# JeongsooP/RGB-no-more

Hardware: AMD Instinct MI355X
Metric: images/sec JPEG-Ti DCT 512x512 train step (higher is better)
Workload: dtype bf16

## Files before the change

### include/rgbnm.h

```cpp
#ifndef RGBNM_H
#define RGBNM_H
#include <stddef.h>
#include <stdint.h>

#ifdef __cplusplus
extern "C" {
#endif

#define RGBNM_ABI_VERSION 3
#define RGBNM_DT_F32 0
#define RGBNM_DT_BF16 1
#define RGBNM_DT_F16 2
#define RGBNM_DT_I16 2

#define RGBNM_EPI_NONE 0
#define RGBNM_EPI_RES 1
#define RGBNM_EPI_GELU 2
#define RGBNM_EPI_POS 3
#define RGBNM_EPI_DGELU 4
#define RGBNM_EPI_TANH 5
#define RGBNM_EPI_DTANH 6
#define RGBNM_EPI_RES_DROP 7
#define RGBNM_EPI_GELU_DROP 8

// ... 61 lines not shown
                        void* workspace, size_t workspace_bytes, void* stream);

int rgbnm_attention_fwd(int dtype, const void* qkv, void* out, float* lse, int B, int N, int heads, float scale,
                        void* stream);
int rgbnm_attention_bwd(int dtype, const void* qkv, const void* out, const void* dout, const float* lse, void* dqkv,
                        int B, int N, int heads, float scale, void* stream);

int rgbnm_subblock_embed(int in_dtype, int out_dtype, const void* y, const void* cbcr, const float* conv16,
                         void* feat, int B, int Hb, int Wb, int transpose_a, void* stream);
int rgbnm_subblock_embed_mix(int in_dtype, int out_dtype, const void* y, const void* cbcr, const float* lam_dev, const float* conv16,
                             void* feat, int B, int Hb, int Wb, int transpose_a, void* stream);

#define RGBNM_OP_IDENTITY 0
#define RGBNM_OP_AUTOCONTRAST 1
#define RGBNM_OP_POSTERIZE 2
#define RGBNM_OP_SOLARIZEADD 3
#define RGBNM_OP_COLOR 4
#define RGBNM_OP_CONTRAST 5
#define RGBNM_OP_BRIGHTNESS 6
#define RGBNM_OP_MIDFREQAUG 7
#define RGBNM_OP_CUTOUT 8
#define RGBNM_OP_TRANSLATEX 9
#define RGBNM_OP_TRANSLATEY 10
#define RGBNM_OP_ROTATE90 11
#define RGBNM_OP_AUTOSATURATION 12
#define RGBNM_OP_GRAYSCALE 13
#define RGBNM_OP_CHROMADROP 14
#define RGBNM_OP_SHARPNESS 15
#define RGBNM_OP_INVERT 16
#define RGBNM_OP_SOLARIZE 17
#define RGBNM_OP_FREQENHANCE 18
#define RGBNM_OP_EQUALIZE 19

typedef struct rgbnm_aug_params {
  int crop_i, crop_j, crop_h, crop_w;
  int flip;
  int op[2];
  float fmag[2];
  int iarg0[2], iarg1[2], iarg2[2];
} rgbnm_aug_params;

size_t rgbnm_dct_augment_workspace(int B);
int rgbnm_dct_augment(const int16_t* Yq, const int16_t* CbCrq, const int16_t* quant, const rgbnm_aug_params* params_dev,
                      const rgbnm_aug_params* params_host, const float* conv16, const float* filters, void* outY,
                      void* outC, int out_dtype, int B, int Hy, int Wy, int Hc, int Wc, int entry_clamp, int nops,
                      void* workspace, size_t workspace_bytes, void* stream);
size_t rgbnm_dct_augment_workspace_ex(int B, int size);
int rgbnm_dct_augment_ex(const int16_t* Yq, const int16_t* CbCrq, const int16_t* quant, const rgbnm_aug_params* params_dev,
                         const rgbnm_aug_params* params_host, const float* conv16, const float* filters, void* outY,
                         void* outC, int out_dtype, int size, int B, int Hy, int Wy, int Hc, int Wc, int entry_clamp,
                         int nops, void* workspace, size_t workspace_bytes, void* stream);

int rgbnm_dct_augment_packed(const int16_t* Ypacked, const int16_t* Cpacked, const long long* y_off, const long long* c_off,
                             const int16_t* quant, const rgbnm_aug_params* params_dev, const rgbnm_aug_params* params_host,
                             const float* conv16, const float* filters, void* outY, void* outC, int out_dtype, int size, int B,
                             int Hy, int Wy, int Hc, int Wc, int entry_clamp, int nops, void* workspace, size_t workspace_bytes,
                             void* stream);

int rgbnm_softxent(int dl_dtype, const float* logits, const float* soft_target, const long long* hard_target,
                   float* loss_rows, float* loss, void* dlogits, int B, int C, float grad_scale, void* stream);
int rgbnm_softxent_loss(const float* logits, const float* soft_target, const long long* hard_target, float* loss_rows,
                        float* row_stats, float* loss, unsigned* ticket, int B, int C, void* stream);
int rgbnm_softxent_grad(int dl_dtype, const float* logits, const float* soft_target, const long long* hard_target,
                        const float* row_stats, const float* gout_dev, void* dlogits, int B, int C, float grad_scale, void* stream);
int rgbnm_softxent_loss_mix(const float* logits, const long long* labels, const float* mix_lam_dev, float* loss_rows,
                            float* row_stats, float* loss, unsigned* ticket, int B, int C, void* stream);
int rgbnm_softxent_grad_mix(int dl_dtype, const float* logits, const long long* labels, const float* mix_lam_dev,
                            const float* row_stats, const float* gout_dev, void* dlogits, int B, int C, float grad_scale,
                            void* stream);
int rgbnm_mixup(int in_dtype, int out_dtype, const void* in, void* out, const float* lam_dev, int B,
                long long per_sample, void* stream);
int rgbnm_mixup_target(const long long* labels, float* target, const float* lam_dev, int B, int C, void* stream);
size_t rgbnm_clip_adamw_wd_workspace(void);
int rgbnm_clip_adamw_wd_step(float* p, const float* g, float* m, float* v, const unsigned char* wd_flag_per_256,
                             long long n, float lr, float beta1, float beta2, float eps, int step, float wd_factor,
                             float max_norm, float* norm_out, void* workspace, size_t workspace_bytes, void* stream);

typedef struct rgbnm_vit_cfg {
  int dtype, B, N, E, heads;
  float ln_eps, attn_scale;
} rgbnm_vit_cfg;

typedef struct rgbnm_block_params {
  const float *ln1_g, *ln1_b, *ln2_g, *ln2_b;
  const float *bqkv_perm, *bproj, *b1, *b2;
  const void *wqkv, *wqkv_t, *wproj, *wproj_t, *w1, *w1_t, *w2, *w2_t;
} rgbnm_block_params;

typedef struct rgbnm_block_acts {
  void* x_in;
  void* xn1;
  float *mean1, *rstd1;
  void* qkv;
  float* lse;
  void* attn;
  void* x_mid;
  void* xn2;
  float *mean2, *rstd2;
  void* u;
  void* gl;
  void* x_out;
} rgbnm_block_acts;

typedef struct rgbnm_block_grads {
  float *dln1_g, *dln1_b, *dln2_g, *dln2_b;
  float *dwqkv, *dbqkv, *dwproj, *dbproj, *dw1, *db1, *dw2, *db2;
} rgbnm_block_grads;

typedef struct rgbnm_block_scratch {
  void* du;
  void* dxn;
  void* dx_mid;
  void* dattn;
  void* dqkv;
  void* ws;
  size_t ws_bytes;
} rgbnm_block_scratch;

size_t rgbnm_vit_workspace(const rgbnm_vit_cfg* cfg);
size_t rgbnm_vit_workspace_ex(const rgbnm_vit_cfg* cfg, int n_classes);
int rgbnm_vit_block_fwd(const rgbnm_vit_cfg* cfg, const rgbnm_block_params* p, const rgbnm_block_acts* a,
                        void* stream);
int rgbnm_vit_ln_chain(const rgbnm_vit_cfg* cfg);
int rgbnm_vit_block_fwd_chain(const rgbnm_vit_cfg* cfg, const rgbnm_block_params* p, const rgbnm_block_acts* a,
                              int flags, const rgbnm_block_params* next_p, const rgbnm_block_acts* next_a,
                              void* stream);
int rgbnm_vit_block_bwd(const rgbnm_vit_cfg* cfg, const rgbnm_block_params* p, const rgbnm_block_acts* a,
                        const rgbnm_block_grads* g, const rgbnm_block_scratch* s, const void* dy, void* dx,
                        void* stream);

typedef struct rgbnm_dropout {
  const void* seed;
  float p;
  int block;
  void *dy_m, *dxmid_m;
} rgbnm_dropout;
int rgbnm_vit_block_fwd_drop(const rgbnm_vit_cfg* cfg, const rgbnm_block_params* p, const rgbnm_block_acts* a,
                             const rgbnm_dropout* d, void* stream);
int rgbnm_vit_block_bwd_drop(const rgbnm_vit_cfg* cfg, const rgbnm_block_params* p, const rgbnm_block_acts* a,
                             const rgbnm_block_grads* g, const rgbnm_block_scratch* s, const rgbnm_dropout* d, const void* dy,
                             void* dx, void* stream);

typedef struct rgbnm_chain_block {
  const void* wimg;
  const float *ln1_g, *ln1_b, *ln2_g, *ln2_b, *bqkv_perm, *bproj, *b1, *b2;
  void* xn1; float *mean1, *rstd1;
  void* qkv; float* lse; void* attn; void* x_mid; void* xn2; float *mean2, *rstd2;
  void* u; void* gl; void* x_out;
} rgbnm_chain_block;
size_t rgbnm_chain_block_bytes(void);
long long rgbnm_chain_image_elems(void);
int rgbnm_chain_gather(const void* src, const int* idx, void* dst, long long n, void* stream);
int rgbnm_vit_chain_fwd(const rgbnm_vit_cfg* cfg, const rgbnm_chain_block* blocks, int depth, const void* x0, void* stream);

typedef struct rgbnm_chain_bwd_block {
  const void* wimg;
  const float *ln1_g, *ln2_g;
  const void* x_in; const float *mean1, *rstd1;
  const void* qkv; const float* lse; const void* attn; const void* x_mid; const float *mean2, *rstd2; const void* u;
  const void* dy;
  void* du; void* dx_mid; void* dqkv; void* dx;
  float *part2, *part1;
} rgbnm_chain_bwd_block;
size_t rgbnm_chain_bwd_block_bytes(void);
int rgbnm_vit_chain_bwd(const rgbnm_vit_cfg* cfg, const rgbnm_chain_bwd_block* blocks, int depth, void* dattn, void* stream);
int rgbnm_vit_block_bwd_dw(const rgbnm_vit_cfg* cfg, const rgbnm_block_acts* a, const rgbnm_block_grads* g,
                           const rgbnm_block_scratch* s, const void* dy, const float* part2, const float* part1, void* stream);
int rgbnm_vit_blocks_bwd_dw(const rgbnm_vit_cfg* cfg, int n, const rgbnm_block_acts* const* a, const rgbnm_block_grads* const* g,
                            const rgbnm_block_scratch* const* s, const void* const* dy, const float* const* part2,
                            const float* const* part1, void* stream);
int rgbnm_vit_blocks_bwd_dw_pe(const rgbnm_vit_cfg* cfg, int n, const rgbnm_block_acts* const* a, const rgbnm_block_grads* const* g,
                               const rgbnm_block_scratch* const* s, const void* const* dy, const float* const* part2,
                               const float* const* part1, const void* pe_dx0, const void* pe_feat, float* pe_dw, float* pe_db,
                               void* pe_ws, size_t pe_ws_bytes, void* stream);

int rgbnm_gelu_table_init(void* stream);
int rgbnm_gelu_table_info(int* win16, unsigned* full65536);

int rgbnm_reduce_hold_begin(void);
int rgbnm_reduce_hold_end(void* table, void* table_host, size_t table_bytes, void* stream);
void rgbnm_reduce_hold_cancel(void);
size_t rgbnm_reduce_hold_table_bytes(void);

int rgbnm_patch_embed_fwd(const rgbnm_vit_cfg* cfg, int in_dtype, const void* y, const void* cbcr,
                          const float* conv16, const void* wpe, const float* bpe, const float* pos, void* feat,
                          void* x0, int Hb, int Wb, void* stream);
int rgbnm_patch_embed_fwd_mix(const rgbnm_vit_cfg* cfg, int in_dtype, const void* y, const void* cbcr, const float* lam_dev,
                              const float* conv16, const void* wpe, const float* bpe, const float* pos, void* feat, void* x0,
                              int Hb, int Wb, void* stream);
int rgbnm_patch_embed_bwd(const rgbnm_vit_cfg* cfg, const void* dx0, const void* feat, float* dwpe, float* dbpe,
                          void* ws, size_t ws_bytes, void* stream);

typedef struct rgbnm_head_params {
  const float *ln_g, *ln_b, *b1, *b2;
  const void *w1, *w1_t, *w2, *w2_t;
  int n_classes;
  int _pad;
} rgbnm_head_params;
typedef struct rgbnm_head_acts {
  void* x;
  float *mean, *rstd;
  void* pooled;
  void* h1;
  float* logits;
} rgbnm_head_acts;
typedef struct rgbnm_head_grads {
  float *dln_g, *dln_b, *dw1, *db1, *dw2, *db2;
} rgbnm_head_grads;
int rgbnm_head_fwd(const rgbnm_vit_cfg* cfg, const rgbnm_head_params* p, const rgbnm_head_acts* a, void* stream);
size_t rgbnm_head_bwd_workspace(const rgbnm_vit_cfg* cfg, int n_classes);
int rgbnm_head_bwd(const rgbnm_vit_cfg* cfg, const rgbnm_head_params* p, const rgbnm_head_acts* a,
                   const rgbnm_head_grads* g, const void* dlogits, void* da, void* dpooled, void* dx, void* ws,
                   size_t ws_bytes, void* stream);

int rgbnm_swin_embed(int in_dtype, int out_dtype, const void* y, const void* cbcr, const float* convY, const float* convC,
                     void* feat, int B, int Hb, int Wb, void* stream);
int rgbnm_ln_generic_fwd(int dtype, const void* x, const float* gamma, const float* beta, const void* res,
                         const float* sample_scale, int rows_per_sample, void* y, float* mean, float* rstd, int M, int E,
                         float eps, void* stream);
size_t rgbnm_ln_generic_bwd_workspace(int M, int E);
int rgbnm_ln_generic_bwd(int dtype, const void* dy, const void* x, const float* gamma, const float* mean,
                         const float* rstd, const float* sample_scale, int rows_per_sample, void* dx, float* dgamma,
                         float* dbeta, int M, int E, int accumulate, void* workspace, size_t workspace_bytes,
                         void* stream);
int rgbnm_window_attention_fwd(int dtype, const void* qkv, const float* bias, const float* scale, void* out, float* lse,
                               int B, int res, int C, int heads, int shift, void* stream);
size_t rgbnm_window_attention_bwd_workspace(int B, int res, int heads);
int rgbnm_window_attention_bwd(int dtype, const void* qkv, const void* out, const void* dout, const float* bias,
                               float* dscale , const float* scale, const float* lse, void* dqkv,
                               float* dbias, float* dscale_part, int B, int res, int C, int heads, int shift, void* workspace,
                               size_t workspace_bytes, void* stream);
typedef struct rgbnm_cpb_block {
  const float *w1, *b1, *w2, *ls;
  float *bias, *scale;
  const float *dbias, *dscale;
  float *dw1, *db1, *dw2, *dls;
  int heads, _pad;
} rgbnm_cpb_block;
size_t rgbnm_swin_cpb_table_elems(int nblocks);
int rgbnm_swin_cpb_fwd(const rgbnm_cpb_block* blocks, int nblocks, const float* coords, const int* index, float* table, void* stream);
int rgbnm_swin_cpb_bwd(const rgbnm_cpb_block* blocks, int nblocks, const float* coords, const int* inv_index, const float* table,
                       float* dtable, void* stream);
int rgbnm_merge_gather(int dtype, const void* in, void* out, int B, int res, int C, int inverse, void* stream);
int rgbnm_token_mean(int dtype, const void* in, void* out, int B, int N, int C, int backward, void* stream);


int rgbnm_calib_mfma_bf16(int workgroups, int iters, float* sink, void* stream);
int rgbnm_calib_stream(const void* src, void* dst, size_t bytes, int mode, int workgroups, void* sink, void* stream);
int rgbnm_calib_vmem_issue(int mode, int workgroups, int waves, void* buf, size_t wave_bytes, int ld,
                           unsigned long long* out, void* stream);
int rgbnm_calib_l2(const void* buf, size_t slice_bytes, int iters, int mode, int workgroups, int waves, void* sink,
                   void* stream);
int rgbnm_calib_pipes(const int* role_dev, int waves, int iters, int workgroups, unsigned long long* out, float* sink,
                      void* stream);

int rgbnm_calib_occupy(const void* buf, size_t slice_bytes, int workgroups, int lds_bytes, long long ticks, int mode,
                       const int* stop, void* sink, void* stream);
int rgbnm_calib_occupy_log(const void* buf, size_t slice_bytes, int workgroups, int lds_bytes, long long ticks, int mode,
                           const int* stop, void* sink, unsigned long long* log, void* stream);

#ifdef __cplusplus
}
#endif
#endif
```

### rgb-no-more_amd/csrc/vit.hip

```cpp
#include "common.h"
#include "../../include/rgbnm.h"

#define TRY(x)                 \
  do {                         \
    int rc__ = (x);            \
    if (rc__ != 0) return rc__; \
  } while (0)

static inline size_t max_sz(size_t a, size_t b) { return a > b ? a : b; }

#include <string.h>
#include <atomic>
#include <mutex>
#include <vector>
#include "internal.h"
namespace {
std::mutex g_trace_mu;
struct TraceRec { hipEvent_t a, b; int tag; double flops, bytes; };
std::vector<TraceRec> g_recs;
std::vector<hipEvent_t> g_event_pool;
hipEvent_t take_event() {
  if (!g_event_pool.empty()) { hipEvent_t e = g_event_pool.back(); g_event_pool.pop_back(); return e; }
  hipEvent_t e = nullptr;
  if (hipEventCreate(&e) != hipSuccess) return nullptr;
  return e;
}
struct Opt { const char* name; std::atomic<int> value; };
Opt g_opts[] = {{"nt_staged", 1}, {"tn_tr", 1}, {"tn_pipe", 1}, {"attn_v2", 1}, {"nt_wres", 1}, {"nt_kpipe", 1}, {"attn_persist", 1}, {"ln_fuse", 1}, {"tn_group", 2}, {"trace", 0}, {"tn_wgs", 512}, {"mlp_fuse", 1}, {"nt_cold", 0}, {"mlp_bwd", 1}, {"nt_small", 1}, {"mlp_dmast", 1}, {"gelu_table", 1}, {"ln_rows", 1}, {"kp8", 1}, {"win_xcd", 1}, {"kp_persist", 1}, {"fwd_chain", 1}, {"bwd_chain", 1}, {"tn_direct", 1}, {"tn_pack", 1}, {"tn_wide", 1}};
}

int rgbnm_trace_begin(int tag, double flops, double bytes, hipStream_t st) {
  int mask = 0;
  for (auto& o : g_opts) if (!strcmp(o.name, "trace")) mask = o.value.load(std::memory_order_relaxed);
  if (!((mask >> tag) & 1)) return -1;
  std::lock_guard<std::mutex> lk(g_trace_mu);
  TraceRec r;
  r.a = take_event();
  r.b = take_event();
  if (!r.a || !r.b) return -1;
  r.tag = tag; r.flops = flops; r.bytes = bytes;
  (void)hipEventRecord(r.a, st);
  g_recs.push_back(r);
  return (int)g_recs.size() - 1;
}
void rgbnm_trace_end(int slot, hipStream_t st) {
  if (slot < 0) return;
  std::lock_guard<std::mutex> lk(g_trace_mu);
  if (slot >= 0 && slot < (int)g_recs.size()) (void)hipEventRecord(g_recs[slot].b, st);
}

extern "C" {

int rgbnm_abi_version(void) { return RGBNM_ABI_VERSION; }

int rgbnm_set_option(const char* name, int value) {
  for (auto& o : g_opts)
    if (name && !strcmp(o.name, name)) { o.value.store(value, std::memory_order_relaxed); return RGBNM_OK; }
  return RGBNM_EINVAL;
}
int rgbnm_get_option(const char* name) {
  for (auto& o : g_opts)
    if (name && !strcmp(o.name, name)) return o.value.load(std::memory_order_relaxed);
  return -1;
}

int rgbnm_trace_reserve(int n_events) {
  if (n_events < 0 || n_events > (1 << 16)) return RGBNM_EINVAL;
  std::lock_guard<std::mutex> lk(g_trace_mu);
  while ((int)g_event_pool.size() < n_events) {
    hipEvent_t e = nullptr;
    if (hipEventCreate(&e) != hipSuccess) return RGBNM_ELAUNCH;
    g_event_pool.push_back(e);
  }
  return RGBNM_OK;
}

int rgbnm_trace_collect(int tag, double* ms_total, double* flops_total, double* bytes_total, int* count) {
  double ms = 0, fl = 0, by = 0;
  int n = 0;
  std::lock_guard<std::mutex> lk(g_trace_mu);
  std::vector<TraceRec> keep;
  for (auto& r : g_recs) {
    if (r.tag != tag) { keep.push_back(r); continue; }
    if (hipEventSynchronize(r.b) != hipSuccess) return RGBNM_ELAUNCH;
    float t = 0.f;
    if (hipEventElapsedTime(&t, r.a, r.b) != hipSuccess) return RGBNM_ELAUNCH;
    ms += t; fl += r.flops; by += r.bytes; ++n;
    g_event_pool.push_back(r.a);
    g_event_pool.push_back(r.b);
  }
  g_recs.swap(keep);
  if (ms_total) *ms_total = ms;
  if (flops_total) *flops_total = fl;
  if (bytes_total) *bytes_total = by;
  if (count) *count = n;
  return RGBNM_OK;
}

const char* rgbnm_strerror(int code) {
  switch (code) {
    case 0: return "ok";
    case RGBNM_EINVAL: return "invalid argument (null pointer, bad shape, alignment or dtype)";
    case RGBNM_ELAUNCH: return "HIP kernel launch failed";
    case RGBNM_EWORKSPACE: return "workspace too small";
    default: return "unknown rgbnm error";
  }
}

static bool fused_dx_lnbwd(int dt, const void* A, int lda, const void* Wt, int ldw, const void* x, const float* gamma,
                           const float* mean, const float* rstd, const void* dres, void* dx, float* dgamma,
                           float* dbeta, int M, int E, int K, void* ws, size_t ws_bytes, hipStream_t st) {
  if (dt != RGBNM_DT_BF16 || E != 192 || !rgbnm_get_option("ln_fuse") || !rgbnm_get_option("nt_kpipe")) return false;
  if (ws_bytes < (size_t)cdiv(M, cdiv(M, 512)) * 2 * E * sizeof(float)) return false;
  int npanels = 0;
  const int rc = rgbnm_launch_nt_kpipe_lnbwd(A, lda, Wt, ldw, x, E, gamma, mean, rstd, dres, E, dx, E, (float*)ws,
                                             &npanels, M, E, K, st);
  if (rc != RGBNM_OK) return false;
  RgbnmReduceJob j;
  j.part = (const float*)ws; j.stride = 2LL * E; j.out = dgamma; j.n = E; j.S = npanels; j.cols = 1; j.perm_heads = 0;
  j.accumulate = 0; j.epw = 8;
  if (rgbnm_reduce_submit(j, st) != RGBNM_OK) return false;
  j.part = (const float*)ws + E; j.out = dbeta;
  return rgbnm_reduce_submit(j, st) == RGBNM_OK;
}

static bool fused_mlp_bwd(int dt, const void* dy, const void* w2t, const void* w1t, const void* gp, void* du, const void* x,
                          const float* gamma, const float* mean, const float* rstd, void* dx, float* dgamma, float* dbeta,
                          int M, int E, void* ws, size_t ws_bytes, hipStream_t st) {
  if (dt != RGBNM_DT_BF16 || E != 192 || !rgbnm_get_option("mlp_bwd") || !rgbnm_get_option("ln_fuse")) return false;
  if (ws_bytes < (size_t)cdiv(M, cdiv(M, 256)) * 2 * E * sizeof(float)) return false;
  int npanels = 0;
  const int rc = rgbnm_launch_mlp_bwd(dy, E, w2t, w1t, gp, 4 * E, du, 4 * E, x, E, gamma, mean, rstd, dx, E, (float*)ws,
                                      &npanels, M, E, 4 * E, st);
  if (rc != RGBNM_OK) return false;
  RgbnmReduceJob j;
  j.part = (const float*)ws; j.stride = 2LL * E; j.out = dgamma; j.n = E; j.S = npanels; j.cols = 1; j.perm_heads = 0;
  j.accumulate = 0; j.epw = 8;
  if (rgbnm_reduce_submit(j, st) != RGBNM_OK) return false;
  j.part = (const float*)ws + E; j.out = dbeta;
  return rgbnm_reduce_submit(j, st) == RGBNM_OK;
}

static size_t block_ws_offsets(int M, int E, int I, size_t (&off)[7]) {
  const size_t sz[6] = {rgbnm_gemm_tn_workspace(M, E, 4 * E), rgbnm_gemm_tn_workspace(M, 4 * E, E),
                        rgbnm_gemm_tn_workspace(M, E, I),     rgbnm_gemm_tn_workspace(M, 3 * I, E),
                        rgbnm_layernorm_bwd_workspace(M, E),  rgbnm_layernorm_bwd_workspace(M, E)};
  off[0] = 0;
  for (int i = 0; i < 6; ++i) off[i + 1] = off[i] + ((sz[i] + 255) & ~(size_t)255);
  return off[6];
}

size_t rgbnm_vit_workspace(const rgbnm_vit_cfg* c) { return rgbnm_vit_workspace_ex(c, 1024); }

size_t rgbnm_vit_workspace_ex(const rgbnm_vit_cfg* c, int n_classes) {
  if (!c) return 0;
  if (n_classes < 1024) n_classes = 1024;
  const int M = c->B * c->N, E = c->E, I = c->heads * 64;
  size_t off[7];
  size_t w = block_ws_offsets(M, E, I, off);
  w = max_sz(w, rgbnm_gemm_tn_workspace(M, E, 384));
  w = max_sz(w, rgbnm_gemm_tn_workspace(c->B, n_classes, E));
  w = max_sz(w, rgbnm_layernorm_bwd_workspace(M, E));
  w = max_sz(w, (size_t)c->B * 2 * E * sizeof(float));
  return w;
}

int rgbnm_vit_ln_chain(const rgbnm_vit_cfg* c) {
  if (!c) return 0;
  return c->dtype == RGBNM_DT_BF16 && c->E == 192 && c->B * c->N >= 8192 && rgbnm_get_option("ln_fuse") &&
         rgbnm_get_option("nt_kpipe");
}

int rgbnm_vit_block_fwd_chain(const rgbnm_vit_cfg* c, const rgbnm_block_params* p, const rgbnm_block_acts* a, int flags,
                              const rgbnm_block_params* next_p, const rgbnm_block_acts* next_a, void* st) {
  if (!c || !p || !a) return RGBNM_EINVAL;
  const int dt = c->dtype, M = c->B * c->N, E = c->E, I = c->heads * 64;
  const bool chain = rgbnm_vit_ln_chain(c) != 0;
  if ((flags & 1) && !chain) return RGBNM_EINVAL;
  if (!(flags & 1))
    TRY(rgbnm_layernorm_fwd(dt, a->x_in, p->ln1_g, p->ln1_b, a->xn1, a->mean1, a->rstd1, M, E, c->ln_eps, st));
  TRY(rgbnm_gemm_nt(dt, RGBNM_EPI_NONE, a->xn1, E, p->wqkv, E, a->qkv, 3 * I, p->bqkv_perm, 0, 0, 0, 0, 0, 0, M,
// ... 61 lines not shown
  char* wsb = (char*)s->ws;
#define WS(i) (wsb + off[i]), (off[(i) + 1] - off[i])
  rgbnm_reduce_defer_begin();
  bool tn_open = false;
  const int rc = [&]() -> int {
  int group = rgbnm_get_option("tn_group");
  const bool wide4 = rgbnm_get_option("tn_wide") && E % 384 == 0 && I % 384 == 0 && M % 64 == 0;
  if (group == 2 && E > 192 && !wide4) group = 1;
  if (group) { rgbnm_tn_defer_begin(); tn_open = true; }
  const void* dyg = dy;
  if (d) {
    TRY(rgbnm_dropout_apply(dt, d->seed, d->p, 2, d->block, dy, E, d->dy_m, E, M, E, st));
    dyg = d->dy_m;
  }
  TRY(rgbnm_gemm_tn(dt, dyg, E, a->gl, 4 * E, g->dw2, g->db2, M, E, 4 * E, 0, 0, WS(0), st));
  const bool mlp_bwd_fused = !d && fused_mlp_bwd(dt, dy, p->w2_t, p->w1_t, a->u, s->du, a->x_mid, p->ln2_g, a->mean2, a->rstd2,
                                                 s->dx_mid, g->dln2_g, g->dln2_b, M, E, WS(4), (hipStream_t)st);
  if (!mlp_bwd_fused)
    TRY(rgbnm_gemm_nt(dt, RGBNM_EPI_DGELU, dyg, E, p->w2_t, E, s->du, 4 * E, 0, a->u, 4 * E, 0, 0, 0, 0, M, 4 * E, E, 0,
                      st));
  TRY(rgbnm_gemm_tn(dt, s->du, 4 * E, a->xn2, E, g->dw1, g->db1, M, 4 * E, E, 0, 0, WS(1), st));
  if (group == 1) { tn_open = false; TRY(rgbnm_tn_defer_flush((hipStream_t)st)); }
  if (mlp_bwd_fused) {
  } else if (!fused_dx_lnbwd(dt, s->du, 4 * E, p->w1_t, 4 * E, a->x_mid, p->ln2_g, a->mean2, a->rstd2, dy, s->dx_mid,
                      g->dln2_g, g->dln2_b, M, E, 4 * E, WS(4), (hipStream_t)st)) {
    TRY(rgbnm_gemm_nt(dt, RGBNM_EPI_NONE, s->du, 4 * E, p->w1_t, 4 * E, s->dxn, E, 0, 0, 0, 0, 0, 0, 0, M, E, 4 * E,
                      0, st));
    TRY(rgbnm_layernorm_bwd(dt, s->dxn, a->x_mid, p->ln2_g, a->mean2, a->rstd2, dy, s->dx_mid, g->dln2_g, g->dln2_b,
                            M, E, 0, WS(4), st));
  }
  const void* dxmg = s->dx_mid;
  if (d) {
    TRY(rgbnm_dropout_apply(dt, d->seed, d->p, 0, d->block, s->dx_mid, E, d->dxmid_m, E, M, E, st));
    dxmg = d->dxmid_m;
  }
  if (group == 1) { rgbnm_tn_defer_begin(); tn_open = true; }
  TRY(rgbnm_gemm_tn(dt, dxmg, E, a->attn, I, g->dwproj, g->dbproj, M, E, I, 0, 0, WS(2), st));
  TRY(rgbnm_gemm_nt(dt, RGBNM_EPI_NONE, dxmg, E, p->wproj_t, E, s->dattn, I, 0, 0, 0, 0, 0, 0, 0, M, I, E, 0, st));
  TRY(rgbnm_attention_bwd(dt, a->qkv, a->attn, s->dattn, a->lse, s->dqkv, c->B, c->N, c->heads, c->attn_scale, st));
  TRY(rgbnm_gemm_tn(dt, s->dqkv, 3 * I, a->xn1, E, g->dwqkv, g->dbqkv, M, 3 * I, E, c->heads, 0, WS(3), st));
  if (group) { tn_open = false; TRY(rgbnm_tn_defer_flush((hipStream_t)st)); }
  if (!fused_dx_lnbwd(dt, s->dqkv, 3 * I, p->wqkv_t, 3 * I, a->x_in, p->ln1_g, a->mean1, a->rstd1, s->dx_mid, dx,
                      g->dln1_g, g->dln1_b, M, E, 3 * I, WS(5), (hipStream_t)st)) {
    TRY(rgbnm_gemm_nt(dt, RGBNM_EPI_NONE, s->dqkv, 3 * I, p->wqkv_t, 3 * I, s->dxn, E, 0, 0, 0, 0, 0, 0, 0, M, E,
                      3 * I, 0, st));
    TRY(rgbnm_layernorm_bwd(dt, s->dxn, a->x_in, p->ln1_g, a->mean1, a->rstd1, s->dx_mid, dx, g->dln1_g, g->dln1_b, M,
                            E, 0, WS(5), st));
  }
  return RGBNM_OK;
  }();
#undef WS
  const int rt = tn_open ? rgbnm_tn_defer_flush((hipStream_t)st) : RGBNM_OK;
  const int rf = rgbnm_reduce_defer_flush((hipStream_t)st);
  return rc != RGBNM_OK ? rc : (rt != RGBNM_OK ? rt : rf);
}

int rgbnm_vit_block_bwd(const rgbnm_vit_cfg* c, const rgbnm_block_params* p, const rgbnm_block_acts* a,
                        const rgbnm_block_grads* g, const rgbnm_block_scratch* s, const void* dy, void* dx, void* st) {
  return block_bwd(c, p, a, g, s, nullptr, dy, dx, st);
}

int rgbnm_vit_block_bwd_drop(const rgbnm_vit_cfg* c, const rgbnm_block_params* p, const rgbnm_block_acts* a,
                             const rgbnm_block_grads* g, const rgbnm_block_scratch* s, const rgbnm_dropout* d, const void* dy,
                             void* dx, void* st) {
  if (!d) return RGBNM_EINVAL;
  return block_bwd(c, p, a, g, s, d, dy, dx, st);
}

int rgbnm_vit_blocks_bwd_dw(const rgbnm_vit_cfg* c, int n, const rgbnm_block_acts* const* a, const rgbnm_block_grads* const* g,
                            const rgbnm_block_scratch* const* s, const void* const* dy, const float* const* part2,
                            const float* const* part1, void* st) {
  return rgbnm_vit_blocks_bwd_dw_pe(c, n, a, g, s, dy, part2, part1, nullptr, nullptr, nullptr, nullptr, nullptr, 0, st);
}

int rgbnm_vit_blocks_bwd_dw_pe(const rgbnm_vit_cfg* c, int n, const rgbnm_block_acts* const* a, const rgbnm_block_grads* const* g,
                               const rgbnm_block_scratch* const* s, const void* const* dy, const float* const* part2,
                               const float* const* part1, const void* pe_dx0, const void* pe_feat, float* pe_dw, float* pe_db,
                               void* pe_ws, size_t pe_ws_bytes, void* st) {
  if (!c || n < 1 || n > 12 || !a || !g || !s || !dy || !part2 || !part1) return RGBNM_EINVAL;
  if (pe_dx0 && (!pe_feat || !pe_dw || !pe_ws)) return RGBNM_EINVAL;
  const int dt = c->dtype, M = c->B * c->N, E = c->E, I = c->heads * 64;
  size_t off[7];
  const size_t need = block_ws_offsets(M, E, I, off);
  for (int i = 0; i < n; ++i) {
    if (!a[i] || !g[i] || !s[i] || !dy[i] || !part2[i] || !part1[i]) return RGBNM_EINVAL;
    if (s[i]->ws_bytes < need) return RGBNM_EWORKSPACE;
    for (int k = 0; k < i; ++k)
      if (s[k]->ws == s[i]->ws) return RGBNM_EINVAL;
  }
  rgbnm_reduce_defer_begin();
  bool tn_open = false;
  const int rc = [&]() -> int {
    const int group = rgbnm_get_option("tn_group");
    if (group) { rgbnm_tn_defer_begin_n(group == 1 ? 2 : 4 * n + (pe_dx0 ? 1 : 0)); tn_open = true; }
    for (int i = 0; i < n; ++i) {
      char* wsb = (char*)s[i]->ws;
#define WS(k) (wsb + off[k]), (off[(k) + 1] - off[k])
      TRY(rgbnm_gemm_tn(dt, dy[i], E, a[i]->gl, 4 * E, g[i]->dw2, g[i]->db2, M, E, 4 * E, 0, 0, WS(0), st));
      TRY(rgbnm_gemm_tn(dt, s[i]->du, 4 * E, a[i]->xn2, E, g[i]->dw1, g[i]->db1, M, 4 * E, E, 0, 0, WS(1), st));
      TRY(rgbnm_gemm_tn(dt, s[i]->dx_mid, E, a[i]->attn, I, g[i]->dwproj, g[i]->dbproj, M, E, I, 0, 0, WS(2), st));
      TRY(rgbnm_gemm_tn(dt, s[i]->dqkv, 3 * I, a[i]->xn1, E, g[i]->dwqkv, g[i]->dbqkv, M, 3 * I, E, c->heads, 0, WS(3), st));
#undef WS
    }
    if (pe_dx0) TRY(rgbnm_gemm_tn(dt, pe_dx0, E, pe_feat, 384, pe_dw, pe_db, M, E, 384, 0, 0, pe_ws, pe_ws_bytes, st));
    if (group) { tn_open = false; TRY(rgbnm_tn_defer_flush((hipStream_t)st)); }
    for (int i = 0; i < n; ++i) {
      RgbnmReduceJob j;
      j.stride = 2LL * E; j.n = E; j.S = c->B; j.cols = 1; j.perm_heads = 0; j.accumulate = 0; j.epw = 8;
      j.part = part2[i]; j.out = g[i]->dln2_g;
      TRY(rgbnm_reduce_submit(j, (hipStream_t)st));
      j.part = part2[i] + E; j.out = g[i]->dln2_b;
      TRY(rgbnm_reduce_submit(j, (hipStream_t)st));
      j.part = part1[i]; j.out = g[i]->dln1_g;
      TRY(rgbnm_reduce_submit(j, (hipStream_t)st));
      j.part = part1[i] + E; j.out = g[i]->dln1_b;
      TRY(rgbnm_reduce_submit(j, (hipStream_t)st));
    }
    return RGBNM_OK;
  }();
  const int rt = tn_open ? rgbnm_tn_defer_flush((hipStream_t)st) : RGBNM_OK;
  const int rf = rgbnm_reduce_defer_flush((hipStream_t)st);
  return rc != RGBNM_OK ? rc : (rt != RGBNM_OK ? rt : rf);
}

int rgbnm_vit_block_bwd_dw(const rgbnm_vit_cfg* c, const rgbnm_block_acts* a, const rgbnm_block_grads* g,
                           const rgbnm_block_scratch* s, const void* dy, const float* part2, const float* part1, void* st) {
  return rgbnm_vit_blocks_bwd_dw(c, 1, &a, &g, &s, &dy, &part2, &part1, st);
}

int rgbnm_patch_embed_fwd_mix(const rgbnm_vit_cfg* c, int in_dtype, const void* y, const void* cbcr, const float* lam_dev,
                              const float* conv16, const void* wpe, const float* bpe, const float* pos, void* feat, void* x0, int Hb,
                              int Wb, void* st) {
  if (!c) return RGBNM_EINVAL;
  const int M = c->B * c->N;
  if ((Hb / 2) * (Wb / 2) != c->N) return RGBNM_EINVAL;
  TRY(rgbnm_subblock_embed_mix(in_dtype, c->dtype, y, cbcr, lam_dev, conv16, feat, c->B, Hb, Wb, 0, st));
  TRY(rgbnm_gemm_nt(c->dtype, RGBNM_EPI_POS, feat, 384, wpe, 384, x0, c->E, bpe, 0, 0, 0, 0, pos, c->N, M, c->E, 384,
                    0, st));
  return RGBNM_OK;
}

int rgbnm_patch_embed_fwd(const rgbnm_vit_cfg* c, int in_dtype, const void* y, const void* cbcr, const float* conv16,
                          const void* wpe, const float* bpe, const float* pos, void* feat, void* x0, int Hb, int Wb,
                          void* st) {
  return rgbnm_patch_embed_fwd_mix(c, in_dtype, y, cbcr, nullptr, conv16, wpe, bpe, pos, feat, x0, Hb, Wb, st);
}

int rgbnm_patch_embed_bwd(const rgbnm_vit_cfg* c, const void* dx0, const void* feat, float* dwpe, float* dbpe,
                          void* ws, size_t ws_bytes, void* st) {
  if (!c) return RGBNM_EINVAL;
  return rgbnm_gemm_tn(c->dtype, dx0, c->E, feat, 384, dwpe, dbpe, c->B * c->N, c->E, 384, 0, 0, ws, ws_bytes, st);
}

int rgbnm_head_fwd(const rgbnm_vit_cfg* c, const rgbnm_head_params* p, const rgbnm_head_acts* a, void* st) {
  if (!c || !p || !a) return RGBNM_EINVAL;
  const int dt = c->dtype, E = c->E, C = p->n_classes;
  TRY(rgbnm_head_pool_fwd(dt, a->x, p->ln_g, p->ln_b, a->pooled, a->mean, a->rstd, c->B, c->N, E, c->ln_eps, st));
  TRY(rgbnm_gemm_nt(dt, RGBNM_EPI_TANH, a->pooled, E, p->w1, E, a->h1, E, p->b1, 0, 0, 0, 0, 0, 0, c->B, E, E, 0, st));
  TRY(rgbnm_gemm_nt(dt, RGBNM_EPI_NONE, a->h1, E, p->w2, E, a->logits, C, p->b2, 0, 0, 0, 0, 0, 0, c->B, C, E, 1, st));
  return RGBNM_OK;
}

size_t rgbnm_head_bwd_workspace(const rgbnm_vit_cfg* c, int n_classes) {
  if (!c) return 0;
  return ((rgbnm_gemm_tn_workspace(c->B, n_classes, c->E) + 255) & ~(size_t)255) + ((rgbnm_gemm_tn_workspace(c->B, c->E, c->E) + 255) & ~(size_t)255) +
         (size_t)c->B * 2 * c->E * sizeof(float);
}

int rgbnm_head_bwd(const rgbnm_vit_cfg* c, const rgbnm_head_params* p, const rgbnm_head_acts* a,
                   const rgbnm_head_grads* g, const void* dlogits, void* da, void* dpooled, void* dx, void* ws,
                   size_t ws_bytes, void* st) {
  if (!c || !p || !a || !g || !dlogits || !da || !dpooled || !dx) return RGBNM_EINVAL;
  const int dt = c->dtype, E = c->E, C = p->n_classes, B = c->B;
  const size_t s1 = (rgbnm_gemm_tn_workspace(B, C, E) + 255) & ~(size_t)255, s2 = (rgbnm_gemm_tn_workspace(B, E, E) + 255) & ~(size_t)255;
  const size_t s3 = (size_t)B * 2 * E * sizeof(float);
  const bool apart = ws_bytes >= s1 + s2 + s3;
  char* w1 = (char*)ws;
  char* w2 = apart ? w1 + s1 : w1;
  char* w3 = apart ? w2 + s2 : w1;
  const size_t b1 = apart ? s1 : ws_bytes, b2 = apart ? s2 : ws_bytes, b3 = apart ? ws_bytes - s1 - s2 : ws_bytes;
  const bool grouped = apart && rgbnm_get_option("tn_group") != 0;
  if (grouped) rgbnm_tn_defer_begin();
  const int rc = [&]() -> int {
    TRY(rgbnm_gemm_tn(dt, dlogits, C, a->h1, E, g->dw2, g->db2, B, C, E, 0, 0, w1, b1, st));
    TRY(rgbnm_gemm_nt(dt, RGBNM_EPI_DTANH, dlogits, C, p->w2_t, C, da, E, 0, a->h1, E, 0, 0, 0, 0, B, E, C, 0, st));
    TRY(rgbnm_gemm_tn(dt, da, E, a->pooled, E, g->dw1, g->db1, B, E, E, 0, 0, w2, b2, st));
    return RGBNM_OK;
  }();
  const int rt = grouped ? rgbnm_tn_defer_flush((hipStream_t)st) : RGBNM_OK;
  if (rc != RGBNM_OK) return rc;
  if (rt != RGBNM_OK) return rt;
  TRY(rgbnm_gemm_nt(dt, RGBNM_EPI_NONE, da, E, p->w1_t, E, dpooled, E, 0, 0, 0, 0, 0, 0, 0, B, E, E, 0, st));
  TRY(rgbnm_head_pool_bwd(dt, dpooled, a->x, p->ln_g, a->mean, a->rstd, dx, g->dln_g, g->dln_b, B, c->N, E, 0, w3, b3, st));
  return RGBNM_OK;
}

}
```

### rgb-no-more_amd/csrc/vit_chain.hip

```cpp
#include "common.h"
#include <string.h>
#include <type_traits>
#include "internal.h"
#include "tile128.h"
#include "../../include/rgbnm.h"

namespace {

constexpr int E = 192, HID = 768, HD = 64, HEADS = 3, NTOK = 196, NTILE = 7, NPAD = 224, INNER = HEADS * HD;
constexpr int NCW = 7, NTHREADS = 64 * (NCW + 1);
constexpr int SLOT = 24576;
constexpr int A_SLOT0 = 0;
constexpr int K_OFF = 3 * SLOT;
constexpr int ARR = NPAD * ROWB;
constexpr int V_OFF = K_OFF + ARR;
constexpr int STGA_OFF = V_OFF + ARR;
constexpr int STG_TILE = 32 * ROWB;
constexpr int MISC_OFF = STGA_OFF + 6 * STG_TILE + 4 * ROWB;
constexpr int BPROJ_OFF = MISC_OFF + 2 * E * 4, BQKV_OFF = BPROJ_OFF + E * 4;
constexpr int LN1P_OFF = K_OFF + NTOK * ROWB;
constexpr int TAB_LIMIT = 13328;
constexpr int ST1_OFF = 13440;
constexpr int STAGE = 2 * SLOT;
constexpr int TA_OFF = ST1_OFF + STAGE;
constexpr int B1R_OFF = TA_OFF + 2 * STG_TILE + 2 * 4 * ROWB;
constexpr int B2_OFF = B1R_OFF + 512;
constexpr int FLAG_OFF = B2_OFF + E * 4;
constexpr int ST0_OFF = K_OFF;
constexpr int TB_OFF = ST0_OFF + STAGE;
constexpr int SMEM = 163840;
#ifndef PIPE_QKV
#define PIPE_QKV 6
#endif
#ifndef PIPE_P
#define PIPE_P 6
#endif
#ifndef PIPE_M1
#define PIPE_M1 5
#endif
#ifndef PIPE_M2
#define PIPE_M2 6
#endif
static_assert(BQKV_OFF + 3 * INNER * 4 <= SMEM, "LDS");
static_assert(TB_OFF + 10 * STG_TILE <= SMEM, "LDS");
static_assert(FLAG_OFF + 16 <= ST0_OFF, "LDS");
static_assert(LN1P_OFF + 2 * E * 4 <= V_OFF, "LDS");
static_assert(TAB_LIMIT <= ST1_OFF && ST1_OFF % 128 == 0 && TA_OFF % 128 == 0, "LDS");

struct ChainBlk {
  const bf16* wimg;
  const float *ln1_g, *ln1_b, *ln2_g, *ln2_b, *bqkv, *bproj, *b1, *b2;
  bf16* xn1; float *mean1, *rstd1;
  bf16* qkv; float* lse; bf16* attn; bf16* x_mid; bf16* xn2; float *mean2, *rstd2;
  bf16* gp; bf16* gl; bf16* x_out;
};
static_assert(sizeof(ChainBlk) == sizeof(rgbnm_chain_block), "rgbnm_chain_block layout");
constexpr int MAX_DEPTH = 12;
struct ChainArgs {
  ChainBlk blk[MAX_DEPTH]; const bf16* x0;
  int depth, nimg;
  float eps, scale;
  const unsigned* tab_img; int tab_pieces;
  unsigned kneg, kpos, klo, koff, ksgn;
};

#ifndef X_STORE
#define X_STORE 1
#endif
template <typename V, typename P>
__device__ __forceinline__ void gstore(P* ptr, const V& v) {
#if X_STORE == 1
  __builtin_nontemporal_store(v, reinterpret_cast<V*>(ptr));
#elif X_STORE == 2
  asm volatile("global_store_dwordx4 %0, %1, off sc1\n\ts_nop 2" ::"v"(reinterpret_cast<V*>(ptr)), "v"(v) : "memory");
#elif X_STORE == 3
  asm volatile("global_store_dwordx4 %0, %1, off sc0 sc1\n\ts_nop 2" ::"v"(reinterpret_cast<V*>(ptr)), "v"(v) : "memory");
#else
  *reinterpret_cast<V*>(ptr) = v;
#endif
}

__device__ __forceinline__ void dma_f32x192(const float* src, unsigned char* dst, int lane) {
#pragma unroll
  for (int i = 0; i < 3; ++i)
    __builtin_amdgcn_global_load_lds((glb_ptr)(src + 64 * i + lane), (lds_ptr)(dst + 256 * i), 4, 0, 0);
}

struct Rows { u32x4 v[12]; };
__device__ __forceinline__ float bf_lo(unsigned u) { return __builtin_bit_cast(float, u << 16); }
__device__ __forceinline__ float bf_hi(unsigned u) { return __builtin_bit_cast(float, u & 0xffff0000u); }

__device__ __forceinline__ void ln_stats(const Rows& x, float& mu, float& rs, float eps) {
  float s0 = 0.f, s1 = 0.f;
#pragma unroll
  for (int c = 0; c < 12; ++c)
#pragma unroll
    for (int d = 0; d < 4; ++d) {
      const unsigned u = opaque(x.v[c][d]);
      s0 += bf_lo(u);
      s1 += bf_hi(u);
    }
  float s = s0 + s1;
  s += __shfl_xor(s, 32, 64);
  mu = s * (1.f / E);
  float q0 = 0.f, q1 = 0.f;
#pragma unroll
  for (int c = 0; c < 12; ++c)
#pragma unroll
    for (int d = 0; d < 4; ++d) {
      const unsigned u = opaque(x.v[c][d]);
      const float d0 = bf_lo(u) - mu, d1 = bf_hi(u) - mu;
      q0 = __builtin_fmaf(d0, d0, q0);
      q1 = __builtin_fmaf(d1, d1, q1);
    }
  float q = q0 + q1;
  q += __shfl_xor(q, 32, 64);
  rs = rsqrtf(__builtin_fmaf(q, 1.f / E, eps));
}
__device__ __forceinline__ void ln_apply(const Rows& x, float mu, float rs, const float* gb, int g, Rows& y) {
#ifdef X_NOLN
#pragma unroll
  for (int c = 0; c < 12; ++c) y.v[c] = x.v[c];
  return;
#endif
#pragma unroll
  for (int c = 0; c < 12; ++c) {
    const float* gp = gb + 16 * c + 8 * g;
    const f32x4 g0 = *reinterpret_cast<const f32x4*>(gp), g1 = *reinterpret_cast<const f32x4*>(gp + 4);
    const f32x4 b0 = *reinterpret_cast<const f32x4*>(gp + E), b1 = *reinterpret_cast<const f32x4*>(gp + E + 4);
#pragma unroll
    for (int d = 0; d < 4; ++d) {
      const float gm0 = d < 2 ? g0[2 * d] : g1[2 * d - 4], gm1 = d < 2 ? g0[2 * d + 1] : g1[2 * d - 3];
      const float bt0 = d < 2 ? b0[2 * d] : b1[2 * d - 4], bt1 = d < 2 ? b0[2 * d + 1] : b1[2 * d - 3];
      const unsigned u = opaque(x.v[c][d]);
      y.v[c][d] = pack2(__builtin_fmaf((bf_lo(u) - mu) * rs, gm0, bt0), __builtin_fmaf((bf_hi(u) - mu) * rs, gm1, bt1));
    }
    if (c & 1) __builtin_amdgcn_sched_barrier(0);
  }
}

__device__ __forceinline__ void tile_out(unsigned char* smem, unsigned stg, const u32x4& p0, const u32x4& p1, const u32x4& p2,
                                         const u32x4& p3, bf16* dst, int ld, int live) {
  const int ln = lane_id_here();
  const unsigned wo = stg + (unsigned)((ln & 31) * ROWB + (((ln >> 5) ^ (ln & 7)) << 4));
  if ((ln & 31) < live) {
    *reinterpret_cast<u32x4*>(smem + wo) = p0;
    *reinterpret_cast<u32x4*>(smem + (wo ^ 32u)) = p1;
    *reinterpret_cast<u32x4*>(smem + (wo ^ 64u)) = p2;
    *reinterpret_cast<u32x4*>(smem + (wo ^ 96u)) = p3;
  }
  own_tile_fence();
  const int rl = ln >> 3, seg = ln & 7;
  const unsigned ro = stg + (unsigned)(rl * ROWB + ((seg ^ rl) << 4));
  bf16* gp = dst + (size_t)rl * ld + seg * 8;
  u32x4 v[4];
#pragma unroll
  for (int i = 0; i < 4; ++i) v[i] = *reinterpret_cast<const u32x4*>(smem + ro + i * 8 * ROWB);
#ifndef X_NOSAVE
  if (live == 32) {
#pragma unroll
    for (int i = 0; i < 4; ++i) gstore(gp + (size_t)i * 8 * ld, v[i]);
  } else {
#pragma unroll
    for (int i = 0; i < 4; ++i)
      if (i * 8 + rl < live) gstore(gp + (size_t)i * 8 * ld, v[i]);
  }
#endif
  own_tile_fence();
}
__device__ __forceinline__ void rows_out(unsigned char* smem, unsigned stg, const Rows& x, bf16* dst, int live) {
#pragma unroll
  for (int t = 0; t < 3; ++t) {
    tile_out(smem, stg, x.v[4 * t], x.v[4 * t + 1], x.v[4 * t + 2], x.v[4 * t + 3], dst + 64 * t, E, live);
    __builtin_amdgcn_sched_barrier(0);
  }
}

__device__ __forceinline__ void gemm_k192(f32x16& acc, const unsigned char* sW, int ht, const Rows& x, const Geo& L) {
  int wbase = L.l31 * (E * 2) + ((L.g ^ L.fl) << 4) + ht * 32 * (E * 2);
  asm volatile("" : "+v"(wbase));
  Frag<bf16> fb;
#pragma unroll
  for (int c = 0; c < 12; ++c) {
    Frag<bf16> fx;
#ifdef X_HALFW
    if ((c & 1) == 0)
#endif
    fb.v = *reinterpret_cast<const bf16x8*>(sW + ((wbase ^ ((c % 4) << 5)) + 128 * (c / 4)));
    fx.v = as_bf16x8(x.v[c]);
    mma(acc, fb, fx);
  }
}

template <int DEPTH>
__device__ __forceinline__ void gemm_k192x2(f32x16& a0, f32x16& a1, const unsigned char* sW, const Rows& x, const Geo& L) {
  int wb0 = L.l31 * (E * 2) + ((L.g ^ L.fl) << 4);
  asm volatile("" : "+v"(wb0));
  const int wb1 = wb0 + 32 * (E * 2);
  Frag<bf16> fb[24];
#pragma unroll
  for (int i = 0; i < 24; ++i) {
    const int c = i >> 1;
    fb[i].v = *reinterpret_cast<const bf16x8*>(sW + ((((i & 1) ? wb1 : wb0) ^ ((c % 4) << 5)) + 128 * (c / 4)));
  }
#pragma unroll
  for (int i = 0; i < 24; ++i) {
    Frag<bf16> fx;
    fx.v = as_bf16x8(x.v[i >> 1]);
    mma((i & 1) ? a1 : a0, fb[i], fx);
  }
  __builtin_amdgcn_sched_group_barrier(0x100, DEPTH, 0);
#pragma unroll
  for (int i = 0; i < 24 - DEPTH; ++i) {
    __builtin_amdgcn_sched_group_barrier(0x008, 1, 0);
    __builtin_amdgcn_sched_group_barrier(0x100, 1, 0);
  }
#pragma unroll
  for (int i = 0; i < DEPTH; ++i) __builtin_amdgcn_sched_group_barrier(0x008, 1, 0);
}

#ifdef CHAIN_PROF
#ifndef CHAIN_PROF_BLK
#define CHAIN_PROF_BLK 1
#endif
__device__ unsigned long long g_chain_prof[8 * 8 * 128];
#define CP(i)                                                                                          \
  do {                                                                                                 \
    if (ib == CHAIN_PROF_BLK && blockIdx.x < 8) {                                                      \
      const unsigned long long t_ = __builtin_amdgcn_s_memtime();                                      \
      if ((threadIdx.x & 63) == 0) g_chain_prof[(blockIdx.x * 8 + (threadIdx.x >> 6)) * 128 + (i)] = t_; \
    }                                                                                                  \
  } while (0)
#define CP_RT(i)                                                                                       \
  do {                                                                                                 \
    if (blockIdx.x < 8 && (threadIdx.x & 63) == 0)                                                     \
      g_chain_prof[(blockIdx.x * 8 + (threadIdx.x >> 6)) * 128 + (i)] = __builtin_amdgcn_s_memrealtime(); \
  } while (0)
#else
#define CP(i) do {} while (0)
#define CP_RT(i) do {} while (0)
#endif
#define BAR(s) do { CP(2 * (s)); wg_barrier(); CP(2 * (s) + 1); } while (0)

__global__ __launch_bounds__(NTHREADS) void vit_chain_fwd_kernel(ChainArgs p) {
  extern __shared__ __attribute__((aligned(16))) unsigned char smem[];
  const int img = blockIdx.x;
  if (img >= p.nimg) return;
  const Geo L = make_geo();
  const int w = __builtin_amdgcn_readfirstlane(threadIdx.x >> 6);
  const int depth = p.depth;
  CP_RT(126);

  if (w == NCW) {
#ifdef X_DMAPRIO
    __builtin_amdgcn_s_setprio(X_DMAPRIO);
#endif
    const int lane = L.lane;
    auto chunkA = [&](const ChainBlk& b, int idx, int slot) {
      dma_linear<24>(reinterpret_cast<const unsigned char*>(b.wimg) + (size_t)idx * SLOT, smem + A_SLOT0 + slot * SLOT, lane);
    };
    auto chunkM = [&](const ChainBlk& b, int c) {
      unsigned char* st = smem + ((c & 1) ? ST1_OFF : ST0_OFF);
      dma_linear<48>(reinterpret_cast<const unsigned char*>(b.wimg) + (size_t)12 * SLOT + (size_t)c * STAGE, st, lane);
    };
    auto bias1 = [&](const ChainBlk& b, int c) {
      __builtin_amdgcn_global_load_lds((glb_ptr)(b.b1 + c * 64 + lane), (lds_ptr)(smem + B1R_OFF + (c & 1) * 256), 4, 0, 0);
    };
    auto ln1p = [&](const ChainBlk& b) {
      dma_f32x192(b.ln1_g, smem + LN1P_OFF, lane);
      dma_f32x192(b.ln1_b, smem + LN1P_OFF + E * 4, lane);
    };
    auto misc = [&](const ChainBlk& b) {
      dma_f32x192(b.ln2_g, smem + MISC_OFF, lane);
      dma_f32x192(b.ln2_b, smem + MISC_OFF + E * 4, lane);
      dma_f32x192(b.bproj, smem + BPROJ_OFF, lane);
#pragma unroll
      for (int i = 0; i < 3; ++i) dma_f32x192(b.bqkv + i * INNER, smem + BQKV_OFF + i * INNER * 4, lane);
    };
    {
      const ChainBlk& b0 = p.blk[0];
      ln1p(b0);
      misc(b0);
      chunkA(b0, 0, 0);
      chunkA(b0, 1, 1);
      wait_vm<24>();
      wg_barrier();
    }
    for (int ib = 0; ib < depth; ++ib) {
      const ChainBlk& b = p.blk[ib];
      wait_vm<24>(); BAR(0);
      chunkA(b, 2, 2); wait_vm<24>(); BAR(1);
      chunkA(b, 3, 0); wait_vm<24>(); BAR(2);
      chunkA(b, 4, 1); BAR(3);
      chunkA(b, 5, 2); wait_vm<48>(); BAR(4);
      wait_vm<24>(); BAR(5);
      chunkA(b, 6, 0); wait_vm<24>(); BAR(6);
      chunkA(b, 7, 1); BAR(7);
      chunkA(b, 8, 2); wait_vm<48>(); BAR(8);
      wait_vm<24>(); BAR(9);
      chunkA(b, 9, 0); wait_vm<24>(); BAR(10);
      chunkA(b, 10, 1); BAR(11);
      chunkA(b, 11, 2); wait_vm<48>(); BAR(12);
      chunkM(b, 0); wait_vm<63>(); BAR(13);
      {
        for (int i = 0; i * 64 < p.tab_pieces; ++i)
          if (i * 64 + lane < p.tab_pieces)
            __builtin_amdgcn_global_load_lds((glb_ptr)(p.tab_img + (i * 64 + lane) * 4), (lds_ptr)(smem + i * 1024), 16, 0, 0);
      }
      wait_vm<48>(); BAR(14);
      BAR(15);
      bias1(b, 0);
      dma_f32x192(b.b2, smem + B2_OFF, lane);
      volatile int* flag = reinterpret_cast<volatile int*>(smem + FLAG_OFF);
      if (lane == 0) *flag = 0;
      u32x4 tv[3][2][4];
      const int trow = lane >> 3, tvec = lane & 7;
      auto take_tiles = [&]() {
#pragma unroll
        for (int q = 0; q < 3; ++q) {
          const unsigned tb = (unsigned)(q == 0 ? TB_OFF + 8 * STG_TILE : (q == 1 ? TA_OFF : TA_OFF + 2 * STG_TILE));
          const int lr = q == 2 ? NTOK - 6 * 32 : 32;
#pragma unroll
          for (int t = 0; t < 2; ++t)
#pragma unroll
            for (int i = 0; i < 4; ++i) {
              const int row = trow + 8 * i;
              if (row < lr) tv[q][t][i] = *reinterpret_cast<const u32x4*>(smem + tb + t * lr * ROWB + row * ROWB + ((tvec ^ (row & 7)) << 4));
            }
        }
        wait_lds();
      };
      auto store_tiles = [&](int chunk) {
#pragma unroll
        for (int q = 0; q < 3; ++q) {
          const int lr = q == 2 ? NTOK - 6 * 32 : 32;
#pragma unroll
          for (int i = 0; i < 4; ++i) {
            const int row = trow + 8 * i;
            if (row < lr) {
              const size_t go = ((size_t)img * NTOK + 32 * (4 + q) + row) * HID + chunk * 64 + tvec * 8;
#ifndef X_NOSAVE
              gstore(b.gl + go, tv[q][0][i]);
              gstore(b.gp + go, tv[q][1][i]);
#endif
            }
          }
        }
      };
      wait_vm<0>(); BAR(16);
      for (int c = 0; c < 11; ++c) {
        if (c >= 1) {
          take_tiles();
          if (lane == 0) *flag = c;
          store_tiles(c - 1);
        }
        chunkM(b, c + 1);
        bias1(b, c + 1);
        wait_vm<0>(); BAR(17 + c);
      }
      take_tiles();
      if (lane == 0) *flag = 11;
      store_tiles(10);
      if (ib + 1 < depth) ln1p(p.blk[ib + 1]);
      wait_vm<0>(); BAR(28);
      take_tiles();
      if (lane == 0) *flag = 12;
      store_tiles(11);
      if (ib + 1 < depth) {
        const ChainBlk& nb = p.blk[ib + 1];
        misc(nb);
        chunkA(nb, 0, 0);
        chunkA(nb, 1, 1);
      }
    }
    return;
  }

#if defined(X_PRIO) && X_PRIO == 1
  if (w >= 4) __builtin_amdgcn_s_setprio(1);
#elif defined(X_PRIO) && X_PRIO == 2
  if (w < 4) __builtin_amdgcn_s_setprio(1);
#endif
  const int row0 = 32 * w;
  const int live = NTOK - row0 < 32 ? NTOK - row0 : 32;
  const int tok = row0 + L.l31 < NTOK ? row0 + L.l31 : NTOK - 1;
  const size_t grow0 = (size_t)img * NTOK + row0;
  const unsigned stg = (unsigned)(STGA_OFF + w * STG_TILE);
  const float c2 = p.scale * 1.4426950408889634f;
  const float* ln1p = reinterpret_cast<const float*>(smem + LN1P_OFF);
  const float* ln2p = reinterpret_cast<const float*>(smem + MISC_OFF);
  const float* bprj = reinterpret_cast<const float*>(smem + BPROJ_OFF);

  Rows xr;
  {
    const bf16* xrow = p.x0 + ((size_t)img * NTOK + tok) * E + 8 * L.g;
#pragma unroll
    for (int c = 0; c < 12; ++c) xr.v[c] = *reinterpret_cast<const u32x4*>(xrow + 16 * c);
  }
  float mu1, rs1;
  ln_stats(xr, mu1, rs1, p.eps);
  asm volatile("s_waitcnt vmcnt(0)" ::: "memory");
  wg_barrier();
  {
    const ChainBlk& b0 = p.blk[0];
    Rows xn;
    ln_apply(xr, mu1, rs1, ln1p, L.g, xn);
    rows_out(smem, stg, xn, b0.xn1 + grow0 * E, live);
    if (L.g == 0 && L.l31 < live) {
      b0.mean1[grow0 + L.l31] = mu1;
      b0.rstd1[grow0 + L.l31] = rs1;
    }
  }

  for (int ib = 0; ib < depth; ++ib) {
    const ChainBlk& b = p.blk[ib];
    Frag<bf16> of[HEADS][4];
#pragma unroll
    for (int h = 0; h < HEADS; ++h) {
      const Geo L = fresh_geo();
      Rows xn;
      __builtin_amdgcn_sched_barrier(0);
      ln_apply(xr, mu1, rs1, ln1p, L.g, xn);
      __builtin_amdgcn_sched_barrier(0);
      Frag<bf16> qf[4];
#pragma unroll
      for (int m = 0; m < 3; ++m) {
        const float* bias = reinterpret_cast<const float*>(smem + BQKV_OFF) + m * INNER + h * HD + 8 * L.g;
        BAR(4 * h + m);
        const unsigned char* sW = smem + A_SLOT0 + m * SLOT;
        f32x16 acc[2];
#pragma unroll
        for (int ht = 0; ht < 2; ++ht)
#pragma unroll
          for (int r = 0; r < 16; ++r) acc[ht][r] = 0.f;
#ifdef X_NOPIPE
        gemm_k192(acc[0], sW, 0, xn, L);
        gemm_k192(acc[1], sW, 1, xn, L);
#else
        gemm_k192x2<PIPE_QKV>(acc[0], acc[1], sW, xn, L);
#endif
        u32x4 pc[4];
#pragma unroll
        for (int ht = 0; ht < 2; ++ht)
#pragma unroll
          for (int hs = 0; hs < 2; ++hs) {
            const f32x4 b0 = *reinterpret_cast<const f32x4*>(bias + 32 * ht + 16 * hs);
            const f32x4 b1 = *reinterpret_cast<const f32x4*>(bias + 32 * ht + 16 * hs + 4);
#pragma unroll
            for (int d = 0; d < 4; ++d)
              pc[2 * ht + hs][d] = pack2(acc[ht][8 * hs + 2 * d] + (d < 2 ? b0[2 * d] : b1[2 * d - 4]),
                                         acc[ht][8 * hs + 2 * d + 1] + (d < 2 ? b0[2 * d + 1] : b1[2 * d - 3]));
          }
        if (m == 0) {
#pragma unroll
          for (int c = 0; c < 4; ++c) qf[c].v = as_bf16x8(pc[c]);
        } else {
          const unsigned ao = opaque((unsigned)((m == 1 ? K_OFF : V_OFF) + (row0 + L.l31) * ROWB + ((L.g ^ L.fl) << 4)));
          if (m == 2 || L.l31 < live) {
#pragma unroll
            for (int c = 0; c < 4; ++c) *reinterpret_cast<u32x4*>(smem + (ao ^ (unsigned)(c << 5))) = pc[c];
          }
        }
        tile_out(smem, stg, pc[0], pc[1], pc[2], pc[3], b.qkv + grow0 * (3 * INNER) + m * INNER + h * HD, 3 * INNER, live);
      }
      BAR(4 * h + 3);
      {
        const Geo L = fresh_geo();
        const unsigned char* Ks = smem + K_OFF;
        unsigned rb = (unsigned)(L.l31 * ROWB + ((L.g ^ L.fl) << 4)), tr = L.tr0;
        asm volatile("" : "+v"(rb), "+v"(tr));
        float mx = -INFINITY;
#if defined(X_NOPIPE) || defined(X_NOATTN)
#ifdef X_NOATTN
        TileLoop<0>::run([&](auto tc) {
#else
        TileLoop<NTILE>::run([&](auto tc) {
#endif
          constexpr int t = decltype(tc)::value;
          f32x16 acc;
#pragma unroll
          for (int r = 0; r < 16; ++r) acc[r] = 0.f;
#pragma unroll
          for (int c = 0; c < 4; ++c) {
            Frag<bf16> kf;
            kf.v = *reinterpret_cast<const bf16x8*>(Ks + (rb ^ (unsigned)(c << 5)) + t * 32 * ROWB);
            mma(acc, kf, qf[c]);
          }
#pragma unroll
          for (int r = 0; r < 16; ++r) {
            float v = acc[r];
            if (t * 32 + 32 > NTOK && t * 32 + acc_row(r, L.lane) >= NTOK) v = -INFINITY;
            mx = fmaxf(mx, v);
          }
        });
#else
        {
          Frag<bf16> kc[4], kn[4];
          f32x16 prev;
#pragma unroll
          for (int c = 0; c < 4; ++c) kc[c].v = *reinterpret_cast<const bf16x8*>(Ks + (rb ^ (unsigned)(c << 5)));
          TileLoop<NTILE + 1>::run([&](auto tc) {
            constexpr int t = decltype(tc)::value;
            f32x16 acc;
            if (t + 1 < NTILE) {
#pragma unroll
              for (int c = 0; c < 4; ++c)
                kn[c].v = *reinterpret_cast<const bf16x8*>(Ks + (rb ^ (unsigned)(c << 5)) + (t + 1) * 32 * ROWB);
            }
            if (t < NTILE) {
#pragma unroll
              for (int r = 0; r < 16; ++r) acc[r] = 0.f;
#pragma unroll
              for (int c = 0; c < 4; ++c) mma(acc, kc[c], qf[c]);
            }
            if (t >= 1) {
#pragma unroll
              for (int r = 0; r < 16; ++r) {
                float v = prev[r];
                if (t * 32 > NTOK && (t - 1) * 32 + acc_row(r, L.lane) >= NTOK) v = -INFINITY;
                mx = fmaxf(mx, v);
              }
            }
            __builtin_amdgcn_sched_barrier(0);
            prev = acc;
#pragma unroll
            for (int c = 0; c < 4; ++c) kc[c] = kn[c];
          });
// ... 297 lines not shown
            agv[jj] = alo[jj] = ahi[jj] = 0;
            continue;
#endif
            unsigned p1, p2, ak, i4, sg;
            asm("v_pk_min_u16 %0, %1, %2" : "=v"(p1) : "v"(pb[jj]), "s"(kneg));
            asm("v_pk_min_i16 %0, %1, %2" : "=v"(p2) : "v"(p1), "s"(kpos));
            p1 &= 0x7FFF7FFFu;
            p2 &= 0x7FFF7FFFu;
            asm("v_pk_max_u16 %0, %1, %2" : "=v"(agv[jj]) : "v"(p1), "s"(0x00800080u));
            asm("v_pk_max_u16 %0, %1, %2" : "=v"(ak) : "v"(p2), "s"(klo));
            asm("v_pk_mad_u16 %0, %1, %2, %3" : "=v"(i4) : "v"(ak), "v"(k4v), "s"(koff));
            asm("v_pk_lshrrev_b16 %0, %1, %2" : "=v"(sg) : "s"(0x000F000Fu), "v"(pb[jj]));
            asm("v_pk_mad_u16 %0, %1, %2, %3" : "=v"(i4) : "v"(sg), "s"(ksgn), "v"(i4));
            alo[jj] = i4 & 0xffffu;
            ahi[jj] = i4 >> 16;
          }
#ifndef X_NOGELU
          asm volatile(
              "ds_read_b32 %0, %8\n\tds_read_b32 %1, %9\n\tds_read_b32 %2, %10\n\tds_read_b32 %3, %11\n\t"
              "ds_read_b32 %4, %12\n\tds_read_b32 %5, %13\n\tds_read_b32 %6, %14\n\tds_read_b32 %7, %15\n\t"
              "s_waitcnt lgkmcnt(0)"
              : "=&v"(e0[0]), "=&v"(e1[0]), "=&v"(e0[1]), "=&v"(e1[1]), "=&v"(e0[2]), "=&v"(e1[2]), "=&v"(e0[3]), "=&v"(e1[3])
              : "v"(alo[0]), "v"(ahi[0]), "v"(alo[1]), "v"(ahi[1]), "v"(alo[2]), "v"(ahi[2]), "v"(alo[3]), "v"(ahi[3])
              : "memory");
#endif
          u32x4 gq, dq;
#pragma unroll
          for (int jj = 0; jj < 4; ++jj) {
#ifdef X_NOGELU
            gq[jj] = dq[jj] = pb[jj];
#else
            const unsigned dpair = __builtin_amdgcn_perm(e1[jj], e0[jj], 0x05040100u);
            unsigned gm;
            asm("v_pk_sub_u16 %0, %1, %2" : "=v"(gm) : "v"(agv[jj]), "v"(dpair));
            gq[jj] = (pb[jj] & 0x80008000u) | gm;
            dq[jj] = __builtin_amdgcn_perm(e1[jj], e0[jj], 0x07060302u);
#endif
          }
          gv = __builtin_bit_cast(bf16x8, gq);
          dv = __builtin_bit_cast(bf16x8, dq);
          pg[hs].v = gv;
          if (lane_live) {
            const unsigned to = two ^ (unsigned)((2 * ht + hs) << 5);
            *reinterpret_cast<bf16x8*>(smem + to) = gv;
            *reinterpret_cast<bf16x8*>(smem + to + tpoff) = dv;
          }
        }
#ifdef X_NOPIPE
#pragma unroll
        for (int hs = 0; hs < 2; ++hs) {
          const int s = 2 * ht + hs;
          Frag<bf16> fw[6];
#pragma unroll
          for (int bt = 0; bt < 6; ++bt)
#ifdef X_HALFW
            if (bt & 1) fw[bt].v = fw[bt - 1].v; else
#endif
            fw[bt].v = *reinterpret_cast<const bf16x8*>(smem + (w2o ^ (unsigned)(s << 5)) + bt * 32 * ROWB);
#pragma unroll
          for (int bt = 0; bt < 6; ++bt) mma(acc2[bt], fw[bt], pg[hs]);
        }
#else
        __builtin_amdgcn_sched_barrier(0);
#pragma unroll
        for (int bt = 0; bt < 6; ++bt)
          fw2[6 + bt].v = *reinterpret_cast<const bf16x8*>(smem + (w2o ^ (unsigned)((2 * ht + 1) << 5)) + bt * 32 * ROWB);
#pragma unroll
        for (int bt = 0; bt < 6; ++bt) mma(acc2[bt], fw2[bt], pg[0]);
#pragma unroll
        for (int bt = 0; bt < 6; ++bt) mma(acc2[bt], fw2[6 + bt], pg[1]);
#pragma unroll
        for (int i = 0; i < 6; ++i) {
          __builtin_amdgcn_sched_group_barrier(0x008, 1, 0);
          __builtin_amdgcn_sched_group_barrier(0x100, 1, 0);
        }
        __builtin_amdgcn_sched_group_barrier(0x008, 6, 0);
        __builtin_amdgcn_sched_barrier(0);
#endif
      }
      if (handed) wait_lds();
      else own_tile_fence();
      if (!handed) {
        const int ln = lane_id_here();
        if (live == 32) {
          bf16x8 v0[4], v1[4];
#pragma unroll
          for (int i = 0; i < 4; ++i) {
            const int idx = ln + 64 * i, row = idx >> 3, vec = idx & 7;
            const unsigned so = tg + (unsigned)(row * ROWB + ((vec ^ (row & 7)) << 4));
            v0[i] = *reinterpret_cast<const bf16x8*>(smem + so);
            v1[i] = *reinterpret_cast<const bf16x8*>(smem + so + tpoff);
          }
#ifndef X_NOSAVE
#pragma unroll
          for (int i = 0; i < 4; ++i) {
            const int idx = ln + 64 * i, row = idx >> 3, vec = idx & 7;
            const size_t go = (grow0 + row) * HID + chunk * 64 + vec * 8;
            gstore(b.gl + go, v0[i]);
            gstore(b.gp + go, v1[i]);
          }
#endif
        } else {
#pragma unroll
          for (int i = 0; i < 4; ++i) {
            const int idx = ln + 64 * i, row = idx >> 3, vec = idx & 7;
            if (row < live) {
              const unsigned so = tg + (unsigned)(row * ROWB + ((vec ^ (row & 7)) << 4));
              const bf16x8 v0 = *reinterpret_cast<const bf16x8*>(smem + so);
              const bf16x8 v1 = *reinterpret_cast<const bf16x8*>(smem + so + tpoff);
              const size_t go = (grow0 + row) * HID + chunk * 64 + vec * 8;
#ifndef X_NOSAVE
              gstore(b.gl + go, v0);
              gstore(b.gp + go, v1);
#endif
            }
          }
        }
        own_tile_fence();
      }
    }
    BAR(28);
    while (__builtin_amdgcn_readfirstlane(*flag) < HID / 64) __builtin_amdgcn_s_sleep(1);
    {
      const float* b2p = reinterpret_cast<const float*>(smem + B2_OFF) + 8 * L.g;
#pragma unroll
      for (int c = 0; c < 12; ++c) {
        const f32x4 b0 = *reinterpret_cast<const f32x4*>(b2p + 16 * c), b1 = *reinterpret_cast<const f32x4*>(b2p + 16 * c + 4);
#pragma unroll
        for (int d = 0; d < 4; ++d)
          xr.v[c][d] = pack2(acc2[c >> 1][8 * (c & 1) + 2 * d] + (d < 2 ? b0[2 * d] : b1[2 * d - 4]),
                             acc2[c >> 1][8 * (c & 1) + 2 * d + 1] + (d < 2 ? b0[2 * d + 1] : b1[2 * d - 3]));
        if (c & 1) __builtin_amdgcn_sched_barrier(0);
      }
      __builtin_amdgcn_sched_barrier(0);
      rows_out(smem, stg, xr, b.x_out + grow0 * E, live);
      __builtin_amdgcn_sched_barrier(0);
      if (ib + 1 < depth) {
        const ChainBlk& nb = p.blk[ib + 1];
        ln_stats(xr, mu1, rs1, p.eps);
        __builtin_amdgcn_sched_barrier(0);
        Rows xn;
        ln_apply(xr, mu1, rs1, ln1p, L.g, xn);
        __builtin_amdgcn_sched_barrier(0);
        rows_out(smem, stg, xn, nb.xn1 + grow0 * E, live);
        __builtin_amdgcn_sched_barrier(0);
        if (L.g == 0 && L.l31 < live) {
          nb.mean1[grow0 + L.l31] = mu1;
          nb.rstd1[grow0 + L.l31] = rs1;
        }
      }
    }
    CP(58);
  }
  CP_RT(127);
}

__global__ __launch_bounds__(256) void chain_gather_kernel(const bf16* __restrict__ src, const int* __restrict__ idx,
                                                           bf16* __restrict__ dst, long long n8) {
  for (long long i = blockIdx.x * 256ll + threadIdx.x; i < n8; i += (long long)gridDim.x * 256) {
    const int4 a = *reinterpret_cast<const int4*>(idx + 8 * i), c = *reinterpret_cast<const int4*>(idx + 8 * i + 4);
    bf16x8 v;
    v[0] = src[a.x]; v[1] = src[a.y]; v[2] = src[a.z]; v[3] = src[a.w];
    v[4] = src[c.x]; v[5] = src[c.y]; v[6] = src[c.z]; v[7] = src[c.w];
    *reinterpret_cast<bf16x8*>(dst + 8 * i) = v;
  }
}

}

int rgbnm_gelu_table_query(const unsigned** img, int* A0, int* P1, int* N1, int* ndw);

#ifdef CHAIN_PROF
extern "C" int rgbnm_chain_prof_read(unsigned long long* host_out) {
  return hipMemcpyFromSymbol(host_out, HIP_SYMBOL(g_chain_prof), sizeof(unsigned long long) * 8 * 8 * 128) == hipSuccess ? 0 : -1;
}
#endif

extern "C" {

size_t rgbnm_chain_block_bytes(void) { return sizeof(ChainBlk); }
long long rgbnm_chain_image_elems(void) { return 12ll * (SLOT / 2) + 12ll * (STAGE / 2); }

int rgbnm_chain_gather(const void* src, const int* idx, void* dst, long long n, void* stream) {
  if (!src || !idx || !dst || n <= 0 || n % 8) return RGBNM_EINVAL;
  const long long n8 = n / 8;
  int grid = (int)((n8 + 255) / 256);
  if (grid > 2048) grid = 2048;
  hipLaunchKernelGGL(chain_gather_kernel, dim3(grid), dim3(256), 0, (hipStream_t)stream, (const bf16*)src, idx, (bf16*)dst, n8);
  LAUNCH_CHECK();
  return RGBNM_OK;
}

int rgbnm_vit_chain_fwd(const rgbnm_vit_cfg* c, const rgbnm_chain_block* blocks, int depth, const void* x0, void* stream) {
  if (!c || !blocks || !x0 || depth <= 0) return RGBNM_EINVAL;
  if (c->dtype != RGBNM_DT_BF16 || c->E != E || c->heads != HEADS || c->N != NTOK || c->B < 1 || depth > MAX_DEPTH) return 1;
  const unsigned* img = nullptr;
  int A0 = 0, P1 = 0, N1 = 0, ndw = 0;
  if (rgbnm_gelu_table_query(&img, &A0, &P1, &N1, &ndw) != 1 || ndw * 4 > TAB_LIMIT) return 1;
  ChainArgs p;
  memcpy(p.blk, blocks, sizeof(ChainBlk) * depth);
  p.x0 = (const bf16*)x0; p.depth = depth; p.nimg = c->B;
  p.eps = c->ln_eps; p.scale = c->attn_scale;
  p.tab_img = img; p.tab_pieces = (ndw * 4 + 15) / 16;
  p.kneg = 0x00010001u * (unsigned)(0x8000 | N1);
  p.kpos = 0x00010001u * (unsigned)P1;
  p.klo = 0x00010001u * (unsigned)(A0 - 1);
  p.koff = 0x00010001u * (unsigned)((0x10000 - 4 * (A0 - 1)) & 0xffff);
  p.ksgn = 0x00010001u * (unsigned)(4 * (P1 - A0 + 2));
  static DevOnce attr;
  if (attr.need()) {
    if (hipFuncSetAttribute((const void*)vit_chain_fwd_kernel, hipFuncAttributeMaxDynamicSharedMemorySize, SMEM) != hipSuccess)
      return RGBNM_ELAUNCH;
    attr.done();
  }
  const double tok = (double)c->B * NTOK;
  const double flops = depth * tok * 2.0 * (E * 3.0 * INNER + 2.0 * NTOK * INNER + INNER * E + 2.0 * E * HID);
  const double bytes = depth * (tok * ((5.0 * E + 3.0 * INNER + 2.0 * HID) * 2.0 + 4 * 4 + HEADS * 4) + 12.0 * SLOT + 12.0 * STAGE) + tok * E * 2.0;
  const int slot = rgbnm_trace_begin(TR_CHAIN_FWD, flops, bytes, (hipStream_t)stream);
  hipLaunchKernelGGL(vit_chain_fwd_kernel, dim3(c->B), dim3(NTHREADS), SMEM, (hipStream_t)stream, p);
  rgbnm_trace_end(slot, (hipStream_t)stream);
  LAUNCH_CHECK();
  return RGBNM_OK;
}

}
```

### rgb-no-more_amd/csrc/vit_chain_bwd.hip

```cpp
#include "common.h"
#include <string.h>
#include <type_traits>
#include "internal.h"
#include "ln_bwd_rows.h"
#include "tile128.h"
#include "../../include/rgbnm.h"

namespace {

constexpr int E = 192, HID = 768, HD = 64, HEADS = 3, NTOK = 196, NTILE = 7, NPAD = 224, INNER = HEADS * HD, LDQ = 3 * INNER;
constexpr int NCW = 7, NTHREADS = 64 * (NCW + 1), CTHREADS = 64 * NCW, BM = 32 * NCW;
constexpr int ARR = NPAD * ROWB, SLOT = 24576, STAGE = 2 * SLOT, CH = 64, NCHUNK = HID / CH;
constexpr int CP = E + 4;
constexpr int SMEM = 163840;
#ifndef PIPE_P
#define PIPE_P 6
#endif
#ifndef PIPE_M1
#define PIPE_M1 5
#endif
#ifndef PIPE_X
#define PIPE_X 7
#endif
constexpr int M_STG = 2 * STAGE;
constexpr int TILE = 32 * ROWB;
typedef rgbnm::LnBwdRows<CTHREADS, BM> LnBwd;
constexpr int RED_OFF = (BM * CP * 2 + 1023) / 1024 * 1024;
static_assert(RED_OFF + LnBwd::RED_BYTES <= 132096, "LDS");
constexpr int P_SLOT0 = 132096, P_SLOT1 = 0, P_TILES = 98304;
static_assert(P_SLOT0 + SLOT <= SMEM && P_TILES + NCW * TILE <= P_SLOT0, "LDS");
constexpr int A_Q = 0, A_K = ARR, A_V = 2 * ARR, A_G = 3 * ARR, A_L2 = 4 * ARR, A_D = A_L2 + NPAD * 4, A_STG = A_D + NPAD * 4;
constexpr int A_SIDE = A_STG + NCW * STG_WAVE;
static_assert(A_SIDE + NCW * 1024 <= SMEM, "LDS");
constexpr int X_SLOT0 = A_K, X_SLOT1 = A_K + SLOT, X_SLOT2 = 0, X_TILES = A_K + 2 * SLOT, X_TSET = NCW * TILE;
static_assert(X_SLOT1 + SLOT <= X_TILES && X_TILES + 3 * X_TSET <= SMEM && SLOT <= A_K, "LDS");

struct BwdBlk {
  const bf16* wimg;
  const float *ln1_g, *ln2_g;
  const bf16* x_in; const float *mean1, *rstd1;
  const bf16* qkv; const float* lse; const bf16* attn; const bf16* x_mid; const float *mean2, *rstd2; const bf16* gp;
  const bf16* dy;
  bf16* du; bf16* dx_mid; bf16* dqkv; bf16* dx;
  float *part2, *part1;
};
static_assert(sizeof(BwdBlk) == sizeof(rgbnm_chain_bwd_block), "rgbnm_chain_bwd_block layout");
constexpr int MAX_DEPTH = 12;
struct BwdArgs {
  BwdBlk blk[MAX_DEPTH]; bf16* dattn;
  int depth, nimg;
  float scale;
};

#ifndef XB_ROWPIPE
#define XB_ROWPIPE 1
#endif
#ifndef XB_NT
#define XB_NT 1
#endif
#ifndef XB_NTLD
#define XB_NTLD 0
#endif
constexpr int A_AUX = (XB_NTLD & 2) ? 2 : 0;
template <bool NT, typename V, typename P>
__device__ __forceinline__ void gstore(P* ptr, const V& v) {
#ifdef XB_NOSTORE
  if ((XB_NOSTORE & 1) && NT) return;
  if ((XB_NOSTORE & 2) && !NT) return;
#endif
  if constexpr (NT) __builtin_nontemporal_store(v, reinterpret_cast<V*>(ptr));
  else *reinterpret_cast<V*>(ptr) = v;
}

struct Rows { u32x4 v[12]; };

__device__ __forceinline__ void dma_row_tiles(const bf16* __restrict__ src, int ld, unsigned char* dst, int lane) {
#pragma unroll 4
  for (int i = 0; i < 28; ++i) {
    const int row = 8 * i + (lane >> 3), pc = lane & 7;
    const int lc = pc ^ (row & 7);
    const int srow = row < NTOK ? row : NTOK - 1;
    __builtin_amdgcn_global_load_lds((glb_ptr)(src + (size_t)srow * ld + lc * 8), (lds_ptr)(dst + i * 1024), 16, 0, 0);
  }
}

__device__ __forceinline__ void tile_out(unsigned char* smem, unsigned stg, const u32x4& p0, const u32x4& p1, const u32x4& p2,
                                         const u32x4& p3, bf16* dst, int ld, int live) {
  const int ln = lane_id_here();
  const unsigned wo = stg + (unsigned)((ln & 31) * ROWB + (((ln >> 5) ^ (ln & 7)) << 4));
  *reinterpret_cast<u32x4*>(smem + wo) = p0;
  *reinterpret_cast<u32x4*>(smem + (wo ^ 32u)) = p1;
  *reinterpret_cast<u32x4*>(smem + (wo ^ 64u)) = p2;
  *reinterpret_cast<u32x4*>(smem + (wo ^ 96u)) = p3;
  own_tile_fence();
  const int rl = ln >> 3, seg = ln & 7;
  const unsigned ro = stg + (unsigned)(rl * ROWB + ((seg ^ rl) << 4));
  bf16* gp = dst + (size_t)rl * ld + seg * 8;
  u32x4 v[4];
#pragma unroll
  for (int i = 0; i < 4; ++i) v[i] = *reinterpret_cast<const u32x4*>(smem + ro + i * 8 * ROWB);
  if (live == 32) {
#pragma unroll
    for (int i = 0; i < 4; ++i) gstore<(XB_NT & 4) != 0>(gp + (size_t)i * 8 * ld, v[i]);
  } else {
#pragma unroll
    for (int i = 0; i < 4; ++i)
      if (i * 8 + rl < live) gstore<(XB_NT & 4) != 0>(gp + (size_t)i * 8 * ld, v[i]);
  }
  own_tile_fence();
}

__device__ __forceinline__ void gemm_k192(f32x16& acc, const unsigned char* sW, int ht, const Rows& x, const Geo& L) {
  int wbase = L.l31 * (E * 2) + ((L.g ^ L.fl) << 4) + ht * 32 * (E * 2);
  asm volatile("" : "+v"(wbase));
#pragma unroll
  for (int c = 0; c < 12; ++c) {
    Frag<bf16> fb, fx;
    fb.v = *reinterpret_cast<const bf16x8*>(sW + ((wbase ^ ((c % 4) << 5)) + 128 * (c / 4)));
    fx.v = as_bf16x8(x.v[c]);
    mma(acc, fb, fx);
  }
}

template <int DEPTH>
__device__ __forceinline__ void gemm_k192x2(f32x16& a0, f32x16& a1, const unsigned char* sW, const Rows& x, const Geo& L) {
  int wb0 = L.l31 * (E * 2) + ((L.g ^ L.fl) << 4);
  asm volatile("" : "+v"(wb0));
  const int wb1 = wb0 + 32 * (E * 2);
  Frag<bf16> fb[24];
#pragma unroll
  for (int i = 0; i < 24; ++i) {
    const int c = i >> 1;
    fb[i].v = *reinterpret_cast<const bf16x8*>(sW + ((((i & 1) ? wb1 : wb0) ^ ((c % 4) << 5)) + 128 * (c / 4)));
  }
#pragma unroll
  for (int i = 0; i < 24; ++i) {
    Frag<bf16> fx;
    fx.v = as_bf16x8(x.v[i >> 1]);
    mma((i & 1) ? a1 : a0, fb[i], fx);
  }
  __builtin_amdgcn_sched_group_barrier(0x100, DEPTH, 0);
#pragma unroll
  for (int i = 0; i < 24 - DEPTH; ++i) {
    __builtin_amdgcn_sched_group_barrier(0x008, 1, 0);
    __builtin_amdgcn_sched_group_barrier(0x100, 1, 0);
  }
#pragma unroll
  for (int i = 0; i < DEPTH; ++i) __builtin_amdgcn_sched_group_barrier(0x008, 1, 0);
  __builtin_amdgcn_sched_barrier(0);
}
__device__ __forceinline__ void tiles_write(const u32x4 (&v)[NTILE][4], bf16* __restrict__ g0, size_t ld, int lane) {
  const int rl = lane >> 3, seg = lane & 7;
#pragma unroll
  for (int wv = 0; wv < NTILE; ++wv)
#pragma unroll
    for (int i = 0; i < 4; ++i) {
      const int row = wv * 32 + i * 8 + rl;
      if (row < NTOK) gstore<(XB_NT & 2) != 0>(g0 + (size_t)row * ld + seg * 8, v[wv][i]);
    }
}

#ifdef CHAINB_PROF
__device__ unsigned long long g_chainb_prof[8 * 8 * 128];
#define CP_(i)                                                                                          \
  do {                                                                                                  \
    if (ib == CHAINB_PROF_BLK && blockIdx.x < 8) {                                                      \
      const unsigned long long t_ = __builtin_amdgcn_s_memtime();                                       \
      if ((threadIdx.x & 63) == 0) g_chainb_prof[(blockIdx.x * 8 + (threadIdx.x >> 6)) * 128 + (i)] = t_; \
    }                                                                                                   \
  } while (0)
#ifndef CHAINB_PROF_BLK
#define CHAINB_PROF_BLK 6
#endif
#else
#define CP_(i) do {} while (0)
#endif
#define BAR(s) do { CP_(2 * (s)); wg_barrier(); CP_(2 * (s) + 1); } while (0)
constexpr int B_M0 = 0;
constexpr int B_E2 = 12;
constexpr int B_P = 19;
constexpr int B_A = 24;
constexpr int B_X = 37;
constexpr int B_E1 = 46;
constexpr int B_END = 53;

__device__ __forceinline__ void ln_bwd_request(LnBwd& lnb, const bf16* X, const float* mean, const float* rstd, const bf16* R, int img,
                                               int w) {
  const int tid = w * 64 + lane_id_here();
  lnb.request_x(X, E, mean, rstd, img * NTOK, NTOK, tid);
  lnb.request_res(R, E, img * NTOK, NTOK, tid);
}
template <int B0>
__device__ __forceinline__ void ln_bwd_epilogue(unsigned char* smem, const f32x16 (&acc)[6], const bf16* X, const float* mean,
                                                const float* rstd, const bf16* R, const float* gamma, bf16* DX,
                                                float* part, int img, int w, int ib) {
  const int lane_ = lane_id_here();
  const int tid = w * 64 + lane_, rloc = w * 32 + (lane_ & 31), g = lane_ >> 5;
  LnBwd lnb;
  lnb.request_x(X, E, mean, rstd, img * NTOK, NTOK, tid);
  lnb.request_res(R, E, img * NTOK, NTOK, tid);
  wait_lds();
  BAR(B0);
  bf16* Cs = reinterpret_cast<bf16*>(smem);
#pragma unroll
  for (int b = 0; b < 6; ++b)
#pragma unroll
    for (int q = 0; q < 4; ++q) {
      const int nl = 32 * b + 8 * q + 4 * g;
      const f32x4 v = {acc[b][4 * q + 0], acc[b][4 * q + 1], acc[b][4 * q + 2], acc[b][4 * q + 3]};
      store4<bf16>(Cs + rloc * CP + nl, v);
    }
  wait_lds();
  BAR(B0 + 1);
  lnb.run<true>(Cs, CP, DX, E, gamma, true, part, img, reinterpret_cast<float*>(smem + RED_OFF), img * NTOK, NTOK, tid, Cs,
          [&](int k) { if (k == 0) BAR(B0 + 2); else if (k == 1) BAR(B0 + 3); else if (k == 2) BAR(B0 + 4); else BAR(B0 + 5); });
  wait_lds();
  BAR(B0 + 6);
}
__device__ __forceinline__ void read_own_rows(const unsigned char* smem, int w, Rows& x) {
  const int lane_ = lane_id_here();
  const unsigned char* rp = smem + (w * 32 + (lane_ & 31)) * (CP * 2) + 16 * (lane_ >> 5);
#pragma unroll
  for (int c = 0; c < 12; ++c) {
    const u32x2 lo = *reinterpret_cast<const u32x2*>(rp + 32 * c), hi = *reinterpret_cast<const u32x2*>(rp + 32 * c + 8);
    x.v[c] = u32x4{lo[0], lo[1], hi[0], hi[1]};
  }
}

__global__ __launch_bounds__(NTHREADS) void vit_chain_bwd_kernel(BwdArgs p) {
  extern __shared__ __attribute__((aligned(16))) unsigned char smem[];
  const int img = blockIdx.x;
  if (img >= p.nimg) return;
  const int w = __builtin_amdgcn_readfirstlane(threadIdx.x >> 6);
  const int depth = p.depth;

  if (w == NCW) {
#ifdef X_DMAPRIO
    __builtin_amdgcn_s_setprio(X_DMAPRIO);
#endif
    const int lane = threadIdx.x & 63;
    for (int ib = depth - 1; ib >= 0; --ib) {
      const BwdBlk& b = p.blk[ib];
      const unsigned char* wimg = reinterpret_cast<const unsigned char*>(b.wimg);
      dma_linear<48>(wimg, smem, lane);
      for (int c = 0; c < NCHUNK; ++c) {
        wait_vm<0>();
        BAR(B_M0 + c);
        if (c + 1 < NCHUNK) dma_linear<48>(wimg + (size_t)(c + 1) * STAGE, smem + ((c + 1) & 1) * STAGE, lane);
      }
      BAR(B_E2);
      dma_linear<24>(wimg + (size_t)NCHUNK * STAGE, smem + P_SLOT0, lane);
#pragma unroll
      for (int k = 1; k < 7; ++k) BAR(B_E2 + k);
      const bf16* qkv0 = b.qkv + (size_t)img * NTOK * LDQ;
      const bf16* do0 = p.dattn + (size_t)img * NTOK * INNER;
      bf16* dq0 = b.dqkv + (size_t)img * NTOK * LDQ;
      const unsigned char* stg0 = smem + A_STG;
      auto issue_kv = [&](int h) {
        dma_matrix_all<A_AUX>(qkv0 + INNER + h * HD, LDQ, NTOK, smem + A_K, lane);
        dma_matrix_all<A_AUX>(qkv0 + 2 * INNER + h * HD, LDQ, NTOK, smem + A_V, lane);
      };
      auto issue_q = [&](int h) { dma_matrix_all<A_AUX>(qkv0 + h * HD, LDQ, NTOK, smem + A_Q, lane); };
      auto issue_g = [&](int h) { dma_matrix_all<A_AUX>(do0 + h * HD, INNER, NTOK, smem + A_G, lane); };
      const unsigned char* xw = wimg + (size_t)NCHUNK * STAGE + 3 * SLOT;
      auto issue_xt = [&](int j) { dma_row_tiles(dq0 + j * 64, LDQ, smem + X_TILES + (j % 3) * X_TSET, lane); };
      wait_vm<0>();
      BAR(B_P);
      BAR(B_P + 1);
      dma_linear<24>(wimg + (size_t)NCHUNK * STAGE + SLOT, smem + P_SLOT1, lane);
      issue_kv(0);
      wait_vm<56>(); BAR(B_P + 2);
      dma_linear<24>(wimg + (size_t)NCHUNK * STAGE + 2 * SLOT, smem + P_SLOT0, lane);
      wait_vm<0>(); BAR(B_P + 3);
      issue_q(0);
      BAR(B_P + 4);
      {
        issue_g(0);
        wait_vm<0>();
        BAR(B_A);
        for (int h = 0; h < HEADS; ++h) {
          bf16* g0 = dq0 + h * HD;
          wait_vm<0>();
          BAR(B_A + 1 + 4 * h);
          u32x4 tq[NTILE][4];
          tiles_read<true>(stg0, NTOK, lane, tq);
          wait_lds();
          BAR(B_A + 2 + 4 * h);
          tiles_write(tq, g0, LDQ, lane);
          if (h + 1 < HEADS) issue_kv(h + 1);
          else {
            dma_linear<24>(xw, smem + X_SLOT0, lane);
            dma_linear<24>(xw + SLOT, smem + X_SLOT1, lane);
          }
          wait_vm<0>();
          BAR(B_A + 3 + 4 * h);
          tiles_read<true>(stg0, NTOK, lane, tq);
          wait_lds();
          BAR(B_A + 4 + 4 * h);
          tiles_write(tq, g0 + INNER, LDQ, lane);
          tiles_read<false>(smem + A_G, NTOK, lane, tq);
          wait_lds();
          if (h + 1 < HEADS) {
            issue_q(h + 1);
            issue_g(h + 1);
          } else {
            issue_xt(0);
          }
          tiles_write(tq, g0 + 2 * INNER, LDQ, lane);
        }
      }
      for (int j = 0; j < 9; ++j) {
        if (j == 0) wait_vm<28>();
        else if (j + 1 < 9) wait_vm<52>();
        else wait_vm<0>();
        BAR(B_X + j);
        if (j == 0) {
          issue_xt(1);
          dma_linear<24>(xw + 2 * SLOT, smem + X_SLOT2, lane);
          issue_xt(2);
        }
        if (j + 2 < 9 && j >= 1) {
          dma_linear<24>(xw + (size_t)(j + 2) * SLOT, smem + ((j + 2) % 3 == 0 ? X_SLOT0 : ((j + 2) % 3 == 1 ? X_SLOT1 : X_SLOT2)), lane);
          issue_xt(j + 2);
        }
      }
#pragma unroll
      for (int k = 0; k < 7; ++k) BAR(B_E1 + k);
      BAR(B_END);
    }
    return;
  }

#if defined(X_PRIO) && X_PRIO == 1
  if (w >= 4) __builtin_amdgcn_s_setprio(1);
#elif defined(X_PRIO) && X_PRIO == 2
  if (w < 4) __builtin_amdgcn_s_setprio(1);
#endif
  const int row0 = 32 * w;
  const int live = NTOK - row0 < 32 ? NTOK - row0 : 32;
  const size_t grow0 = (size_t)img * NTOK + row0;
  const float LOG2E = 1.4426950408889634f;
  const float c2 = p.scale * LOG2E;

  Rows dyf;
  {
    const int lane_ = lane_id_here();
    const int rloc = row0 + (lane_ & 31), tok = rloc < NTOK ? rloc : NTOK - 1;
    const bf16* yrow = p.blk[depth - 1].dy + ((size_t)img * NTOK + tok) * E + 8 * (lane_ >> 5);
#pragma unroll
    for (int c = 0; c < 12; ++c) dyf.v[c] = *reinterpret_cast<const u32x4*>(yrow + 16 * c);
  }

  for (int ib = depth - 1; ib >= 0; --ib) {
    const BwdBlk& b = p.blk[ib];
    f32x16 acc2[6];
#pragma unroll
    for (int bt = 0; bt < 6; ++bt)
#pragma unroll
      for (int r = 0; r < 16; ++r) acc2[bt][r] = 0.f;
    {
      const Geo L = fresh_geo();
      const int fl = L.fl;
      const int woff0 = L.l31 * (E * 2) + ((L.g ^ fl) << 4);
      const unsigned stg = (unsigned)(M_STG + w * 2 * TILE);
      bf16x8 gpraw[4];
      auto load_gp = [&](int chunk) {
        const int ln = lane_id_here();
#pragma unroll
        for (int i = 0; i < 4; ++i) {
          const int idx = ln + 64 * i, row = idx >> 3, vec = idx & 7;
          int rr = row0 + row;
          rr = rr < NTOK ? rr : NTOK - 1;
          const bf16x8* gsrc = reinterpret_cast<const bf16x8*>(b.gp + ((size_t)img * NTOK + rr) * HID + chunk * CH + vec * 8);
          gpraw[i] = (XB_NTLD & 1) ? __builtin_nontemporal_load(gsrc) : *gsrc;
        }
      };
      load_gp(0);
      for (int chunk = 0; chunk < NCHUNK; ++chunk) {
        {
          const int ln = lane_id_here();
#pragma unroll
          for (int i = 0; i < 4; ++i) {
            const int idx = ln + 64 * i, row = idx >> 3, vec = idx & 7;
            *reinterpret_cast<bf16x8*>(smem + stg + row * ROWB + ((vec ^ (row & 7)) << 4)) = gpraw[i];
          }
        }
        if (chunk + 1 < NCHUNK) load_gp(chunk + 1);
        wait_lds();
        BAR(B_M0 + chunk);
        const unsigned st_off = (unsigned)((chunk & 1) * STAGE);
        const unsigned char* sW1 = smem + st_off;
        const unsigned w2o = opaque(st_off + (unsigned)(SLOT + L.l31 * ROWB + ((L.g ^ fl) << 4)));
        const unsigned two = opaque(stg + (unsigned)(L.l31 * ROWB + ((L.g ^ (L.l31 & 7)) << 4)));
#pragma unroll
        for (int ht = 0; ht < 2; ++ht) {
          f32x16 a1;
#pragma unroll
          for (int r = 0; r < 16; ++r) a1[r] = 0.f;
          int wbase = woff0 + ht * 32 * (E * 2);
          asm volatile("" : "+v"(wbase));
#ifdef X_NOPIPE
#pragma unroll
          for (int c = 0; c < 12; ++c) {
            Frag<bf16> fb, fx;
            fb.v = *reinterpret_cast<const bf16x8*>(sW1 + ((wbase ^ ((c % 4) << 5)) + 128 * (c / 4)));
            fx.v = as_bf16x8(dyf.v[c]);
            mma(a1, fb, fx);
          }
#else
          {
            Frag<bf16> fb[12];
#pragma unroll
            for (int c = 0; c < 12; ++c)
              fb[c].v = *reinterpret_cast<const bf16x8*>(sW1 + ((wbase ^ ((c % 4) << 5)) + 128 * (c / 4)));
#pragma unroll
            for (int c = 0; c < 12; ++c) {
              Frag<bf16> fx;
              fx.v = as_bf16x8(dyf.v[c]);
              mma(a1, fb[c], fx);
            }
            __builtin_amdgcn_sched_group_barrier(0x100, PIPE_M1, 0);
#pragma unroll
            for (int i = 0; i < 12 - PIPE_M1; ++i) {
              __builtin_amdgcn_sched_group_barrier(0x008, 1, 0);
              __builtin_amdgcn_sched_group_barrier(0x100, 1, 0);
            }
#pragma unroll
            for (int i = 0; i < PIPE_M1; ++i) __builtin_amdgcn_sched_group_barrier(0x008, 1, 0);
            __builtin_amdgcn_sched_barrier(0);
          }
          Frag<bf16> fw2[12];
#pragma unroll
          for (int bt = 0; bt < 6; ++bt)
            fw2[bt].v = *reinterpret_cast<const bf16x8*>(smem + (w2o ^ (unsigned)((2 * ht) << 5)) + bt * 32 * ROWB);
          __builtin_amdgcn_sched_barrier(0);
#endif
          Frag<bf16> pg[2];
#pragma unroll
          for (int hs = 0; hs < 2; ++hs) {
            const unsigned to = two ^ (unsigned)((2 * ht + hs) << 5);
            const bf16x8 gpv = *reinterpret_cast<const bf16x8*>(smem + to);
            bf16x8 dv;
#pragma unroll
            for (int j = 0; j < 8; ++j) dv[j] = (bf16)((float)(bf16)a1[8 * hs + j] * (float)gpv[j]);
            pg[hs].v = dv;
            *reinterpret_cast<bf16x8*>(smem + to + TILE) = dv;
          }
#ifdef X_NOPIPE
#pragma unroll
          for (int hs = 0; hs < 2; ++hs) {
            const int s = 2 * ht + hs;
            Frag<bf16> fw[6];
#pragma unroll
            for (int bt = 0; bt < 6; ++bt)
              fw[bt].v = *reinterpret_cast<const bf16x8*>(smem + (w2o ^ (unsigned)(s << 5)) + bt * 32 * ROWB);
#pragma unroll
            for (int bt = 0; bt < 6; ++bt) mma(acc2[bt], fw[bt], pg[hs]);
          }
#else
          __builtin_amdgcn_sched_barrier(0);
#pragma unroll
          for (int bt = 0; bt < 6; ++bt)
            fw2[6 + bt].v = *reinterpret_cast<const bf16x8*>(smem + (w2o ^ (unsigned)((2 * ht + 1) << 5)) + bt * 32 * ROWB);
#pragma unroll
          for (int bt = 0; bt < 6; ++bt) mma(acc2[bt], fw2[bt], pg[0]);
#pragma unroll
          for (int bt = 0; bt < 6; ++bt) mma(acc2[bt], fw2[6 + bt], pg[1]);
#pragma unroll
          for (int i = 0; i < 6; ++i) {
            __builtin_amdgcn_sched_group_barrier(0x008, 1, 0);
            __builtin_amdgcn_sched_group_barrier(0x100, 1, 0);
          }
          __builtin_amdgcn_sched_group_barrier(0x008, 6, 0);
          __builtin_amdgcn_sched_barrier(0);
#endif
        }
        own_tile_fence();
        const int ln = lane_id_here();
        bf16x8 dv0[4];
#pragma unroll
        for (int i = 0; i < 4; ++i) {
          const int idx = ln + 64 * i, row = idx >> 3, vec = idx & 7;
          dv0[i] = *reinterpret_cast<const bf16x8*>(smem + stg + TILE + row * ROWB + ((vec ^ (row & 7)) << 4));
        }
        if (live == 32) {
#pragma unroll
          for (int i = 0; i < 4; ++i) {
            const int idx = ln + 64 * i, row = idx >> 3, vec = idx & 7;
            gstore<(XB_NT & 1) != 0>(b.du + (grow0 + row) * HID + chunk * CH + vec * 8, dv0[i]);
          }
        } else {
#pragma unroll
          for (int i = 0; i < 4; ++i) {
            const int idx = ln + 64 * i, row = idx >> 3, vec = idx & 7;
            if (row < live) gstore<(XB_NT & 1) != 0>(b.du + (grow0 + row) * HID + chunk * CH + vec * 8, dv0[i]);
          }
        }
      }
// ... 130 lines not shown
#pragma unroll
            for (int r = 0; r < 16; ++r) dq[dt][r] = 0.f;
          unsigned rb = rb0, tr = L.tr0;
          asm volatile("" : "+v"(rb), "+v"(tr));
          const unsigned kt = (unsigned)A_K + tr;
          TileLoop<NTILE>::run([&](auto tc) {
            constexpr int t = decltype(tc)::value;
            f32x16 sa, da;
#pragma unroll
            for (int r = 0; r < 16; ++r) { sa[r] = 0.f; da[r] = 0.f; }
            row_pair_mma<XB_ROWPIPE != 0>(sa, da, Ks, Vs, rb, t, qf, gf);
            float ds[16];
#pragma unroll
            for (int r = 0; r < 16; ++r) {
              const float pr = __builtin_amdgcn_exp2f(fmaf(sa[r], c2, -lq2));
              ds[r] = pr * (da[r] - Dq);
            }
            if (t * 32 + 32 > NTOK) {
#pragma unroll
              for (int r = 0; r < 16; ++r)
                if (t * 32 + acc_row(r, L.lane) >= NTOK) ds[r] = 0.f;
            }
            Frag<bf16> kk[4];
            tfrag4<t>(kt, kk);
            Frag<bf16> sf = pfrag<bf16>(ds, 0);
            mma(dq[0], kk[0], sf);
            mma(dq[1], kk[1], sf);
            sf = pfrag<bf16>(ds, 1);
            mma(dq[0], kk[2], sf);
            mma(dq[1], kk[3], sf);
          });
          tile_park_private(stg, dq, p.scale, L);
#pragma unroll
          for (int c = 0; c < 4; ++c) {
            kf[c] = rowfrag_x(Ks, rb, w, c);
            vf[c] = rowfrag_x(Vs, rb, w, c);
          }
        }
        wait_lds();
        BAR(B_A + 1 + 4 * h);
        BAR(B_A + 2 + 4 * h);
        {
          f32x16 dk[2], dv[2];
#pragma unroll
          for (int dt = 0; dt < 2; ++dt)
#pragma unroll
            for (int r = 0; r < 16; ++r) { dk[dt][r] = 0.f; dv[dt][r] = 0.f; }
          unsigned rb = rb0, tr = L.tr0;
          asm volatile("" : "+v"(rb), "+v"(tr));
          const unsigned qt_ = (unsigned)A_Q + tr, gt_ = (unsigned)A_G + tr;
          TileLoop<NTILE>::run([&](auto tc) {
            constexpr int t = decltype(tc)::value;
            f32x16 sa, da;
#pragma unroll
            for (int r = 0; r < 16; ++r) { sa[r] = 0.f; da[r] = 0.f; }
            row_pair_mma<XB_ROWPIPE != 0>(sa, da, Qs, Gs, rb, t, kf, vf);
            float pp[16], ds[16];
#pragma unroll
            for (int q4 = 0; q4 < 4; ++q4) {
              const f32x4 l4 = *reinterpret_cast<const f32x4*>(L2_s + t * 32 + 8 * q4 + 4 * L.g);
              const f32x4 d4 = *reinterpret_cast<const f32x4*>(D_s + t * 32 + 8 * q4 + 4 * L.g);
#pragma unroll
              for (int e = 0; e < 4; ++e) {
                const int r = 4 * q4 + e;
                const float pr = __builtin_amdgcn_exp2f(fmaf(sa[r], c2, -l4[e]));
                pp[r] = pr;
                ds[r] = pr * (da[r] - d4[e]);
              }
            }
            if (t * 32 + 32 > NTOK) {
#pragma unroll
              for (int r = 0; r < 16; ++r)
                if (t * 32 + acc_row(r, L.lane) >= NTOK) { pp[r] = 0.f; ds[r] = 0.f; }
            }
            Frag<bf16> gg[4];
            tfrag4<t>(gt_, gg);
            Frag<bf16> f = pfrag<bf16>(pp, 0);
            mma(dv[0], gg[0], f);
            mma(dv[1], gg[1], f);
            f = pfrag<bf16>(pp, 1);
            mma(dv[0], gg[2], f);
            mma(dv[1], gg[3], f);
            tfrag4<t>(qt_, gg);
            f = pfrag<bf16>(ds, 0);
            mma(dk[0], gg[0], f);
            mma(dk[1], gg[1], f);
            f = pfrag<bf16>(ds, 1);
            mma(dk[0], gg[2], f);
            mma(dk[1], gg[3], f);
          });
          if (more) load_own_g(h + 1);
          tile_park_private(stg, dk, p.scale, L);
          if (more) load_own_q(h + 1);
          wait_lds();
          BAR(B_A + 3 + 4 * h);
          tile_park_rows(Gs, w, dv, 1.0f);
        }
        if (more) load_own_o(h + 1);
        wait_lds();
        BAR(B_A + 4 + 4 * h);
      }
    }
    f32x16 accx[6];
#pragma unroll
    for (int bt = 0; bt < 6; ++bt)
#pragma unroll
      for (int r = 0; r < 16; ++r) accx[bt][r] = 0.f;
    for (int j = 0; j < 9; ++j) {
      BAR(B_X + j);
      const Geo L = fresh_geo();
      const int fl = L.fl;
      const int set = j % 3;
      const unsigned wo = opaque((unsigned)((set == 0 ? X_SLOT0 : (set == 1 ? X_SLOT1 : X_SLOT2)) + L.l31 * ROWB + ((L.g ^ fl) << 4)));
      const unsigned to = opaque((unsigned)(X_TILES + set * X_TSET + w * TILE + L.l31 * ROWB + ((L.g ^ (L.l31 & 7)) << 4)));
#pragma unroll
      for (int s = 0; s < 4; ++s) {
        Frag<bf16> fx, fw[6];
        fx.v = *reinterpret_cast<const bf16x8*>(smem + (to ^ (unsigned)(s << 5)));
#pragma unroll
        for (int bt = 0; bt < 6; ++bt)
          fw[bt].v = *reinterpret_cast<const bf16x8*>(smem + (wo ^ (unsigned)(s << 5)) + bt * 32 * ROWB);
#pragma unroll
        for (int bt = 0; bt < 6; ++bt) mma(accx[bt], fw[bt], fx);
      }
#ifndef X_NOPIPE
      __builtin_amdgcn_sched_group_barrier(0x100, PIPE_X, 0);
#pragma unroll
      for (int i = 0; i < 24; ++i) {
        __builtin_amdgcn_sched_group_barrier(0x008, 1, 0);
        if (i < 28 - PIPE_X) __builtin_amdgcn_sched_group_barrier(0x100, 1, 0);
      }
      __builtin_amdgcn_sched_barrier(0);
#endif
    }
    ln_bwd_epilogue<B_E1>(smem, accx, b.x_in, b.mean1, b.rstd1, b.dx_mid, b.ln1_g, b.dx, b.part1, img, w, ib);
    read_own_rows(smem, w, dyf);
    wait_lds();
    BAR(B_END);
  }
}

}

#ifdef CHAINB_PROF
extern "C" int rgbnm_chainb_prof_read(unsigned long long* host_out) {
  return hipMemcpyFromSymbol(host_out, HIP_SYMBOL(g_chainb_prof), sizeof(unsigned long long) * 8 * 8 * 128) == hipSuccess ? 0 : -1;
}
#endif

extern "C" {

size_t rgbnm_chain_bwd_block_bytes(void) { return sizeof(BwdBlk); }

int rgbnm_vit_chain_bwd(const rgbnm_vit_cfg* c, const rgbnm_chain_bwd_block* blocks, int depth, void* dattn, void* stream) {
  if (!c || !blocks || !dattn || depth <= 0) return RGBNM_EINVAL;
  if (c->dtype != RGBNM_DT_BF16 || c->E != E || c->heads != HEADS || c->N != NTOK || c->B < 1 || depth > MAX_DEPTH) return 1;
  BwdArgs p;
  memcpy(p.blk, blocks, sizeof(BwdBlk) * depth);
  p.dattn = (bf16*)dattn; p.depth = depth; p.nimg = c->B; p.scale = c->attn_scale;
  static DevOnce attr;
  if (attr.need()) {
    if (hipFuncSetAttribute((const void*)vit_chain_bwd_kernel, hipFuncAttributeMaxDynamicSharedMemorySize, SMEM) != hipSuccess)
      return RGBNM_ELAUNCH;
    attr.done();
  }
  const double tok = (double)c->B * NTOK;
  const double flops = depth * tok * 2.0 * (2.0 * E * HID + INNER * E + 3.0 * INNER * E + 4.0 * NTOK * INNER);
  const double bytes = depth * (tok * ((2.0 * HID + 5.0 * E + 2.0 * 3.0 * INNER) * 2.0 + 4 * 4 + HEADS * 4) + 36.0 * SLOT) + tok * E * 2.0;
  const int slot = rgbnm_trace_begin(TR_CHAIN_BWD, flops, bytes, (hipStream_t)stream);
  hipLaunchKernelGGL(vit_chain_bwd_kernel, dim3(c->B), dim3(NTHREADS), SMEM, (hipStream_t)stream, p);
  rgbnm_trace_end(slot, (hipStream_t)stream);
  LAUNCH_CHECK();
  return RGBNM_OK;
}

}
```

### rgb-no-more_amd/lib.py

```python
import ctypes as C
import os

import torch

HERE = os.path.dirname(os.path.abspath(__file__))
LIB_PATH = os.path.join(HERE, "librgbnm.so")

DT_F32, DT_BF16, DT_F16 = 0, 1, 2
EPI_NONE, EPI_RES, EPI_GELU, EPI_POS, EPI_DGELU, EPI_TANH, EPI_DTANH = range(7)
EPI_RES_DROP, EPI_GELU_DROP = 7, 8

_vp, _i, _f, _sz, _ll = C.c_void_p, C.c_int, C.c_float, C.c_size_t, C.c_longlong
HOST_WAIT = {"sec": 0.0}


class LinearDesc(C.Structure):
    _fields_ = [("w_off", _ll), ("b_off", _ll), ("ws_off", _ll), ("wst_off", _ll), ("bperm_off", _ll),
                ("N", _i), ("K", _i), ("perm_heads", _i), ("add_identity", _i), ("ldn", _i), ("pair", _i),
                ("chain_kind", _i), ("chain_off", _ll), ("bias_mode", _i), ("_pad2", _i), ("b2_off", _ll)]


class VitCfg(C.Structure):
    _fields_ = [("dtype", _i), ("B", _i), ("N", _i), ("E", _i), ("heads", _i), ("ln_eps", _f), ("attn_scale", _f)]


class BlockParams(C.Structure):
    _fields_ = [(n, _vp) for n in ("ln1_g", "ln1_b", "ln2_g", "ln2_b", "bqkv_perm", "bproj", "b1", "b2",
                                   "wqkv", "wqkv_t", "wproj", "wproj_t", "w1", "w1_t", "w2", "w2_t")]


class BlockActs(C.Structure):
    _fields_ = [(n, _vp) for n in ("x_in", "xn1", "mean1", "rstd1", "qkv", "lse", "attn", "x_mid", "xn2", "mean2",
                                   "rstd2", "u", "gl", "x_out")]


class BlockGrads(C.Structure):
    _fields_ = [(n, _vp) for n in ("dln1_g", "dln1_b", "dln2_g", "dln2_b", "dwqkv", "dbqkv", "dwproj", "dbproj",
                                   "dw1", "db1", "dw2", "db2")]


class BlockScratch(C.Structure):
    _fields_ = [("du", _vp), ("dxn", _vp), ("dx_mid", _vp), ("dattn", _vp), ("dqkv", _vp), ("ws", _vp),
                ("ws_bytes", _sz)]


class Dropout(C.Structure):
    _fields_ = [("seed", _vp), ("p", _f), ("block", _i), ("dy_m", _vp), ("dxmid_m", _vp)]


class HeadParams(C.Structure):
    _fields_ = [(n, _vp) for n in ("ln_g", "ln_b", "b1", "b2", "w1", "w1_t", "w2", "w2_t")] + \
               [("n_classes", _i), ("_pad", _i)]


class HeadActs(C.Structure):
    _fields_ = [(n, _vp) for n in ("x", "mean", "rstd", "pooled", "h1", "logits")]


class HeadGrads(C.Structure):
    _fields_ = [(n, _vp) for n in ("dln_g", "dln_b", "dw1", "db1", "dw2", "db2")]


class CpbBlock(C.Structure):
    _fields_ = [(n, _vp) for n in ("w1", "b1", "w2", "ls", "bias", "scale", "dbias", "dscale", "dw1", "db1", "dw2", "dls")] + \
               [("heads", _i), ("_pad", _i)]


class ChainBlock(C.Structure):
    _fields_ = [(n, _vp) for n in ("wimg", "ln1_g", "ln1_b", "ln2_g", "ln2_b", "bqkv_perm", "bproj", "b1", "b2", "xn1", "mean1",
                                   "rstd1", "qkv", "lse", "attn", "x_mid", "xn2", "mean2", "rstd2", "u", "gl", "x_out")]


class ChainBwdBlock(C.Structure):
    _fields_ = [(n, _vp) for n in ("wimg", "ln1_g", "ln2_g", "x_in", "mean1", "rstd1", "qkv", "lse", "attn", "x_mid", "mean2",
                                   "rstd2", "u", "dy", "du", "dx_mid", "dqkv", "dx", "part2", "part1")]


ABI_VERSION = 3

_P = C.POINTER
PROTOTYPES = {
    "rgbnm_abi_version": (_i, []),
    "rgbnm_strerror": (C.c_char_p, [_i]),
    "rgbnm_set_option": (_i, [C.c_char_p, _i]),
    "rgbnm_gemm_tn_group_begin": (None, []),
    "rgbnm_gemm_tn_group_begin_n": (None, [_i]),
    "rgbnm_gemm_tn_group_begin_id": (None, [_i, C.c_ulonglong]),
    "rgbnm_gemm_tn_group_abort": (None, [C.c_ulonglong]),
    "rgbnm_gemm_tn_group_end": (_i, [_vp]),
    "rgbnm_get_option": (_i, [C.c_char_p]),
    "rgbnm_trace_collect": (_i, [_i, _vp, _vp, _vp, _vp]),
    "rgbnm_trace_reserve": (_i, [_i]),
    "rgbnm_gemm_nt": (_i, [_i, _i, _vp, _i, _vp, _i, _vp, _i, _vp, _vp, _i, _vp, _i, _vp, _i, _i, _i, _i, _i, _vp]),
    "rgbnm_gemm_nt_drop": (_i, [_i, _i, _vp, _i, _vp, _i, _vp, _i, _vp, _vp, _i, _vp, _i, _vp, _i, _i, _i, _i, _i, _vp, _f, _i,
                                _i, _vp]),
    "rgbnm_dropout_apply": (_i, [_i, _vp, _f, _i, _i, _vp, _i, _vp, _i, _i, _i, _vp]),
    "rgbnm_gemm_tn_workspace": (_sz, [_i, _i, _i]),
    "rgbnm_gemm_tn_workspace_splits": (_sz, [_i, _i, _i]),
    "rgbnm_gemm_tn": (_i, [_i, _vp, _i, _vp, _i, _vp, _vp, _i, _i, _i, _i, _i, _vp, _sz, _vp]),
    "rgbnm_prep_weights": (_i, [_i, _vp, _i, _vp, _vp, _vp, _vp]),
    "rgbnm_prep_weights_chain": (_i, [_i, _vp, _i, _vp, _vp, _vp, _vp, _vp, _i, _vp]),
    "rgbnm_layernorm_fwd": (_i, [_i, _vp, _vp, _vp, _vp, _vp, _vp, _i, _i, _f, _vp]),
    "rgbnm_layernorm_bwd_workspace": (_sz, [_i, _i]),
    "rgbnm_layernorm_bwd": (_i, [_i, _vp, _vp, _vp, _vp, _vp, _vp, _vp, _vp, _vp, _i, _i, _i, _vp, _sz, _vp]),
    "rgbnm_head_pool_fwd": (_i, [_i, _vp, _vp, _vp, _vp, _vp, _vp, _i, _i, _i, _f, _vp]),
    "rgbnm_head_pool_bwd": (_i, [_i, _vp, _vp, _vp, _vp, _vp, _vp, _vp, _vp, _i, _i, _i, _i, _vp, _sz, _vp]),
    "rgbnm_attention_fwd": (_i, [_i, _vp, _vp, _vp, _i, _i, _i, _f, _vp]),
    "rgbnm_attention_bwd": (_i, [_i, _vp, _vp, _vp, _vp, _vp, _i, _i, _i, _f, _vp]),
    "rgbnm_subblock_embed": (_i, [_i, _i, _vp, _vp, _vp, _vp, _i, _i, _i, _i, _vp]),
    "rgbnm_subblock_embed_mix": (_i, [_i, _i, _vp, _vp, _vp, _vp, _vp, _i, _i, _i, _i, _vp]),
    "rgbnm_dct_augment_workspace": (_sz, [_i]),
    "rgbnm_dct_augment": (_i, [_vp, _vp, _vp, _vp, _vp, _vp, _vp, _vp, _vp, _i, _i, _i, _i, _i, _i, _i, _i, _vp, _sz,
                               _vp]),
    "rgbnm_dct_augment_workspace_ex": (_sz, [_i, _i]),
    "rgbnm_dct_augment_ex": (_i, [_vp, _vp, _vp, _vp, _vp, _vp, _vp, _vp, _vp, _i, _i, _i, _i, _i, _i, _i, _i, _i, _vp,
                                  _sz, _vp]),
    "rgbnm_dct_augment_packed": (_i, [_vp, _vp, _vp, _vp, _vp, _vp, _vp, _vp, _vp, _vp, _vp, _i, _i, _i, _i, _i, _i, _i, _i,
                                      _i, _vp, _sz, _vp]),
    "rgbnm_softxent": (_i, [_i, _vp, _vp, _vp, _vp, _vp, _vp, _i, _i, _f, _vp]),
    "rgbnm_softxent_loss": (_i, [_vp, _vp, _vp, _vp, _vp, _vp, _vp, _i, _i, _vp]),
    "rgbnm_softxent_grad": (_i, [_i, _vp, _vp, _vp, _vp, _vp, _vp, _i, _i, _f, _vp]),
    "rgbnm_softxent_loss_mix": (_i, [_vp, _vp, _vp, _vp, _vp, _vp, _vp, _i, _i, _vp]),
    "rgbnm_softxent_grad_mix": (_i, [_i, _vp, _vp, _vp, _vp, _vp, _vp, _i, _i, _f, _vp]),
    "rgbnm_mixup": (_i, [_i, _i, _vp, _vp, _vp, _i, _ll, _vp]),
    "rgbnm_mixup_target": (_i, [_vp, _vp, _vp, _i, _i, _vp]),
    "rgbnm_clip_adamw_wd_workspace": (_sz, []),
    "rgbnm_clip_adamw_wd_step": (_i, [_vp, _vp, _vp, _vp, _vp, _ll, _f, _f, _f, _f, _i, _f, _f, _vp, _vp, _sz, _vp]),
    "rgbnm_vit_workspace": (_sz, [_P(VitCfg)]),
    "rgbnm_vit_workspace_ex": (_sz, [_P(VitCfg), _i]),
    "rgbnm_head_bwd_workspace": (_sz, [_vp, _i]),
    "rgbnm_gelu_table_init": (_i, [_vp]),
    "rgbnm_gelu_table_info": (_i, [_vp, _vp]),
    "rgbnm_reduce_hold_begin": (_i, []),
    "rgbnm_reduce_hold_end": (_i, [_vp, _vp, _sz, _vp]),
    "rgbnm_reduce_hold_cancel": (None, []),
    "rgbnm_reduce_hold_table_bytes": (_sz, []),
    "rgbnm_vit_block_fwd": (_i, [_P(VitCfg), _P(BlockParams), _P(BlockActs), _vp]),
    "rgbnm_vit_ln_chain": (_i, [_P(VitCfg)]),
    "rgbnm_swin_embed": (_i, [_i, _i, _vp, _vp, _vp, _vp, _vp, _i, _i, _i, _vp]),
    "rgbnm_ln_generic_fwd": (_i, [_i, _vp, _vp, _vp, _vp, _vp, _i, _vp, _vp, _vp, _i, _i, _f, _vp]),
    "rgbnm_ln_generic_bwd_workspace": (_sz, [_i, _i]),
    "rgbnm_ln_generic_bwd": (_i, [_i, _vp, _vp, _vp, _vp, _vp, _vp, _i, _vp, _vp, _vp, _i, _i, _i, _vp, _sz, _vp]),
    "rgbnm_window_attention_fwd": (_i, [_i, _vp, _vp, _vp, _vp, _vp, _i, _i, _i, _i, _i, _vp]),
    "rgbnm_window_attention_bwd_workspace": (_sz, [_i, _i, _i]),
    "rgbnm_window_attention_bwd": (_i, [_i, _vp, _vp, _vp, _vp, _vp, _vp, _vp, _vp, _vp, _vp, _i, _i, _i, _i, _i, _vp, _sz, _vp]),
    "rgbnm_swin_cpb_table_elems": (_sz, [_i]),
    "rgbnm_swin_cpb_fwd": (_i, [_vp, _i, _vp, _vp, _vp, _vp]),
    "rgbnm_swin_cpb_bwd": (_i, [_vp, _i, _vp, _vp, _vp, _vp, _vp]),
    "rgbnm_merge_gather": (_i, [_i, _vp, _vp, _i, _i, _i, _i, _vp]),
    "rgbnm_token_mean": (_i, [_i, _vp, _vp, _i, _i, _i, _i, _vp]),
    "rgbnm_calib_mfma_bf16": (_i, [_i, _i, _vp, _vp]),
    "rgbnm_calib_stream": (_i, [_vp, _vp, _sz, _i, _i, _vp, _vp]),
    "rgbnm_calib_vmem_issue": (_i, [_i, _i, _i, _vp, _sz, _i, _vp, _vp]),
    "rgbnm_calib_l2": (_i, [_vp, _sz, _i, _i, _i, _i, _vp, _vp]),
    "rgbnm_calib_pipes": (_i, [_vp, _i, _i, _i, _vp, _vp, _vp]),
    "rgbnm_calib_occupy": (_i, [_vp, _sz, _i, _i, C.c_longlong, _i, _vp, _vp, _vp]),
    "rgbnm_calib_occupy_log": (_i, [_vp, _sz, _i, _i, C.c_longlong, _i, _vp, _vp, _vp, _vp]),
    "rgbnm_chain_block_bytes": (_sz, []),
    "rgbnm_chain_image_elems": (_ll, []),
    "rgbnm_chain_gather": (_i, [_vp, _vp, _vp, _ll, _vp]),
    "rgbnm_vit_chain_fwd": (_i, [_P(VitCfg), _P(ChainBlock), _i, _vp, _vp]),
    "rgbnm_chain_bwd_block_bytes": (_sz, []),
    "rgbnm_vit_chain_bwd": (_i, [_P(VitCfg), _P(ChainBwdBlock), _i, _vp, _vp]),
    "rgbnm_vit_block_bwd_dw": (_i, [_P(VitCfg), _P(BlockActs), _P(BlockGrads), _P(BlockScratch), _vp, _vp, _vp, _vp]),
    "rgbnm_vit_blocks_bwd_dw": (_i, [_P(VitCfg), _i, _vp, _vp, _vp, _vp, _vp, _vp, _vp]),
    "rgbnm_vit_blocks_bwd_dw_pe": (_i, [_P(VitCfg), _i, _vp, _vp, _vp, _vp, _vp, _vp, _vp, _vp, _vp, _vp, _vp, _sz, _vp]),
    "rgbnm_vit_block_fwd_chain": (_i, [_P(VitCfg), _P(BlockParams), _P(BlockActs), _i, _P(BlockParams), _P(BlockActs), _vp]),
    "rgbnm_vit_block_bwd": (_i, [_P(VitCfg), _P(BlockParams), _P(BlockActs), _P(BlockGrads), _P(BlockScratch), _vp,
                                 _vp, _vp]),
    "rgbnm_vit_block_fwd_drop": (_i, [_P(VitCfg), _P(BlockParams), _P(BlockActs), _P(Dropout), _vp]),
    "rgbnm_vit_block_bwd_drop": (_i, [_P(VitCfg), _P(BlockParams), _P(BlockActs), _P(BlockGrads), _P(BlockScratch), _P(Dropout),
                                      _vp, _vp, _vp]),
    "rgbnm_patch_embed_fwd": (_i, [_P(VitCfg), _i, _vp, _vp, _vp, _vp, _vp, _vp, _vp, _vp, _i, _i, _vp]),
    "rgbnm_patch_embed_fwd_mix": (_i, [_P(VitCfg), _i, _vp, _vp, _vp, _vp, _vp, _vp, _vp, _vp, _vp, _i, _i, _vp]),
    "rgbnm_patch_embed_bwd": (_i, [_P(VitCfg), _vp, _vp, _vp, _vp, _vp, _sz, _vp]),
    "rgbnm_head_fwd": (_i, [_P(VitCfg), _P(HeadParams), _P(HeadActs), _vp]),
    "rgbnm_head_bwd": (_i, [_P(VitCfg), _P(HeadParams), _P(HeadActs), _P(HeadGrads), _vp, _vp, _vp, _vp, _vp, _sz,
                            _vp]),
}

_lib = None


class RgbnmError(RuntimeError):
    pass


def lib():
    global _lib
    if _lib is None:
        if not os.path.exists(LIB_PATH):
            raise RgbnmError(f"HIP extension missing: {LIB_PATH} (run `python -c 'import __graft_entry__ as g; g.build()'`). "
                             "There is no CPU fallback.")
        L = C.CDLL(LIB_PATH)
        for name, (res, args) in PROTOTYPES.items():
            fn = getattr(L, name)
            fn.restype = res
            fn.argtypes = args
        if L.rgbnm_abi_version() != ABI_VERSION:
            raise RgbnmError(f"{LIB_PATH} has ABI version {L.rgbnm_abi_version()}, this binding expects {ABI_VERSION}: rebuild "
                             "(python rgb-no-more_amd/build.py)")
        if L.rgbnm_chain_block_bytes() != C.sizeof(ChainBlock) or L.rgbnm_chain_bwd_block_bytes() != C.sizeof(ChainBwdBlock):
            raise RgbnmError("rgbnm_chain_block layout mismatch between librgbnm.so and lib.py")
        _lib = L
    return _lib


def source_hash():
    import hashlib
    h = hashlib.sha256()
    csrc = os.path.join(HERE, "csrc")
    files = sorted(os.path.join(csrc, f) for f in os.listdir(csrc) if f.endswith((".hip", ".inc", ".h", ".c")))
    files.append(os.path.join(os.path.dirname(HERE), "include", "rgbnm.h"))
    for f in files:
        h.update(os.path.basename(f).encode())
        with open(f, "rb") as fh:
            h.update(fh.read())
    return h.hexdigest()[:16]


def check(rc, what=""):
    if rc != 0:
        msg = lib().rgbnm_strerror(rc).decode()
        raise RgbnmError(f"{what}: rgbnm error {rc}: {msg}")


def dt_of(t):
    if t == torch.float32:
        return DT_F32
    if t == torch.bfloat16:
        return DT_BF16
    if t == torch.float16:
        return DT_F16
    raise TypeError(f"unsupported dtype {t} (float32, bfloat16 or float16)")


def ptr(t):
    return None if t is None else t.data_ptr()


_raw_stream = getattr(torch._C, "_cuda_getCurrentRawStream", None)


def stream():
    if _raw_stream is not None:
        return _raw_stream(torch.cuda.current_device())
    return torch.cuda.current_stream().cuda_stream


def require_cuda(*tensors):
    for t in tensors:
        if t is not None and not t.is_cuda:
            raise RgbnmError("rgb-no-more_amd kernels need device (HIP) tensors; there is no CPU fallback")
        if t is not None and not t.is_contiguous():
            raise RgbnmError("tensor must be contiguous")
```

### rgb-no-more_amd/plainvit.py

```python
import ctypes as C
import numpy as np
import math
import threading
import warnings
from collections import OrderedDict

import torch
from torch import nn

from . import dct_ops as dops
from . import lib as L
from .cls_transforms import LazyMixed
from .flatparams import FlatParamModule, align as _align


class ResidualAdd(nn.Module):
    def __init__(self, fn):
        super().__init__()
        self.fn = fn


class MultiHeadAttention(nn.Module):
    def __init__(self, emb_size, num_heads, head_size, input_embed=-1, device="cpu", dtype=torch.float32):
        super().__init__()
# ... 247 lines not shown
                                         a.feat.data_ptr(), a.cfg.B, Hb, Wb, 0, L.stream()), "subblock_embed")
        g, gp = a.pe_g, a.pe_gp
        L.check(lib.rgbnm_gemm_nt(dt, L.EPI_GELU, a.feat.data_ptr(), 384, m._sh_ptr("peY", "ws"), 256, g.data_ptr(), E,
                                  by.data_ptr(), None, 0, gp.data_ptr(), E, None, 0, M, Ey, 256, 0, L.stream()), "pe2 Y")
        L.check(lib.rgbnm_gemm_nt(dt, L.EPI_GELU, a.feat.data_ptr() + 256 * es, 384, m._sh_ptr("peC", "ws"), 128,
                                  g.data_ptr() + Ey * es, E, bc.data_ptr(), None, 0, gp.data_ptr() + Ey * es, E, None,
                                  0, M, E - Ey, 128, 0, L.stream()), "pe2 C")
        L.check(lib.rgbnm_gemm_nt(dt, L.EPI_POS, g.data_ptr(), E, m._sh_ptr("peM", "ws"), E, a.xbuf(0).data_ptr(), E,
                                  bm.data_ptr(), None, 0, None, 0, m._pos.data_ptr(), a.cfg.N, M, E, E, 0, L.stream()),
                "pe2 mix")
        ctx.st = st
        return a.xbuf(0).detach()

    @staticmethod
    def backward(ctx, dx0):
        st = ctx.st
        st.end_hold()
        m, a = st.model, st.arena
        lib, dt, M, E = L.lib(), a.cfg.dtype, a.cfg.B * a.cfg.N, a.cfg.E
        Ey = E // 6 * 4
        dx0 = dx0.contiguous()
        es = a.feat.element_size()
        gr = [m._gview(st.gbuf, n) for n in _PE2_NAMES]
        ws, wsb = a.ws.data_ptr(), a.ws_bytes
        L.check(lib.rgbnm_gemm_tn(dt, dx0.data_ptr(), E, a.pe_g.data_ptr(), E, gr[4].data_ptr(), gr[5].data_ptr(), M, E,
                                  E, 0, 0, ws, wsb, L.stream()), "pe2 dWm")
        dh = a.pe_dh
        L.check(lib.rgbnm_gemm_nt(dt, L.EPI_DGELU, dx0.data_ptr(), E, m._sh_ptr("peM", "wst"), E, dh.data_ptr(), E,
                                  None, a.pe_gp.data_ptr(), E, None, 0, None, 0, M, E, E, 0, L.stream()), "pe2 dh")
        L.check(lib.rgbnm_gemm_tn(dt, dh.data_ptr(), E, a.feat.data_ptr(), 384, gr[0].data_ptr(), gr[1].data_ptr(), M, Ey,
                                  256, 0, 0, ws, wsb, L.stream()), "pe2 dWy")
        L.check(lib.rgbnm_gemm_tn(dt, dh.data_ptr() + Ey * es, E, a.feat.data_ptr() + 256 * es, 384, gr[2].data_ptr(),
                                  gr[3].data_ptr(), M, E - Ey, 128, 0, 0, ws, wsb, L.stream()), "pe2 dWc")
        if m._grad_sync is not None:
            m._grad_sync.ready(st.gbuf, _PE2_NAMES, last=True)
        return (None, None, None) + tuple(gr)


_PES_NAMES = ([f"patchembed.LinearY.{i}.{k}" for i in range(4) for k in ("weight", "bias")] +
              [f"patchembed.LinearC.{i}.{k}" for i in range(2) for k in ("weight", "bias")] +
              ["patchembed.LinearMix.weight", "patchembed.LinearMix.bias"])


class _PatchEmbedSepFn(torch.autograd.Function):

    @staticmethod
    def forward(ctx, y, cbcr, st, *params):
        m, a = st.model, st.arena
        lib, dt, M, E = L.lib(), a.cfg.dtype, a.cfg.B * a.cfg.N, a.cfg.E
        Hb, Wb = y.shape[2], y.shape[3]
        if (Hb // 2) * (Wb // 2) != a.cfg.N:
            raise ValueError("expected a 28 x 28 block grid")
        L.check(lib.rgbnm_subblock_embed(L.dt_of(y.dtype), dt, y.data_ptr(), cbcr.data_ptr(), m._eye16.data_ptr(),
                                         a.feat.data_ptr(), a.cfg.B, Hb, Wb, 0, L.stream()), "subblock_embed")
        wbd, bcat = m._sep_operands(a.cdtype)
        g, gp = a.pe_g, a.pe_gp
        L.check(lib.rgbnm_gemm_nt(dt, L.EPI_GELU, a.feat.data_ptr(), 384, wbd.data_ptr(), 384, g.data_ptr(), E,
                                  bcat.data_ptr(), None, 0, gp.data_ptr(), E, None, 0, M, E, 384, 0, L.stream()), "pe-sep blocks")
        bm = m._named["patchembed.LinearMix.bias"]
        L.check(lib.rgbnm_gemm_nt(dt, L.EPI_POS, g.data_ptr(), E, m._sh_ptr("peMix", "ws"), E, a.xbuf(0).data_ptr(), E,
                                  bm.data_ptr(), None, 0, None, 0, m._pos.data_ptr(), a.cfg.N, M, E, E, 0, L.stream()),
                "pe-sep mix")
        ctx.st = st
        return a.xbuf(0).detach()

    @staticmethod
    def backward(ctx, dx0):
        st = ctx.st
        st.end_hold()
        m, a = st.model, st.arena
        lib, dt, M, E = L.lib(), a.cfg.dtype, a.cfg.B * a.cfg.N, a.cfg.E
        dx0 = dx0.contiguous()
        gr = [m._gview(st.gbuf, n) for n in _PES_NAMES]
        ws, wsb = a.ws.data_ptr(), a.ws_bytes
        L.check(lib.rgbnm_gemm_tn(dt, dx0.data_ptr(), E, a.pe_g.data_ptr(), E, gr[12].data_ptr(), gr[13].data_ptr(), M, E,
                                  E, 0, 0, ws, wsb, L.stream()), "pe-sep dWmix")
        dh = a.pe_dh
        L.check(lib.rgbnm_gemm_nt(dt, L.EPI_DGELU, dx0.data_ptr(), E, m._sh_ptr("peMix", "wst"), E, dh.data_ptr(), E,
                                  None, a.pe_gp.data_ptr(), E, None, 0, None, 0, M, E, E, 0, L.stream()), "pe-sep dh")
        dwbd = torch.empty(E, 384, device=dx0.device, dtype=torch.float32)
        dbcat = torch.empty(E, device=dx0.device, dtype=torch.float32)
        L.check(lib.rgbnm_gemm_tn(dt, dh.data_ptr(), E, a.feat.data_ptr(), 384, dwbd.data_ptr(), dbcat.data_ptr(), M, E,
                                  384, 0, 0, ws, wsb, L.stream()), "pe-sep dWbd")
        e6 = E // 6
        for i in range(6):
            gr[2 * i].copy_(dwbd[i * e6:(i + 1) * e6].index_select(1, m._sep_cols[i]))
            gr[2 * i + 1].copy_(dbcat[i * e6:(i + 1) * e6])
        if m._grad_sync is not None:
            m._grad_sync.ready(st.gbuf, _PES_NAMES, last=True)
        return (None, None, None) + tuple(gr)


_PE3_NAMES = ["patchembed.projectionY.1.weight", "patchembed.projectionY.1.bias", "patchembed.projectionC.1.weight",
              "patchembed.projectionC.1.bias"]


class _PatchEmbedConcatFn(torch.autograd.Function):

    @staticmethod
    def forward(ctx, y, cbcr, st, wy, by, wc, bc):
        m, a = st.model, st.arena
        lib, dt, E, B = L.lib(), a.cfg.dtype, a.cfg.E, a.cfg.B
        if y.shape[2:4] != (28, 28) or cbcr.shape[2:4] != (14, 14):
            raise ValueError("expected a 28 x 28 luma / 14 x 14 chroma block grid")
        idt = L.dt_of(y.dtype)
        zc = m._zero_chroma(2 * B, y.dtype)
        L.check(lib.rgbnm_subblock_embed(idt, dt, y.data_ptr(), cbcr.data_ptr(), m._conv16.data_ptr(), a.feat.data_ptr(),
                                         B, 28, 28, 0, L.stream()), "subblock_embed Y")
        L.check(lib.rgbnm_subblock_embed(idt, dt, cbcr.data_ptr(), zc.data_ptr(), m._conv16.data_ptr(), a.featC.data_ptr(),
                                         2 * B, 14, 14, 0, L.stream()), "subblock_embed C")
        L.check(lib.rgbnm_gemm_nt(dt, L.EPI_POS, a.feat.data_ptr(), 384, m._sh_ptr("peY3", "ws"), 256, a.pe_ty.data_ptr(), E,
                                  by.data_ptr(), None, 0, None, 0, m._pos.data_ptr(), 196, B * 196, E, 256, 0, L.stream()),
                "pe3 Y")
        L.check(lib.rgbnm_gemm_nt(dt, L.EPI_POS, a.featC.data_ptr(), 384, m._sh_ptr("peC3", "ws"), 256, a.pe_tc.data_ptr(), E,
                                  bc.data_ptr(), None, 0, None, 0, m._pos7.data_ptr(), 49, B * 98, E, 256, 0, L.stream()),
                "pe3 C")
        x0 = a.xbuf(0).view(B, 294, E)
        x0[:, :196].copy_(a.pe_ty.view(B, 196, E))
        x0[:, 196:].copy_(a.pe_tc.view(B, 98, E))
        ctx.st = st
        return a.xbuf(0).detach()

    @staticmethod
    def backward(ctx, dx0):
        st = ctx.st
        st.end_hold()
        m, a = st.model, st.arena
        lib, dt, E, B = L.lib(), a.cfg.dtype, a.cfg.E, a.cfg.B
        dxv = dx0.contiguous().view(B, 294, E)
        dty = dxv[:, :196].contiguous()
        dtc = dxv[:, 196:].contiguous()
        gr = [m._gview(st.gbuf, n) for n in _PE3_NAMES]
        ws, wsb = a.ws.data_ptr(), a.ws_bytes
        L.check(lib.rgbnm_gemm_tn(dt, dty.data_ptr(), E, a.feat.data_ptr(), 384, gr[0].data_ptr(), gr[1].data_ptr(),
                                  B * 196, E, 256, 0, 0, ws, wsb, L.stream()), "pe3 dWy")
        L.check(lib.rgbnm_gemm_tn(dt, dtc.data_ptr(), E, a.featC.data_ptr(), 384, gr[2].data_ptr(), gr[3].data_ptr(),
                                  B * 98, E, 256, 0, 0, ws, wsb, L.stream()), "pe3 dWc")
        if m._grad_sync is not None:
            m._grad_sync.ready(st.gbuf, _PE3_NAMES, last=True)
        return (None, None, None) + tuple(gr)


class _BlockFn(torch.autograd.Function):
    @staticmethod
    def forward(ctx, x, st, idx, *params):
        m, a = st.model, st.arena
        assert x.data_ptr() == a.xbuf(idx).data_ptr()
        if st.drop is not None:
            L.check(L.lib().rgbnm_vit_block_fwd_drop(C.byref(a.cfg), C.byref(m._bparams[idx]), C.byref(a.acts[idx]),
                                                     C.byref(st.drop[idx]), L.stream()), "vit_block_fwd_drop")
            ctx.st, ctx.idx = st, idx
            return a.xbuf(idx + 1).detach()
        if idx == 0:
            st.chain_fwd = m._chain_forward(a)
        if st.chain_fwd:
            ctx.st, ctx.idx = st, idx
            return a.xbuf(idx + 1).detach()
        chain = st.ln_chain
        last = idx + 1 >= m.depth
        nxt_p = C.byref(m._bparams[idx + 1]) if chain and not last else None
        nxt_a = C.byref(a.acts[idx + 1]) if chain and not last else None
        L.check(L.lib().rgbnm_vit_block_fwd_chain(C.byref(a.cfg), C.byref(m._bparams[idx]), C.byref(a.acts[idx]),
                                                  1 if (chain and idx > 0) else 0, nxt_p, nxt_a, L.stream()),
                "vit_block_fwd")
        ctx.st, ctx.idx = st, idx
        return a.xbuf(idx + 1).detach()

    @staticmethod
    def backward(ctx, dy):
        st, idx = ctx.st, ctx.idx
        m, a = st.model, st.arena
        dy = dy.contiguous()
        dx = a.dx[idx & 1]
        if dx.data_ptr() == dy.data_ptr():
            dx = a.dx[(idx + 1) & 1]
        grads = [m._gview(st.gbuf, n) for n in m._block_names[idx]]
        g = L.BlockGrads(*[t.data_ptr() for t in grads])
        scratch = a.scratch_blk[idx] if st.holding else a.scratch
        if idx == m.depth - 1:
            m._check_prep_gen(st)
            st.chain_bwd = st.drop is None and m._chain_backward(a, dy)
            st.dw_pending = []
        try:
            if st.drop is not None:
                L.check(L.lib().rgbnm_vit_block_bwd_drop(C.byref(a.cfg), C.byref(m._bparams[idx]), C.byref(a.acts[idx]),
                                                         C.byref(g), C.byref(scratch), C.byref(st.drop[idx]), dy.data_ptr(),
                                                         dx.data_ptr(), L.stream()), "vit_block_bwd_drop")
            elif getattr(st, "chain_bwd", False):
                dx = a.dx_blk[idx]
                st.dw_pending.append((idx, g, dy.data_ptr()))
                if st.gbuf.data_ptr() != m._gflat.data_ptr():
                    group = 1
                elif st.holding:
                    group = m.depth
                elif m._grad_sync is not None:
                    group = m.dw_group_overlapped
                else:
                    group = 1
                if len(st.dw_pending) >= min(group, CHAIN_MAX_DEPTH) or idx == 0:
                    pend, st.dw_pending = st.dw_pending, []
                    n = len(pend)
                    scs = [L.BlockScratch(a.du_blk[i].data_ptr(), a.dxn.data_ptr(), a.dxmid_blk[i].data_ptr(), a.dattn_chain.data_ptr(),
                                          a.dqkv_blk[i].data_ptr(), a.ws_chain.data_ptr() + i * a.ws_bytes, a.ws_bytes)
                           for i, _, _ in pend]
                    pa = (C.POINTER(L.BlockActs) * n)(*[C.pointer(a.acts[i]) for i, _, _ in pend])
                    pg = (C.POINTER(L.BlockGrads) * n)(*[C.pointer(gg) for _, gg, _ in pend])
                    ps = (C.POINTER(L.BlockScratch) * n)(*[C.pointer(x) for x in scs])
                    pdy = (C.c_void_p * n)(*[d for _, _, d in pend])
                    p2 = (C.c_void_p * n)(*[a.lnpart[i, 0].data_ptr() for i, _, _ in pend])
                    p1 = (C.c_void_p * n)(*[a.lnpart[i, 1].data_ptr() for i, _, _ in pend])
                    L.check(L.lib().rgbnm_vit_blocks_bwd_dw(C.byref(a.cfg), n, pa, pg, ps, pdy, p2, p1, L.stream()), "vit_blocks_bwd_dw")
                    if m._grad_sync is not None:
                        for i, _, _ in pend[:-1]:
                            m._grad_sync.ready(st.gbuf, m._block_names[i])
                else:
                    by_name = dict(zip(m._block_names[idx], grads))
                    return (dx, None, None) + tuple(by_name[n] for n in m._block_param_order[idx])
            else:
                L.check(L.lib().rgbnm_vit_block_bwd(C.byref(a.cfg), C.byref(m._bparams[idx]), C.byref(a.acts[idx]),
                                                    C.byref(g), C.byref(scratch), dy.data_ptr(), dx.data_ptr(),
                                                    L.stream()), "vit_block_bwd")
            if m._grad_sync is not None:
                m._grad_sync.ready(st.gbuf, m._block_names[idx])
        except BaseException:
            st.cancel_hold()
            raise
        by_name = dict(zip(m._block_names[idx], grads))
        return (dx, None, None) + tuple(by_name[n] for n in m._block_param_order[idx])


class _EncoderFn(torch.autograd.Function):

    @staticmethod
    def forward(ctx, x, st, *params):
        m, a = st.model, st.arena
        assert x.data_ptr() == a.xbuf(0).data_ptr()
        st.chain_fwd = m._chain_forward(a)
        if not st.chain_fwd:
            chain = st.ln_chain
            for idx in range(m.depth):
                last = idx + 1 >= m.depth
                nxt_p = C.byref(m._bparams[idx + 1]) if chain and not last else None
                nxt_a = C.byref(a.acts[idx + 1]) if chain and not last else None
                L.check(L.lib().rgbnm_vit_block_fwd_chain(C.byref(a.cfg), C.byref(m._bparams[idx]), C.byref(a.acts[idx]),
                                                          1 if (chain and idx > 0) else 0, nxt_p, nxt_a, L.stream()), "vit_block_fwd")
        ctx.st = st
        return a.xbuf(m.depth).detach()

    @staticmethod
    def backward(ctx, dy):
        st = ctx.st
        m, a = st.model, st.arena
        D = m.depth
        dy = dy.contiguous()
        grads = [[m._gview(st.gbuf, n) for n in m._block_names[i]] for i in range(D)]
        gs = [L.BlockGrads(*[t.data_ptr() for t in grads[i]]) for i in range(D)]
        m._check_prep_gen(st)
        try:
            if m._chain_backward(a, dy):
                group = D if (m._grad_sync is None or st.holding) else m.dw_group_overlapped
                group = min(group, CHAIN_MAX_DEPTH)
                idx = D - 1
                while idx >= 0:
                    pend = list(range(idx, max(idx - group, -1), -1))
                    n = len(pend)
                    scs = [L.BlockScratch(a.du_blk[i].data_ptr(), a.dxn.data_ptr(), a.dxmid_blk[i].data_ptr(), a.dattn_chain.data_ptr(),
                                          a.dqkv_blk[i].data_ptr(), a.ws_chain.data_ptr() + i * a.ws_bytes, a.ws_bytes) for i in pend]
                    pa = (C.POINTER(L.BlockActs) * n)(*[C.pointer(a.acts[i]) for i in pend])
                    pg = (C.POINTER(L.BlockGrads) * n)(*[C.pointer(gs[i]) for i in pend])
                    ps = (C.POINTER(L.BlockScratch) * n)(*[C.pointer(x) for x in scs])
                    pdy = (C.c_void_p * n)(*[dy.data_ptr() if i == D - 1 else a.dx_blk[i + 1].data_ptr() for i in pend])
                    p2 = (C.c_void_p * n)(*[a.lnpart[i, 0].data_ptr() for i in pend])
                    p1 = (C.c_void_p * n)(*[a.lnpart[i, 1].data_ptr() for i in pend])
                    pe = None
                    if (pend[-1] == 0 and n == D and m.embed_kind == "group" and getattr(st, "pe_feat_ok", False)
                            and all(p.requires_grad for p in m._pe_params_list())):
                        pe = (m._gview(st.gbuf, "patchembed.projection.0.weight"), m._gview(st.gbuf, "patchembed.projection.0.bias"))
                    if pe is None:
                        L.check(L.lib().rgbnm_vit_blocks_bwd_dw(C.byref(a.cfg), n, pa, pg, ps, pdy, p2, p1, L.stream()), "vit_blocks_bwd_dw")
                    else:
                        L.check(L.lib().rgbnm_vit_blocks_bwd_dw_pe(C.byref(a.cfg), n, pa, pg, ps, pdy, p2, p1, a.dx_blk[0].data_ptr(),
                                                                   a.feat.data_ptr(), pe[0].data_ptr(), pe[1].data_ptr(),
                                                                   a.ws.data_ptr(), a.ws_bytes, L.stream()), "vit_blocks_bwd_dw_pe")
                        st.pe_done = a.dx_blk[0].data_ptr()
                    if m._grad_sync is not None:
                        for i in pend:
                            m._grad_sync.ready(st.gbuf, m._block_names[i])
                    idx -= n
                dx = a.dx_blk[0]
            else:
                cur = dy
                for idx in range(D - 1, -1, -1):
                    dx = a.dx[idx & 1]
                    if dx.data_ptr() == cur.data_ptr():
                        dx = a.dx[(idx + 1) & 1]
                    scratch = a.scratch_blk[idx] if st.holding else a.scratch
                    L.check(L.lib().rgbnm_vit_block_bwd(C.byref(a.cfg), C.byref(m._bparams[idx]), C.byref(a.acts[idx]),
                                                        C.byref(gs[idx]), C.byref(scratch), cur.data_ptr(), dx.data_ptr(),
                                                        L.stream()), "vit_block_bwd")
                    if m._grad_sync is not None:
                        m._grad_sync.ready(st.gbuf, m._block_names[idx])
                    cur = dx
        except BaseException:
            st.cancel_hold()
            raise
        out = []
        for i in range(D):
            by_name = dict(zip(m._block_names[i], grads[i]))
            out += [by_name[n] for n in m._block_param_order[i]]
        return (dx, None) + tuple(out)


class _HeadFn(torch.autograd.Function):
    @staticmethod
    def forward(ctx, x, st, *params):
        m, a = st.model, st.arena
        logits = torch.empty(a.B, m._ncls_pad, device=x.device, dtype=torch.float32)
        acts = L.HeadActs(x.data_ptr(), a.hmean.data_ptr(), a.hrstd.data_ptr(), a.pooled.data_ptr(),
                          a.h1.data_ptr(), logits.data_ptr())
        L.check(L.lib().rgbnm_head_fwd(C.byref(a.cfg), C.byref(m._hparams), C.byref(acts), L.stream()), "head_fwd")
        ctx.st, ctx.acts, ctx.x = st, acts, x
        ctx.set_materialize_grads(False)
        if m._ncls_pad != m.n_classes:
            return logits[:, :m.n_classes].contiguous()
        if a.cdtype == torch.float32:
            return logits
        return logits, torch.empty(a.B, m._ncls_pad, device=x.device, dtype=a.cdtype)

    @staticmethod
    def backward(ctx, dlogits, dedge=None):
        st = ctx.st
        m, a = st.model, st.arena
        if dlogits is None and dedge is None:
            return (None,) * (2 + len(m._head_param_order))
        if dedge is not None:
            dlogits = dedge if dlogits is None else dedge + dlogits.to(dedge.dtype)
        names = m._head_names
        grads = [m._gview(st.gbuf, n) for n in names]
        padded = m._ncls_pad != m.n_classes
        if padded:
            dl = torch.zeros(a.B, m._ncls_pad, device=dlogits.device, dtype=a.cdtype)
            dl[:, :m.n_classes].copy_(dlogits)
            dw2p = torch.empty(m._ncls_pad, m.emb_size, device=dlogits.device, dtype=torch.float32)
            db2p = torch.empty(m._ncls_pad, device=dlogits.device, dtype=torch.float32)
            ptrs = [t.data_ptr() for t in grads]
            ptrs[names.index("classhead.ch_linear2.weight")] = dw2p.data_ptr()
            ptrs[names.index("classhead.ch_linear2.bias")] = db2p.data_ptr()
            g = L.HeadGrads(*ptrs)
        else:
            dl = dlogits.to(a.cdtype).contiguous()
            g = L.HeadGrads(*[t.data_ptr() for t in grads])
        dx = a.dx[0]
        if not padded:
            st.begin_hold()
        ws = a.ws_head if st.holding else a.ws
        try:
            L.check(L.lib().rgbnm_head_bwd(C.byref(a.cfg), C.byref(m._hparams), C.byref(ctx.acts), C.byref(g),
                                           dl.data_ptr(), a.da.data_ptr(), a.dpooled.data_ptr(), dx.data_ptr(),
                                           ws.data_ptr(), ws.numel(), L.stream()), "head_bwd")
            if padded:
                grads[names.index("classhead.ch_linear2.weight")].copy_(dw2p[:m.n_classes])
                grads[names.index("classhead.ch_linear2.bias")].copy_(db2p[:m.n_classes])
            if m._grad_sync is not None:
                m._grad_sync.ready(st.gbuf, names)
        except BaseException:
            st.cancel_hold()
            raise
        if padded:
            st.begin_hold()
        by_name = dict(zip(names, grads))
        return (dx, None) + tuple(by_name[n] for n in m._head_param_order)


class ViT(FlatParamModule):
    defer_grad_reduction = False
    dw_group_overlapped = 4
    single_encoder_node = True
    train_dropout = False
    last_dropout_seed = None

    def __init__(self, in_channels: int = 3, patch_size: int = 16, emb_size: int = 768, input_embed: int = -1,
                 depth: int = 12, n_classes: int = 1000, drop_p=0.1, pixel_space="RGB", ver=1, use_subblock=True,
                 device="cpu", dtype=torch.float32, num_heads: int = 8, head_size: int = 64, **kwargs):
        super().__init__()
        if pixel_space.lower() not in ("dct", "rgb2dct"):
            raise NotImplementedError("rgb-no-more_amd implements the --domain DCT path only")
        if ver not in (1, 2, 3):
            raise NotImplementedError("ver must be 1 (PatchEmbedding_DCT_Group), 2 (PatchEmbedding_DCT_Separate / "
                                      "_Separate_subblock) or 3 (PatchEmbedding_DCT_Concat)")
        if ver in (1, 3) and not use_subblock:
            raise NotImplementedError("embed_type 1 / 3 without sub-block conversion are not in any reference config")
        if not 0.0 <= float(drop_p) < 1.0:
            raise ValueError("dropout probability has to be in [0, 1)")
        self.drop_p = float(drop_p)
        if head_size != 64 or emb_size not in (192, 384, 512, 768, 1024) or input_embed >= 0:
            raise NotImplementedError("HIP kernels cover head_size 64 and emb_size 192 / 384 (JPEG-Ti / JPEG-S; tuned) and "
                                      "512 / 768 / 1024 (vitb / vitl of utils/configs.py:104-122; generic kernels)")
        if dtype != torch.float32:
            raise NotImplementedError("parameters are fp32 masters; choose bf16 compute with autocast")
        if n_classes < 1:
            raise ValueError("n_classes must be positive")
        self.pixel_space = pixel_space
        self.emb_size, self.depth, self.n_classes = emb_size, depth, n_classes
        self._ncls_pad = (n_classes + 7) // 8 * 8
        self.num_heads, self.inner = num_heads, num_heads * head_size
        self.n_tokens = 294 if ver == 3 else 196
        E = emb_size
        kw = dict(device=device, dtype=dtype)
        self.ver = ver
        self.embed_kind = {1: "group", 3: "concat"}.get(ver, "sep_sub" if use_subblock else "sep")
        self.patchembed = {"group": lambda: PatchEmbedding_DCT_Group(patch_size, E, use_subblock, **kw),
                           "sep_sub": lambda: PatchEmbedding_DCT_Separate_subblock(patch_size, E, **kw),
                           "sep": lambda: PatchEmbedding_DCT_Separate(patch_size, E, **kw),
                           "concat": lambda: PatchEmbedding_DCT_Concat(patch_size, E, use_subblock, **kw)}[self.embed_kind]()
        blocks = []
        for _ in range(depth):
            att = ResidualAdd(nn.Sequential(OrderedDict([
                ("eb_lrnorm1", nn.LayerNorm(E, **kw)),
                ("eb_mha", MultiHeadAttention(E, num_heads, head_size, **kw)),
                ("eb_drop1", nn.Identity())])))
            ffn = ResidualAdd(nn.Sequential(OrderedDict([
                ("eb_lrnorm2", nn.LayerNorm(E, **kw)),
                ("eb_ffb", nn.Sequential(nn.Linear(E, 4 * E, **kw), nn.Identity(), nn.Identity(),
                                         nn.Linear(4 * E, E, **kw))),
                ("eb_drop2", nn.Identity())])))
            blocks.append(nn.Sequential(att, ffn))
        self.encoder = nn.Sequential(*blocks)
        self.classhead = nn.Sequential(OrderedDict([
            ("ch_lrnorm", nn.LayerNorm(E, **kw)), ("ch_gap", nn.Identity()),
            ("ch_linear1", nn.Linear(E, E, **kw)), ("ch_tanh", nn.Identity()),
            ("ch_linear2", nn.Linear(E, n_classes, **kw))]))
        self._flat = None
        self._arenas = {}
        self.compute_dtype = None

    def _names(self):
        return [n for n, _ in self.named_parameters()]

    def _flatten(self):
        dev = next(self.parameters()).device
        if dev.type != "cuda":
            raise L.RgbnmError("model parameters must live on a HIP device (no CPU fallback)")
        params = self._pack_parameters()
        offs = self._offs
        if self.embed_kind == "group":
            lin = [("pe", "patchembed.projection.0", 0)]
        elif self.embed_kind == "sep_sub":
            lin = [("peY", "patchembed.projection_Y.1", 0), ("peC", "patchembed.projection_C.1", 0),
                   ("peM", "patchembed.linearMix", 0)]
        elif self.embed_kind == "sep":
            lin = [("peMix", "patchembed.LinearMix", 0)]
        else:
            lin = [("peY3", "patchembed.projectionY.1", 0), ("peC3", "patchembed.projectionC.1", 0)]
        for i in range(self.depth):
            lin += [(f"qkv{i}", f"encoder.{i}.0.fn.eb_mha.qkv", self.num_heads),
                    (f"proj{i}", f"encoder.{i}.0.fn.eb_mha.projection", 0),
                    (f"fc1{i}", f"encoder.{i}.1.fn.eb_ffb.0", 0), (f"fc2{i}", f"encoder.{i}.1.fn.eb_ffb.3", 0)]
        lin += [("h1", "classhead.ch_linear1", 0), ("h2", "classhead.ch_linear2", 0)]
        descs = (L.LinearDesc * len(lin))()
        self._sh_off, so, bo = {}, 0, 0
        chain_ok = self.emb_size == 192 and self.num_heads == 3 and self.n_tokens == 196
        from . import chain as _chain
        kinds = {"eb_mha.qkv": 1, "eb_mha.projection": 2, "eb_ffb.0": 3, "eb_ffb.3": 4}
        for k, (key, name, ph) in enumerate(lin):
            ck = kinds[name.split(".fn.")[1]] if chain_ok and name.startswith("encoder.") else 0
            coff = int(name.split(".")[1]) * _chain.BLOCK_ELEMS if ck else 0
            Nn, Kk = self._shapes[name + ".weight"]
            Np = self._ncls_pad if key == "h2" else Nn
            ws, wst = so, so + _align(Np * Kk)
            so = wst + _align(Np * Kk)
            bp = bo
            if ph:
                bo += _align(Nn)
            descs[k] = L.LinearDesc(offs[name + ".weight"], offs[name + ".bias"], ws, wst, bp, Nn, Kk, ph,
                                    1 if key == "peM" else 0, Np if Np != Nn else 0, 0, ck, coff)
            self._sh_off[key] = (ws, wst, bp)
        self._ndesc, self._sh_total = len(lin), so
        self._descs_dev = torch.frombuffer(bytearray(bytes(descs)), dtype=torch.uint8).to(dev)
        self._bias_perm = torch.zeros(max(bo, 1), device=dev, dtype=torch.float32)
        self._shadow = {}
        if self.embed_kind == "sep":
            self._eye16 = torch.eye(16, device=dev, dtype=torch.float32)
            p1, p2 = torch.meshgrid(torch.arange(8), torch.arange(8), indexing="ij")
            cols = [((pdh * 8 + p1) * 16 + pdw * 8 + p2).reshape(-1) for pdh in range(2) for pdw in range(2)]
            cols += [256 + torch.arange(64), 320 + torch.arange(64)]
            self._sep_cols = [c.to(dev) for c in cols]
            self._sep_cache = {}
        else:
            self._conv16 = self.patchembed.conv_Y.to(dev).contiguous()
        self._chain_idx = None
        self._chain_refused = False
        if chain_ok:
            assert _chain.BLOCK_ELEMS == L.lib().rgbnm_chain_image_elems()
            self._chain_idx = True
            self._chain_img = torch.zeros(self.depth * _chain.BLOCK_ELEMS, device=dev, dtype=torch.bfloat16)
            self._chain_img_bwd = torch.zeros(self.depth * _chain.BLOCK_ELEMS, device=dev, dtype=torch.bfloat16)
        self._pos = sincos_table(14, 14, self.emb_size, dev)
        self._pos7 = sincos_table(7, 7, self.emb_size, dev) if self.embed_kind == "concat" else None
        self._zc = {}
        self._build_names()
        self._arenas = {}
        L.check(L.lib().rgbnm_gelu_table_init(L.stream()), "gelu_table_init")

    def _zero_chroma(self, n, dtype):
        k = (n, dtype)
        if k not in self._zc:
            self._zc[k] = torch.zeros(n, 2, 7, 7, 8, 8, device=self._flat.device, dtype=dtype)
        return self._zc[k]

    def _sep_operands(self, cdtype):
        E, e6 = self.emb_size, self.emb_size // 6
        key = cdtype
        if key not in self._sep_cache:
            self._sep_cache[key] = (torch.zeros(E, 384, device=self._flat.device, dtype=cdtype),
                                    torch.zeros(E, device=self._flat.device, dtype=torch.float32))
        wbd, bcat = self._sep_cache[key]
        named = self._named
        for i in range(6):
            mod = f"patchembed.LinearY.{i}" if i < 4 else f"patchembed.LinearC.{i - 4}"
            wbd[i * e6:(i + 1) * e6].index_copy_(1, self._sep_cols[i], named[mod + ".weight"].detach().to(cdtype))
            bcat[i * e6:(i + 1) * e6].copy_(named[mod + ".bias"].detach())
        return wbd, bcat

    def _build_names(self):
        self._block_names, self._block_param_order, self._bparams_by_dtype = [], [], {}
        for i in range(self.depth):
            a, b = f"encoder.{i}.0.fn.", f"encoder.{i}.1.fn."
            self._block_names.append([a + "eb_lrnorm1.weight", a + "eb_lrnorm1.bias", b + "eb_lrnorm2.weight",
                                      b + "eb_lrnorm2.bias", a + "eb_mha.qkv.weight", a + "eb_mha.qkv.bias",
                                      a + "eb_mha.projection.weight", a + "eb_mha.projection.bias",
                                      b + "eb_ffb.0.weight", b + "eb_ffb.0.bias", b + "eb_ffb.3.weight",
                                      b + "eb_ffb.3.bias"])
            self._block_param_order.append([n for n in self._names() if n.startswith(f"encoder.{i}.")])
        self._head_names = ["classhead.ch_lrnorm.weight", "classhead.ch_lrnorm.bias", "classhead.ch_linear1.weight",
                            "classhead.ch_linear1.bias", "classhead.ch_linear2.weight", "classhead.ch_linear2.bias"]
        self._head_param_order = [n for n in self._names() if n.startswith("classhead.")]
        self._pe_names = {"group": ["patchembed.projection.0.weight", "patchembed.projection.0.bias"], "sep_sub": _PE2_NAMES,
                          "sep": _PES_NAMES, "concat": _PE3_NAMES}[self.embed_kind]

    def grad_ready_order(self):
        if not hasattr(self, "_head_names"):
            self._build_names()
        return ([(self._head_names, False)] + [(self._block_names[i], False) for i in reversed(range(self.depth))] +
                [(self._pe_names, True)])

    def _pe_params_list(self):
        pe = self.__dict__.get("_pe_params")
        if pe is None:
            pe = self.__dict__["_pe_params"] = [p for n, p in self._named.items() if n.startswith("patchembed.")]
        return pe

    def _pptr(self, name):
        return self._flat.data_ptr() + self._offs[name] * 4

    def _sh_ptr(self, key, which):
        sh = self._shadow[self._cur_dtype]
        ws, wst, _ = self._sh_off[key]
        return sh.data_ptr() + (ws if which == "ws" else wst) * sh.element_size()

    def _chain_index_tables(self):
        from . import chain as _chain
        dev = self._flat.device
        idx = np.concatenate([_chain.block_index(self._sh_off[f"qkv{i}"][0], self._sh_off[f"proj{i}"][0],
                                                 self._sh_off[f"fc1{i}"][0], self._sh_off[f"fc2{i}"][0]) for i in range(self.depth)])
        idb = np.concatenate([_chain.block_index_bwd(self._sh_off[f"qkv{i}"][1], self._sh_off[f"proj{i}"][1],
                                                     self._sh_off[f"fc1{i}"][1], self._sh_off[f"fc2{i}"][1])
                              for i in range(self.depth)])
        assert max(idx.max(), idb.max()) < 2 ** 31
        return torch.from_numpy(idx.astype(np.int32)).to(dev), torch.from_numpy(idb.astype(np.int32)).to(dev)

    def _prep(self, cdtype, chains=True):
        if cdtype not in self._shadow:
            self._shadow[cdtype] = torch.zeros(self._sh_total, device=self._flat.device, dtype=cdtype)
        self._cur_dtype = cdtype
        self._prep_gen = getattr(self, "_prep_gen", 0) + 1
        chain = chains and cdtype == torch.bfloat16 and self._chain_idx is not None
        img_f = self._chain_img.data_ptr() if chain and L.lib().rgbnm_get_option(b"fwd_chain") else None
        img_b = (self._chain_img_bwd.data_ptr() if chain and L.lib().rgbnm_get_option(b"bwd_chain") and torch.is_grad_enabled()
                 else None)
        skip = bool(img_f and (img_b or not torch.is_grad_enabled()) and not self._chain_refused)
        L.check(L.lib().rgbnm_prep_weights_chain(L.dt_of(cdtype), self._descs_dev.data_ptr(), self._ndesc, self._flat.data_ptr(),
                                                 self._shadow[cdtype].data_ptr(), self._bias_perm.data_ptr(), img_f, img_b,
                                                 1 if skip else 0, L.stream()), "prep_weights")
        if cdtype not in self._bparams_by_dtype:
            bps = []
            for i in range(self.depth):
                a, b = f"encoder.{i}.0.fn.", f"encoder.{i}.1.fn."
                bps.append(L.BlockParams(
                    self._pptr(a + "eb_lrnorm1.weight"), self._pptr(a + "eb_lrnorm1.bias"),
                    self._pptr(b + "eb_lrnorm2.weight"), self._pptr(b + "eb_lrnorm2.bias"),
                    self._bias_perm.data_ptr() + self._sh_off[f"qkv{i}"][2] * 4,
                    self._pptr(a + "eb_mha.projection.bias"), self._pptr(b + "eb_ffb.0.bias"),
                    self._pptr(b + "eb_ffb.3.bias"),
                    self._sh_ptr(f"qkv{i}", "ws"), self._sh_ptr(f"qkv{i}", "wst"),
                    self._sh_ptr(f"proj{i}", "ws"), self._sh_ptr(f"proj{i}", "wst"),
                    self._sh_ptr(f"fc1{i}", "ws"), self._sh_ptr(f"fc1{i}", "wst"),
                    self._sh_ptr(f"fc2{i}", "ws"), self._sh_ptr(f"fc2{i}", "wst")))
            if self._ncls_pad != self.n_classes and getattr(self, "_b2pad", None) is None:
                self._b2pad = torch.zeros(self._ncls_pad, device=self._flat.device, dtype=torch.float32)
            b2 = self._b2pad.data_ptr() if self._ncls_pad != self.n_classes else self._pptr("classhead.ch_linear2.bias")
            hp = L.HeadParams(self._pptr("classhead.ch_lrnorm.weight"), self._pptr("classhead.ch_lrnorm.bias"),
                              self._pptr("classhead.ch_linear1.bias"), b2,
                              self._sh_ptr("h1", "ws"), self._sh_ptr("h1", "wst"), self._sh_ptr("h2", "ws"),
                              self._sh_ptr("h2", "wst"), self._ncls_pad, 0)
            self._bparams_by_dtype[cdtype] = (bps, hp)
        self._bparams, self._hparams = self._bparams_by_dtype[cdtype]
        if self._ncls_pad != self.n_classes:
            self._b2pad[:self.n_classes].copy_(self._named["classhead.ch_linear2.bias"].detach())

    def _check_prep_gen(self, st):
        if getattr(st, "prep_gen", None) != getattr(self, "_prep_gen", None) and not getattr(self, "_warned_prep_gen", False):
            self._warned_prep_gen = True
            warnings.warn("rgb-no-more_amd: another forward of this model ran between a forward and its backward; the backward uses the "
                          "weight operands of the LATEST forward (identical unless the parameters changed in between)", RuntimeWarning,
                          stacklevel=3)

    def _warn_chain_refused(self, which):
        key = "_warned_chain_" + which
        if not getattr(self, key, False):
            setattr(self, key, True)
            warnings.warn(f"rgb-no-more_amd: the one-launch encoder {which} kernel refused this model (no GELU "
                          f"table); running the per-operation kernels (about 2x slower)", RuntimeWarning, stacklevel=3)

    def _chain_forward(self, a):
        if a.cdtype != torch.bfloat16 or self._chain_idx is None or not L.lib().rgbnm_get_option(b"fwd_chain"):
            return False
        if a.chain_table is None:
            from . import chain as _chain
            blocks = (L.ChainBlock * self.depth)()
            for i in range(self.depth):
                bp, ac = self._bparams[i], a.acts[i]
                blocks[i] = L.ChainBlock(self._chain_img.data_ptr() + i * _chain.BLOCK_ELEMS * 2,
                                         bp.ln1_g, bp.ln1_b, bp.ln2_g, bp.ln2_b, bp.bqkv_perm, bp.bproj, bp.b1, bp.b2,
                                         ac.xn1, ac.mean1, ac.rstd1, ac.qkv, ac.lse, ac.attn, ac.x_mid, ac.xn2, ac.mean2, ac.rstd2,
                                         ac.u, ac.gl, ac.x_out)
            a.chain_table = blocks
        for s0 in range(0, self.depth, CHAIN_MAX_DEPTH):
            n = min(CHAIN_MAX_DEPTH, self.depth - s0)
            sub = C.cast(C.byref(a.chain_table, s0 * C.sizeof(L.ChainBlock)), C.POINTER(L.ChainBlock))
            rc = L.lib().rgbnm_vit_chain_fwd(C.byref(a.cfg), sub, n, a.xbuf(s0).data_ptr(), L.stream())
            if rc == 1 and s0 == 0:
                self._warn_chain_refused("forward")
                if not self._chain_refused:
                    self._chain_refused = True
                    self._prep(a.cdtype)
                return False
            L.check(rc, "vit_chain_fwd")
        return True

    def _chain_backward(self, a, dy):
        if (a.cdtype != torch.bfloat16 or self._chain_idx is None or not a.need_grad
                or not L.lib().rgbnm_get_option(b"bwd_chain")):
            return False
        D, dev = self.depth, self._flat.device
        if a.chain_bwd_table is None or a.chain_bwd_dy != dy.data_ptr():
            from . import chain as _chain
            M, E, I = a.B * self.n_tokens, self.emb_size, self.inner
            if a.chain_bwd_table is None:
                e = lambda *s, dt=a.cdtype: torch.empty(*s, device=dev, dtype=dt)
                a.du_blk = [e(M, 4 * E) for _ in range(D)]
                a.dxmid_blk = [e(M, E) for _ in range(D)]
                a.dqkv_blk = [e(M, 3 * I) for _ in range(D)]
                a.dx_blk = [e(M, E) for _ in range(D)]
                a.dattn_chain = e(M, I)
                a.lnpart = torch.empty(D, 2, a.B, 2, E, device=dev, dtype=torch.float32)
                a.ws_chain = a.ws_blk if a.ws_blk is not None else torch.empty(D * a.ws_bytes, device=dev, dtype=torch.uint8)
            blocks = (L.ChainBwdBlock * D)()
            for i in range(D):
                bp, ac = self._bparams[i], a.acts[i]
                blocks[i] = L.ChainBwdBlock(
                    self._chain_img_bwd.data_ptr() + i * _chain.BLOCK_ELEMS * 2, bp.ln1_g, bp.ln2_g, ac.x_in, ac.mean1, ac.rstd1,
                    ac.qkv, ac.lse, ac.attn, ac.x_mid, ac.mean2, ac.rstd2, ac.u,
                    dy.data_ptr() if i == D - 1 else a.dx_blk[i + 1].data_ptr(),
                    a.du_blk[i].data_ptr(), a.dxmid_blk[i].data_ptr(), a.dqkv_blk[i].data_ptr(), a.dx_blk[i].data_ptr(),
                    a.lnpart[i, 0].data_ptr(), a.lnpart[i, 1].data_ptr())
            a.chain_bwd_table = blocks
            a.chain_bwd_dy = dy.data_ptr()
        starts = list(range(0, D, CHAIN_MAX_DEPTH))
        for s0 in reversed(starts):
            n = min(CHAIN_MAX_DEPTH, D - s0)
            sub = C.cast(C.byref(a.chain_bwd_table, s0 * C.sizeof(L.ChainBwdBlock)), C.POINTER(L.ChainBwdBlock))
            rc = L.lib().rgbnm_vit_chain_bwd(C.byref(a.cfg), sub, n, a.dattn_chain.data_ptr(), L.stream())
            if rc == 1 and s0 == starts[-1]:
                self._warn_chain_refused("backward")
                if not self._chain_refused:
                    self._chain_refused = True
                    self._prep(a.cdtype)
                return False
            L.check(rc, "vit_chain_bwd")
        return True

    def _acquire_arena(self, B, cdtype, need_grad):
        key = (B, cdtype, need_grad)
        pool = self._arenas.setdefault(key, [])
        return pool.pop() if pool else _Arena(self, B, cdtype, need_grad)

    def _release_arena(self, arena):
        pool = self._arenas.setdefault((arena.B, arena.cdtype, arena.need_grad), [])
        if len(pool) < 2:
            pool.append(arena)

    def forward(self, x, cbcr=None):
        if cbcr is None:
            raise ValueError("DCT path needs both Y and CbCr tensors")
        lam = None
        if isinstance(x, LazyMixed) or isinstance(cbcr, LazyMixed):
            if (isinstance(x, LazyMixed) and isinstance(cbcr, LazyMixed) and x.lam.data_ptr() == cbcr.lam.data_ptr()
                    and self.embed_kind == "group"):
                lam, x, cbcr = x.lam, x.tensor, cbcr.tensor
            else:
                x = x.materialize() if isinstance(x, LazyMixed) else x
                cbcr = cbcr.materialize() if isinstance(cbcr, LazyMixed) else cbcr
        L.require_cuda(x, cbcr)
        if x.dim() != 6 or x.shape[1:] != (1, 28, 28, 8, 8) or cbcr.shape[1:] != (2, 14, 14, 8, 8):
            raise ValueError(f"expected Y (B,1,28,28,8,8) and CbCr (B,2,14,14,8,8), got {tuple(x.shape)} {tuple(cbcr.shape)}")
        if x.dtype != cbcr.dtype:
            raise TypeError("Y and CbCr must share a dtype")
        cdtype = self.compute_dtype
        if cdtype is None:
            cdtype = torch.get_autocast_dtype("cuda") if torch.is_autocast_enabled("cuda") else torch.float32
        if cdtype not in (torch.float32, torch.bfloat16, torch.float16):
            raise NotImplementedError(f"compute dtype {cdtype}: the MI355X path implements fp32, bf16 and fp16")
        drop = bool(self.drop_p and self.training)
        if drop and not self.train_dropout:
            raise NotImplementedError("training with dropout p > 0 runs only with model.train_dropout = True (masks from this "
                                      "library's Philox stream, not torch's); model.eval() runs, where nn.Dropout is the identity")
        self._ensure_flat()
        B = x.shape[0]
        need_grad = torch.is_grad_enabled() and any(p.requires_grad for p in self._named.values())
        if need_grad and self._grad_sync is not None:
            self._grad_sync.begin_step()
        self._prep(cdtype, chains=not drop)
        arena = self._acquire_arena(B, cdtype, need_grad)
        st = _FwdState(self, arena, self._grad_buffer() if need_grad else None)
        st.prep_gen = self._prep_gen
        st.ln_chain = bool(L.lib().rgbnm_vit_ln_chain(C.byref(arena.cfg))) and not drop
        if drop:
            self._begin_dropout(st)
        named = self._named
        if self.embed_kind == "group":
            h = _PatchEmbedFn.apply(x, cbcr, st, named["patchembed.projection.0.weight"],
                                    named["patchembed.projection.0.bias"], lam)
        elif self.embed_kind == "sep_sub":
            h = _PatchEmbed2Fn.apply(x, cbcr, st, *[named[n] for n in _PE2_NAMES])
        elif self.embed_kind == "sep":
            h = _PatchEmbedSepFn.apply(x, cbcr, st, *[named[n] for n in _PES_NAMES])
        else:
            h = _PatchEmbedConcatFn.apply(x, cbcr, st, *[named[n] for n in _PE3_NAMES])
        if (not drop and self.single_encoder_node and cdtype == torch.bfloat16 and self._chain_idx is not None
                and L.lib().rgbnm_get_option(b"fwd_chain")):
            h = _EncoderFn.apply(h, st, *self._all_block_params())
        else:
            for i in range(self.depth):
                h = _BlockFn.apply(h, st, i, *[named[n] for n in self._block_param_order[i]])
        out = _HeadFn.apply(h, st, *[named[n] for n in self._head_param_order])
        if isinstance(out, tuple):
            out, edge = out
            out._rgbnm_grad_edge = edge
        return out

    def _begin_dropout(self, st):
        a = st.arena
        st.drop_seed = torch.empty(1, device=self._flat.device, dtype=torch.int64).random_(-2 ** 63, None)
        self.last_dropout_seed = st.drop_seed
        if a.need_grad and getattr(a, "drop_dy", None) is None:
            M, E = a.B * self.n_tokens, self.emb_size
            a.drop_dy = torch.empty(M, E, device=self._flat.device, dtype=a.cdtype)
            a.drop_dxmid = torch.empty(M, E, device=self._flat.device, dtype=a.cdtype)
        dy_m = a.drop_dy.data_ptr() if a.need_grad else None
        dxm_m = a.drop_dxmid.data_ptr() if a.need_grad else None
        st.drop = [L.Dropout(st.drop_seed.data_ptr(), self.drop_p, i, dy_m, dxm_m) for i in range(self.depth)]

    def _all_block_params(self):
        named = self._named
        key = id(named)
        if getattr(self, "_abp_key", None) != key:
            self._abp_key, self._abp = key, [named[n] for i in range(self.depth) for n in self._block_param_order[i]]
        return self._abp
```

Baseline: 68010.

## Fold head layernorm-mean-pool into chain forward and backward kernel ends

The one-launch encoder forward kernel gains a templated tail that computes the final layernorm stats and the token-mean pooled features in-kernel, so the head skips its separate pool kernel. The backward chain kernel likewise computes the pool/layernorm backward at its first block, so the head skips its pool-backward kernel and the extra dx round trip. This removes two launches and a full read/write of the last activation, at the cost of more register pressure, extra LDS use in the already heavy chain kernels, and a more complex host-side eligibility and fallback path.

```diff
diff --git a/include/rgbnm.h b/include/rgbnm.h
--- a/include/rgbnm.h
+++ b/include/rgbnm.h
@@ -237,6 +237,13 @@
 long long rgbnm_chain_image_elems(void);
 int rgbnm_chain_gather(const void* src, const int* idx, void* dst, long long n, void* stream);
 int rgbnm_vit_chain_fwd(const rgbnm_vit_cfg* cfg, const rgbnm_chain_block* blocks, int depth, const void* x0, void* stream);
+typedef struct rgbnm_chain_fwd_tail {
+  const float *ln_g, *ln_b;
+  float *mean, *rstd;
+  void* pooled;
+} rgbnm_chain_fwd_tail;
+int rgbnm_vit_chain_fwd_ends(const rgbnm_vit_cfg* cfg, const rgbnm_chain_block* blocks, int depth, const void* x0,
+                             const rgbnm_chain_fwd_tail* tail, void* stream);
 
 typedef struct rgbnm_chain_bwd_block {
   const void* wimg;
@@ -249,6 +256,14 @@
 } rgbnm_chain_bwd_block;
 size_t rgbnm_chain_bwd_block_bytes(void);
 int rgbnm_vit_chain_bwd(const rgbnm_vit_cfg* cfg, const rgbnm_chain_bwd_block* blocks, int depth, void* dattn, void* stream);
+typedef struct rgbnm_chain_bwd_head {
+  const void* dpooled; const void* x;
+  const float *ln_g, *mean, *rstd;
+  float* part;
+  float *dln_g, *dln_b;
+} rgbnm_chain_bwd_head;
+int rgbnm_vit_chain_bwd_ends(const rgbnm_vit_cfg* cfg, const rgbnm_chain_bwd_block* blocks, int depth, void* dattn,
+                             const rgbnm_chain_bwd_head* head, void* stream);
 int rgbnm_vit_block_bwd_dw(const rgbnm_vit_cfg* cfg, const rgbnm_block_acts* a, const rgbnm_block_grads* g,
                            const rgbnm_block_scratch* s, const void* dy, const float* part2, const float* part1, void* stream);
 int rgbnm_vit_blocks_bwd_dw(const rgbnm_vit_cfg* cfg, int n, const rgbnm_block_acts* const* a, const rgbnm_block_grads* const* g,
@@ -293,10 +308,14 @@
   float *dln_g, *dln_b, *dw1, *db1, *dw2, *db2;
 } rgbnm_head_grads;
 int rgbnm_head_fwd(const rgbnm_vit_cfg* cfg, const rgbnm_head_params* p, const rgbnm_head_acts* a, void* stream);
+int rgbnm_head_fwd_pooled(const rgbnm_vit_cfg* cfg, const rgbnm_head_params* p, const rgbnm_head_acts* a, void* stream);
 size_t rgbnm_head_bwd_workspace(const rgbnm_vit_cfg* cfg, int n_classes);
 int rgbnm_head_bwd(const rgbnm_vit_cfg* cfg, const rgbnm_head_params* p, const rgbnm_head_acts* a,
                    const rgbnm_head_grads* g, const void* dlogits, void* da, void* dpooled, void* dx, void* ws,
                    size_t ws_bytes, void* stream);
+int rgbnm_head_bwd_pooled(const rgbnm_vit_cfg* cfg, const rgbnm_head_params* p, const rgbnm_head_acts* a,
+                          const rgbnm_head_grads* g, const void* dlogits, void* da, void* dpooled, void* ws,
+                          size_t ws_bytes, void* stream);
 
 int rgbnm_swin_embed(int in_dtype, int out_dtype, const void* y, const void* cbcr, const float* convY, const float* convC,
                      void* feat, int B, int Hb, int Wb, void* stream);
diff --git a/rgb-no-more_amd/csrc/chain_ends.h b/rgb-no-more_amd/csrc/chain_ends.h
--- /dev/null
+++ b/rgb-no-more_amd/csrc/chain_ends.h
@@ -0,0 +1,20 @@
+#pragma once
+#include "common.h"
+
+namespace {
+
+__device__ __forceinline__ void token_sum96(float (&v)[96], int l31) {
+#pragma unroll
+  for (int s = 0; s < 5; ++s) {
+    const int half = 48 >> s, m = 16 >> s;
+    const bool up = (l31 & m) != 0;
+#pragma unroll
+    for (int i = 0; i < half; ++i) {
+      const float keep = up ? v[half + i] : v[i], send = up ? v[i] : v[half + i];
+      v[i] = keep + __shfl_xor(send, m, 64);
+    }
+  }
+}
+__device__ __forceinline__ int feature_of(int o, int g) { return 16 * (o >> 3) + 8 * g + (o & 7); }
+
+}
diff --git a/rgb-no-more_amd/csrc/vit.hip b/rgb-no-more_amd/csrc/vit.hip
--- a/rgb-no-more_amd/csrc/vit.hip
+++ b/rgb-no-more_amd/csrc/vit.hip
@@ -26,7 +26,7 @@
   return e;
 }
 struct Opt { const char* name; std::atomic<int> value; };
-Opt g_opts[] = {{"nt_staged", 1}, {"tn_tr", 1}, {"tn_pipe", 1}, {"attn_v2", 1}, {"nt_wres", 1}, {"nt_kpipe", 1}, {"attn_persist", 1}, {"ln_fuse", 1}, {"tn_group", 2}, {"trace", 0}, {"tn_wgs", 512}, {"mlp_fuse", 1}, {"nt_cold", 0}, {"mlp_bwd", 1}, {"nt_small", 1}, {"mlp_dmast", 1}, {"gelu_table", 1}, {"ln_rows", 1}, {"kp8", 1}, {"win_xcd", 1}, {"kp_persist", 1}, {"fwd_chain", 1}, {"bwd_chain", 1}, {"tn_direct", 1}, {"tn_pack", 1}, {"tn_wide", 1}};
+Opt g_opts[] = {{"nt_staged", 1}, {"tn_tr", 1}, {"tn_pipe", 1}, {"attn_v2", 1}, {"nt_wres", 1}, {"nt_kpipe", 1}, {"attn_persist", 1}, {"ln_fuse", 1}, {"tn_group", 2}, {"trace", 0}, {"tn_wgs", 512}, {"mlp_fuse", 1}, {"nt_cold", 0}, {"mlp_bwd", 1}, {"nt_small", 1}, {"mlp_dmast", 1}, {"gelu_table", 1}, {"ln_rows", 1}, {"kp8", 1}, {"win_xcd", 1}, {"kp_persist", 1}, {"fwd_chain", 1}, {"bwd_chain", 1}, {"tn_direct", 1}, {"tn_pack", 1}, {"tn_wide", 1}, {"fold_pool_fwd", 1}, {"fold_pool_bwd", 1}};
 }
 
 int rgbnm_trace_begin(int tag, double flops, double bytes, hipStream_t st) {
@@ -394,13 +394,20 @@
   return rgbnm_gemm_tn(c->dtype, dx0, c->E, feat, 384, dwpe, dbpe, c->B * c->N, c->E, 384, 0, 0, ws, ws_bytes, st);
 }
 
-int rgbnm_head_fwd(const rgbnm_vit_cfg* c, const rgbnm_head_params* p, const rgbnm_head_acts* a, void* st) {
+static int head_fwd(const rgbnm_vit_cfg* c, const rgbnm_head_params* p, const rgbnm_head_acts* a, bool pool, void* st) {
   if (!c || !p || !a) return RGBNM_EINVAL;
   const int dt = c->dtype, E = c->E, C = p->n_classes;
-  TRY(rgbnm_head_pool_fwd(dt, a->x, p->ln_g, p->ln_b, a->pooled, a->mean, a->rstd, c->B, c->N, E, c->ln_eps, st));
+  if (pool) TRY(rgbnm_head_pool_fwd(dt, a->x, p->ln_g, p->ln_b, a->pooled, a->mean, a->rstd, c->B, c->N, E, c->ln_eps, st));
   TRY(rgbnm_gemm_nt(dt, RGBNM_EPI_TANH, a->pooled, E, p->w1, E, a->h1, E, p->b1, 0, 0, 0, 0, 0, 0, c->B, E, E, 0, st));
   TRY(rgbnm_gemm_nt(dt, RGBNM_EPI_NONE, a->h1, E, p->w2, E, a->logits, C, p->b2, 0, 0, 0, 0, 0, 0, c->B, C, E, 1, st));
   return RGBNM_OK;
+}
+
+int rgbnm_head_fwd(const rgbnm_vit_cfg* c, const rgbnm_head_params* p, const rgbnm_head_acts* a, void* st) {
+  return head_fwd(c, p, a, true, st);
+}
+int rgbnm_head_fwd_pooled(const rgbnm_vit_cfg* c, const rgbnm_head_params* p, const rgbnm_head_acts* a, void* st) {
+  return head_fwd(c, p, a, false, st);
 }
 
 size_t rgbnm_head_bwd_workspace(const rgbnm_vit_cfg* c, int n_classes) {
@@ -409,10 +416,10 @@
          (size_t)c->B * 2 * c->E * sizeof(float);
 }
 
-int rgbnm_head_bwd(const rgbnm_vit_cfg* c, const rgbnm_head_params* p, const rgbnm_head_acts* a,
-                   const rgbnm_head_grads* g, const void* dlogits, void* da, void* dpooled, void* dx, void* ws,
-                   size_t ws_bytes, void* st) {
-  if (!c || !p || !a || !g || !dlogits || !da || !dpooled || !dx) return RGBNM_EINVAL;
+static int head_bwd(const rgbnm_vit_cfg* c, const rgbnm_head_params* p, const rgbnm_head_acts* a,
+                    const rgbnm_head_grads* g, const void* dlogits, void* da, void* dpooled, void* dx, void* ws,
+                    size_t ws_bytes, void* st) {
+  if (!c || !p || !a || !g || !dlogits || !da || !dpooled) return RGBNM_EINVAL;
   const int dt = c->dtype, E = c->E, C = p->n_classes, B = c->B;
   const size_t s1 = (rgbnm_gemm_tn_workspace(B, C, E) + 255) & ~(size_t)255, s2 = (rgbnm_gemm_tn_workspace(B, E, E) + 255) & ~(size_t)255;
   const size_t s3 = (size_t)B * 2 * E * sizeof(float);
@@ -433,8 +440,20 @@
   if (rc != RGBNM_OK) return rc;
   if (rt != RGBNM_OK) return rt;
   TRY(rgbnm_gemm_nt(dt, RGBNM_EPI_NONE, da, E, p->w1_t, E, dpooled, E, 0, 0, 0, 0, 0, 0, 0, B, E, E, 0, st));
-  TRY(rgbnm_head_pool_bwd(dt, dpooled, a->x, p->ln_g, a->mean, a->rstd, dx, g->dln_g, g->dln_b, B, c->N, E, 0, w3, b3, st));
-  return RGBNM_OK;
-}
-
-}
+  if (dx) TRY(rgbnm_head_pool_bwd(dt, dpooled, a->x, p->ln_g, a->mean, a->rstd, dx, g->dln_g, g->dln_b, B, c->N, E, 0, w3, b3, st));
+  return RGBNM_OK;
+}
+
+int rgbnm_head_bwd(const rgbnm_vit_cfg* c, const rgbnm_head_params* p, const rgbnm_head_acts* a,
+                   const rgbnm_head_grads* g, const void* dlogits, void* da, void* dpooled, void* dx, void* ws,
+                   size_t ws_bytes, void* st) {
+  if (!dx) return RGBNM_EINVAL;
+  return head_bwd(c, p, a, g, dlogits, da, dpooled, dx, ws, ws_bytes, st);
+}
+int rgbnm_head_bwd_pooled(const rgbnm_vit_cfg* c, const rgbnm_head_params* p, const rgbnm_head_acts* a,
+                          const rgbnm_head_grads* g, const void* dlogits, void* da, void* dpooled, void* ws,
+                          size_t ws_bytes, void* st) {
+  return head_bwd(c, p, a, g, dlogits, da, dpooled, nullptr, ws, ws_bytes, st);
+}
+
+}
diff --git a/rgb-no-more_amd/csrc/vit_chain.hip b/rgb-no-more_amd/csrc/vit_chain.hip
--- a/rgb-no-more_amd/csrc/vit_chain.hip
+++ b/rgb-no-more_amd/csrc/vit_chain.hip
@@ -3,6 +3,7 @@
 #include <type_traits>
 #include "internal.h"
 #include "tile128.h"
+#include "chain_ends.h"
 #include "../../include/rgbnm.h"
 
 namespace {
@@ -45,6 +46,7 @@
 static_assert(TB_OFF + 10 * STG_TILE <= SMEM, "LDS");
 static_assert(FLAG_OFF + 16 <= ST0_OFF, "LDS");
 static_assert(LN1P_OFF + 2 * E * 4 <= V_OFF, "LDS");
+static_assert(NCW * E * 4 <= 2 * ARR, "LDS");
 static_assert(TAB_LIMIT <= ST1_OFF && ST1_OFF % 128 == 0 && TA_OFF % 128 == 0, "LDS");
 
 struct ChainBlk {
@@ -63,6 +65,10 @@
   const unsigned* tab_img; int tab_pieces;
   unsigned kneg, kpos, klo, koff, ksgn;
 };
+struct ChainTail { const float *ln_g, *ln_b; float *mean, *rstd; bf16* pooled; };
+static_assert(sizeof(ChainTail) == sizeof(rgbnm_chain_fwd_tail), "rgbnm_chain_fwd_tail layout");
+struct ChainArgsEnds : ChainArgs { ChainTail tail; };
+constexpr int POOL_OFF = K_OFF;
 
 #ifndef X_STORE
 #define X_STORE 1
@@ -242,7 +248,8 @@
 #endif
 #define BAR(s) do { CP(2 * (s)); wg_barrier(); CP(2 * (s) + 1); } while (0)
 
-__global__ __launch_bounds__(NTHREADS) void vit_chain_fwd_kernel(ChainArgs p) {
+template <bool ENDS>
+__global__ __launch_bounds__(NTHREADS) void vit_chain_fwd_kernel(std::conditional_t<ENDS, ChainArgsEnds, ChainArgs> p) {
   extern __shared__ __attribute__((aligned(16))) unsigned char smem[];
   const int img = blockIdx.x;
   if (img >= p.nimg) return;
@@ -373,6 +380,9 @@
         chunkA(nb, 1, 1);
       }
     }
+    if constexpr (ENDS) {
+      if (p.tail.pooled) wg_barrier();
+    }
     return;
   }
 
@@ -976,6 +986,40 @@
     }
     CP(58);
   }
+  if constexpr (ENDS) {
+    if (p.tail.pooled) {
+      const Geo L = fresh_geo();
+      float mu, rs;
+      ln_stats(xr, mu, rs, p.eps);
+      const bool lv = L.l31 < live;
+      if (L.g == 0 && lv) {
+        p.tail.mean[grow0 + L.l31] = mu;
+        p.tail.rstd[grow0 + L.l31] = rs;
+      }
+      float xh[96];
+#pragma unroll
+      for (int c = 0; c < 12; ++c)
+#pragma unroll
+        for (int d = 0; d < 4; ++d) {
+          const unsigned u = xr.v[c][d];
+          xh[8 * c + 2 * d] = lv ? (bf_lo(u) - mu) * rs : 0.f;
+          xh[8 * c + 2 * d + 1] = lv ? (bf_hi(u) - mu) * rs : 0.f;
+        }
+      token_sum96(xh, L.l31);
+      float* tab = reinterpret_cast<float*>(smem + POOL_OFF);
+#pragma unroll
+      for (int k = 0; k < 3; ++k) tab[w * E + feature_of(3 * L.l31 + k, L.g)] = xh[k];
+      wait_lds();
+      wg_barrier();
+      if (w < E / 64) {
+        const int e = w * 64 + L.lane;
+        float a = tab[e];
+#pragma unroll
+        for (int r = 1; r < NCW; ++r) a += tab[r * E + e];
+        p.tail.pooled[(size_t)img * E + e] = (bf16)(a * (1.f / NTOK) * p.tail.ln_g[e] + p.tail.ln_b[e]);
+      }
+    }
+  }
   CP_RT(127);
 }
 
@@ -1015,14 +1059,18 @@
   return RGBNM_OK;
 }
 
-int rgbnm_vit_chain_fwd(const rgbnm_vit_cfg* c, const rgbnm_chain_block* blocks, int depth, const void* x0, void* stream) {
+int rgbnm_vit_chain_fwd_ends(const rgbnm_vit_cfg* c, const rgbnm_chain_block* blocks, int depth, const void* x0,
+                             const rgbnm_chain_fwd_tail* tail, void* stream) {
   if (!c || !blocks || !x0 || depth <= 0) return RGBNM_EINVAL;
+  if (tail && (!tail->ln_g || !tail->ln_b || !tail->mean || !tail->rstd || !tail->pooled)) return RGBNM_EINVAL;
   if (c->dtype != RGBNM_DT_BF16 || c->E != E || c->heads != HEADS || c->N != NTOK || c->B < 1 || depth > MAX_DEPTH) return 1;
   const unsigned* img = nullptr;
   int A0 = 0, P1 = 0, N1 = 0, ndw = 0;
   if (rgbnm_gelu_table_query(&img, &A0, &P1, &N1, &ndw) != 1 || ndw * 4 > TAB_LIMIT) return 1;
-  ChainArgs p;
+  ChainArgsEnds p;
   memcpy(p.blk, blocks, sizeof(ChainBlk) * depth);
+  memset(&p.tail, 0, sizeof(p.tail));
+  if (tail) memcpy(&p.tail, tail, sizeof(p.tail));
   p.x0 = (const bf16*)x0; p.depth = depth; p.nimg = c->B;
   p.eps = c->ln_eps; p.scale = c->attn_scale;
   p.tab_img = img; p.tab_pieces = (ndw * 4 + 15) / 16;
@@ -1033,7 +1081,8 @@
   p.ksgn = 0x00010001u * (unsigned)(4 * (P1 - A0 + 2));
   static DevOnce attr;
   if (attr.need()) {
-    if (hipFuncSetAttribute((const void*)vit_chain_fwd_kernel, hipFuncAttributeMaxDynamicSharedMemorySize, SMEM) != hipSuccess)
+    if (hipFuncSetAttribute((const void*)vit_chain_fwd_kernel<false>, hipFuncAttributeMaxDynamicSharedMemorySize, SMEM) != hipSuccess ||
+        hipFuncSetAttribute((const void*)vit_chain_fwd_kernel<true>, hipFuncAttributeMaxDynamicSharedMemorySize, SMEM) != hipSuccess)
       return RGBNM_ELAUNCH;
     attr.done();
   }
@@ -1041,10 +1090,15 @@
   const double flops = depth * tok * 2.0 * (E * 3.0 * INNER + 2.0 * NTOK * INNER + INNER * E + 2.0 * E * HID);
   const double bytes = depth * (tok * ((5.0 * E + 3.0 * INNER + 2.0 * HID) * 2.0 + 4 * 4 + HEADS * 4) + 12.0 * SLOT + 12.0 * STAGE) + tok * E * 2.0;
   const int slot = rgbnm_trace_begin(TR_CHAIN_FWD, flops, bytes, (hipStream_t)stream);
-  hipLaunchKernelGGL(vit_chain_fwd_kernel, dim3(c->B), dim3(NTHREADS), SMEM, (hipStream_t)stream, p);
+  if (tail) hipLaunchKernelGGL(vit_chain_fwd_kernel<true>, dim3(c->B), dim3(NTHREADS), SMEM, (hipStream_t)stream, p);
+  else hipLaunchKernelGGL(vit_chain_fwd_kernel<false>, dim3(c->B), dim3(NTHREADS), SMEM, (hipStream_t)stream, static_cast<const ChainArgs&>(p));
   rgbnm_trace_end(slot, (hipStream_t)stream);
   LAUNCH_CHECK();
   return RGBNM_OK;
 }
 
-}
+int rgbnm_vit_chain_fwd(const rgbnm_vit_cfg* c, const rgbnm_chain_block* blocks, int depth, const void* x0, void* stream) {
+  return rgbnm_vit_chain_fwd_ends(c, blocks, depth, x0, nullptr, stream);
+}
+
+}
diff --git a/rgb-no-more_amd/csrc/vit_chain_bwd.hip b/rgb-no-more_amd/csrc/vit_chain_bwd.hip
--- a/rgb-no-more_amd/csrc/vit_chain_bwd.hip
+++ b/rgb-no-more_amd/csrc/vit_chain_bwd.hip
@@ -4,6 +4,7 @@
 #include "internal.h"
 #include "ln_bwd_rows.h"
 #include "tile128.h"
+#include "chain_ends.h"
 #include "../../include/rgbnm.h"
 
 namespace {
@@ -51,6 +52,11 @@
   int depth, nimg;
   float scale;
 };
+struct BwdHead { const bf16* dpooled; const bf16* x; const float *ln_g, *mean, *rstd; float* part; float *dln_g, *dln_b; };
+static_assert(sizeof(BwdHead) == sizeof(rgbnm_chain_bwd_head), "rgbnm_chain_bwd_head layout");
+struct BwdArgsEnds : BwdArgs { BwdHead head; };
+constexpr int HEAD_TAB = M_STG + NCW * 2 * TILE;
+static_assert(HEAD_TAB + NCW * E * 4 <= SMEM, "LDS");
 
 #ifndef XB_ROWPIPE
 #define XB_ROWPIPE 1
@@ -227,7 +233,8 @@
   }
 }
 
-__global__ __launch_bounds__(NTHREADS) void vit_chain_bwd_kernel(BwdArgs p) {
+template <bool ENDS>
+__global__ __launch_bounds__(NTHREADS) void vit_chain_bwd_kernel(std::conditional_t<ENDS, BwdArgsEnds, BwdArgs> p) {
   extern __shared__ __attribute__((aligned(16))) unsigned char smem[];
   const int img = blockIdx.x;
   if (img >= p.nimg) return;
@@ -243,6 +250,9 @@
       const BwdBlk& b = p.blk[ib];
       const unsigned char* wimg = reinterpret_cast<const unsigned char*>(b.wimg);
       dma_linear<48>(wimg, smem, lane);
+      if constexpr (ENDS) {
+        if (ib == depth - 1 && p.head.dpooled) wg_barrier();
+      }
       for (int c = 0; c < NCHUNK; ++c) {
         wait_vm<0>();
         BAR(B_M0 + c);
@@ -343,7 +353,79 @@
   const float c2 = p.scale * LOG2E;
 
   Rows dyf;
-  {
+  if constexpr (ENDS) {
+    if (p.head.dpooled) {
+      const int lane_ = lane_id_here(), l31 = lane_ & 31, g = lane_ >> 5;
+      const int rloc = row0 + l31, tok = rloc < NTOK ? rloc : NTOK - 1;
+      const bool lv = rloc < NTOK;
+      const size_t grow = (size_t)img * NTOK + tok;
+      Rows xr;
+      {
+        const bf16* xrow = p.head.x + grow * E + 8 * g;
+#pragma unroll
+        for (int c = 0; c < 12; ++c) xr.v[c] = *reinterpret_cast<const u32x4*>(xrow + 16 * c);
+      }
+      const float mu = p.head.mean[grow], rs = p.head.rstd[grow];
+      const bf16* dp = p.head.dpooled + (size_t)img * E + 8 * g;
+      const float* gm = p.head.ln_g + 8 * g;
+      const float invN = 1.f / NTOK;
+      auto xval = [&](int c, int j) { const unsigned u = xr.v[c][j >> 1]; return (j & 1) ? __builtin_bit_cast(float, u & 0xffff0000u) : __builtin_bit_cast(float, u << 16); };
+      float dg[96], s1 = 0.f, s2 = 0.f;
+#pragma unroll
+      for (int c = 0; c < 12; ++c) {
+        const bf16x8 d8 = *reinterpret_cast<const bf16x8*>(dp + 16 * c);
+        const f32x4 g0 = *reinterpret_cast<const f32x4*>(gm + 16 * c), g1 = *reinterpret_cast<const f32x4*>(gm + 16 * c + 4);
+#pragma unroll
+        for (int j = 0; j < 8; ++j) {
+          const float xh = (xval(c, j) - mu) * rs, dv = (float)d8[j] * invN, gv = dv * (j < 4 ? g0[j] : g1[j - 4]);
+          s1 += gv;
+          s2 += gv * xh;
+          dg[8 * c + j] = lv ? dv * xh : 0.f;
+        }
+      }
+      s1 += __shfl_xor(s1, 32, 64);
+      s2 += __shfl_xor(s2, 32, 64);
+      const float c1 = s1 * (1.f / E), c2 = s2 * (1.f / E);
+      token_sum96(dg, l31);
+      float* tab = reinterpret_cast<float*>(smem + HEAD_TAB);
+#pragma unroll
+      for (int k = 0; k < 3; ++k) tab[w * E + feature_of(3 * l31 + k, g)] = dg[k];
+      __builtin_amdgcn_sched_barrier(0);
+#pragma unroll
+      for (int c = 0; c < 12; ++c) {
+        const bf16x8 d8 = *reinterpret_cast<const bf16x8*>(dp + 16 * c);
+        const f32x4 g0 = *reinterpret_cast<const f32x4*>(gm + 16 * c), g1 = *reinterpret_cast<const f32x4*>(gm + 16 * c + 4);
+        float o[8];
+#pragma unroll
+        for (int j = 0; j < 8; ++j) {
+          const float xh = (xval(c, j) - mu) * rs, gv = (float)d8[j] * invN * (j < 4 ? g0[j] : g1[j - 4]);
+          o[j] = rs * (gv - c1 - xh * c2);
+        }
+#pragma unroll
+        for (int d = 0; d < 4; ++d) dyf.v[c][d] = pack2(o[2 * d], o[2 * d + 1]);
+      }
+      bf16* dyo = const_cast<bf16*>(p.blk[depth - 1].dy) + grow0 * E;
+      const unsigned stg = (unsigned)(M_STG + w * 2 * TILE);
+#pragma unroll
+      for (int t = 0; t < 3; ++t) {
+        tile_out(smem, stg, dyf.v[4 * t], dyf.v[4 * t + 1], dyf.v[4 * t + 2], dyf.v[4 * t + 3], dyo + 64 * t, E, live);
+        __builtin_amdgcn_sched_barrier(0);
+      }
+      wait_lds();
+      wg_barrier();
+      if (w < E / 64) {
+        const int e = w * 64 + lane_;
+        float a = tab[e];
+#pragma unroll
+        for (int r = 1; r < NCW; ++r) a += tab[r * E + e];
+        p.head.part[((size_t)img * 2 + 0) * E + e] = a;
+        p.head.part[((size_t)img * 2 + 1) * E + e] = (float)p.head.dpooled[(size_t)img * E + e];
+      }
+    }
+  }
+  bool load_dy = true;
+  if constexpr (ENDS) load_dy = !p.head.dpooled;
+  if (load_dy) {
     const int lane_ = lane_id_here();
     const int rloc = row0 + (lane_ & 31), tok = rloc < NTOK ? rloc : NTOK - 1;
     const bf16* yrow = p.blk[depth - 1].dy + ((size_t)img * NTOK + tok) * E + 8 * (lane_ >> 5);
@@ -780,15 +862,21 @@
 
 size_t rgbnm_chain_bwd_block_bytes(void) { return sizeof(BwdBlk); }
 
-int rgbnm_vit_chain_bwd(const rgbnm_vit_cfg* c, const rgbnm_chain_bwd_block* blocks, int depth, void* dattn, void* stream) {
+int rgbnm_vit_chain_bwd_ends(const rgbnm_vit_cfg* c, const rgbnm_chain_bwd_block* blocks, int depth, void* dattn,
+                             const rgbnm_chain_bwd_head* head, void* stream) {
   if (!c || !blocks || !dattn || depth <= 0) return RGBNM_EINVAL;
+  if (head && (!head->dpooled || !head->x || !head->ln_g || !head->mean || !head->rstd || !head->part || !head->dln_g || !head->dln_b))
+    return RGBNM_EINVAL;
   if (c->dtype != RGBNM_DT_BF16 || c->E != E || c->heads != HEADS || c->N != NTOK || c->B < 1 || depth > MAX_DEPTH) return 1;
-  BwdArgs p;
+  BwdArgsEnds p;
   memcpy(p.blk, blocks, sizeof(BwdBlk) * depth);
+  memset(&p.head, 0, sizeof(p.head));
+  if (head) memcpy(&p.head, head, sizeof(p.head));
   p.dattn = (bf16*)dattn; p.depth = depth; p.nimg = c->B; p.scale = c->attn_scale;
   static DevOnce attr;
   if (attr.need()) {
-    if (hipFuncSetAttribute((const void*)vit_chain_bwd_kernel, hipFuncAttributeMaxDynamicSharedMemorySize, SMEM) != hipSuccess)
+    if (hipFuncSetAttribute((const void*)vit_chain_bwd_kernel<false>, hipFuncAttributeMaxDynamicSharedMemorySize, SMEM) != hipSuccess ||
+        hipFuncSetAttribute((const void*)vit_chain_bwd_kernel<true>, hipFuncAttributeMaxDynamicSharedMemorySize, SMEM) != hipSuccess)
       return RGBNM_ELAUNCH;
     attr.done();
   }
@@ -796,10 +884,30 @@
   const double flops = depth * tok * 2.0 * (2.0 * E * HID + INNER * E + 3.0 * INNER * E + 4.0 * NTOK * INNER);
   const double bytes = depth * (tok * ((2.0 * HID + 5.0 * E + 2.0 * 3.0 * INNER) * 2.0 + 4 * 4 + HEADS * 4) + 36.0 * SLOT) + tok * E * 2.0;
   const int slot = rgbnm_trace_begin(TR_CHAIN_BWD, flops, bytes, (hipStream_t)stream);
-  hipLaunchKernelGGL(vit_chain_bwd_kernel, dim3(c->B), dim3(NTHREADS), SMEM, (hipStream_t)stream, p);
+  if (head) hipLaunchKernelGGL(vit_chain_bwd_kernel<true>, dim3(c->B), dim3(NTHREADS), SMEM, (hipStream_t)stream, p);
+  else hipLaunchKernelGGL(vit_chain_bwd_kernel<false>, dim3(c->B), dim3(NTHREADS), SMEM, (hipStream_t)stream, static_cast<const BwdArgs&>(p));
   rgbnm_trace_end(slot, (hipStream_t)stream);
   LAUNCH_CHECK();
-  return RGBNM_OK;
-}
-
-}
+  if (!head) return RGBNM_OK;
+  RgbnmReduceJob j;
+  j.part = head->part; j.stride = 2LL * E; j.out = head->dln_g; j.n = E; j.S = c->B; j.cols = 1; j.perm_heads = 0;
+  j.accumulate = 0; j.epw = 8;
+  const bool own = !rgbnm_reduce_defer_active();
+  if (own) rgbnm_reduce_defer_begin();
+  int rc = rgbnm_reduce_submit(j, (hipStream_t)stream);
+  if (rc == RGBNM_OK) {
+    j.part = head->part + E; j.out = head->dln_b;
+    rc = rgbnm_reduce_submit(j, (hipStream_t)stream);
+  }
+  if (own) {
+    const int rf = rgbnm_reduce_defer_flush((hipStream_t)stream);
+    if (rc == RGBNM_OK) rc = rf;
+  }
+  return rc;
+}
+
+int rgbnm_vit_chain_bwd(const rgbnm_vit_cfg* c, const rgbnm_chain_bwd_block* blocks, int depth, void* dattn, void* stream) {
+  return rgbnm_vit_chain_bwd_ends(c, blocks, depth, dattn, nullptr, stream);
+}
+
+}
diff --git a/rgb-no-more_amd/lib.py b/rgb-no-more_amd/lib.py
--- a/rgb-no-more_amd/lib.py
+++ b/rgb-no-more_amd/lib.py
@@ -74,6 +74,14 @@
 class ChainBwdBlock(C.Structure):
     _fields_ = [(n, _vp) for n in ("wimg", "ln1_g", "ln2_g", "x_in", "mean1", "rstd1", "qkv", "lse", "attn", "x_mid", "mean2",
                                    "rstd2", "u", "dy", "du", "dx_mid", "dqkv", "dx", "part2", "part1")]
+
+
+class ChainFwdTail(C.Structure):
+    _fields_ = [(n, _vp) for n in ("ln_g", "ln_b", "mean", "rstd", "pooled")]
+
+
+class ChainBwdHead(C.Structure):
+    _fields_ = [(n, _vp) for n in ("dpooled", "x", "ln_g", "mean", "rstd", "part", "dln_g", "dln_b")]
 
 
 ABI_VERSION = 3
@@ -160,8 +168,10 @@
     "rgbnm_chain_image_elems": (_ll, []),
     "rgbnm_chain_gather": (_i, [_vp, _vp, _vp, _ll, _vp]),
     "rgbnm_vit_chain_fwd": (_i, [_P(VitCfg), _P(ChainBlock), _i, _vp, _vp]),
+    "rgbnm_vit_chain_fwd_ends": (_i, [_P(VitCfg), _P(ChainBlock), _i, _vp, _P(ChainFwdTail), _vp]),
     "rgbnm_chain_bwd_block_bytes": (_sz, []),
     "rgbnm_vit_chain_bwd": (_i, [_P(VitCfg), _P(ChainBwdBlock), _i, _vp, _vp]),
+    "rgbnm_vit_chain_bwd_ends": (_i, [_P(VitCfg), _P(ChainBwdBlock), _i, _vp, _P(ChainBwdHead), _vp]),
     "rgbnm_vit_block_bwd_dw": (_i, [_P(VitCfg), _P(BlockActs), _P(BlockGrads), _P(BlockScratch), _vp, _vp, _vp, _vp]),
     "rgbnm_vit_blocks_bwd_dw": (_i, [_P(VitCfg), _i, _vp, _vp, _vp, _vp, _vp, _vp, _vp]),
     "rgbnm_vit_blocks_bwd_dw_pe": (_i, [_P(VitCfg), _i, _vp, _vp, _vp, _vp, _vp, _vp, _vp, _vp, _vp, _vp, _vp, _sz, _vp]),
@@ -177,6 +187,8 @@
     "rgbnm_head_fwd": (_i, [_P(VitCfg), _P(HeadParams), _P(HeadActs), _vp]),
     "rgbnm_head_bwd": (_i, [_P(VitCfg), _P(HeadParams), _P(HeadActs), _P(HeadGrads), _vp, _vp, _vp, _vp, _vp, _sz,
                             _vp]),
+    "rgbnm_head_fwd_pooled": (_i, [_P(VitCfg), _P(HeadParams), _P(HeadActs), _vp]),
+    "rgbnm_head_bwd_pooled": (_i, [_P(VitCfg), _P(HeadParams), _P(HeadActs), _P(HeadGrads), _vp, _vp, _vp, _vp, _sz, _vp]),
 }
 
 _lib = None
diff --git a/rgb-no-more_amd/plainvit.py b/rgb-no-more_amd/plainvit.py
--- a/rgb-no-more_amd/plainvit.py
+++ b/rgb-no-more_amd/plainvit.py
@@ -423,7 +423,7 @@
             ctx.st, ctx.idx = st, idx
             return a.xbuf(idx + 1).detach()
         if idx == 0:
-            st.chain_fwd = m._chain_forward(a)
+            st.chain_fwd = m._chain_forward(a, st)
         if st.chain_fwd:
             ctx.st, ctx.idx = st, idx
             return a.xbuf(idx + 1).detach()
@@ -450,7 +450,7 @@
         scratch = a.scratch_blk[idx] if st.holding else a.scratch
         if idx == m.depth - 1:
             m._check_prep_gen(st)
-            st.chain_bwd = st.drop is None and m._chain_backward(a, dy)
+            st.chain_bwd = st.drop is None and m._chain_backward(a, dy, st)
             st.dw_pending = []
         try:
             if st.drop is not None:
@@ -506,7 +506,7 @@
     def forward(ctx, x, st, *params):
         m, a = st.model, st.arena
         assert x.data_ptr() == a.xbuf(0).data_ptr()
-        st.chain_fwd = m._chain_forward(a)
+        st.chain_fwd = m._chain_forward(a, st)
         if not st.chain_fwd:
             chain = st.ln_chain
             for idx in range(m.depth):
@@ -528,7 +528,7 @@
         gs = [L.BlockGrads(*[t.data_ptr() for t in grads[i]]) for i in range(D)]
         m._check_prep_gen(st)
         try:
-            if m._chain_backward(a, dy):
+            if m._chain_backward(a, dy, st):
                 group = D if (m._grad_sync is None or st.holding) else m.dw_group_overlapped
                 group = min(group, CHAIN_MAX_DEPTH)
                 idx = D - 1
@@ -589,7 +589,10 @@
         logits = torch.empty(a.B, m._ncls_pad, device=x.device, dtype=torch.float32)
         acts = L.HeadActs(x.data_ptr(), a.hmean.data_ptr(), a.hrstd.data_ptr(), a.pooled.data_ptr(),
                           a.h1.data_ptr(), logits.data_ptr())
-        L.check(L.lib().rgbnm_head_fwd(C.byref(a.cfg), C.byref(m._hparams), C.byref(acts), L.stream()), "head_fwd")
+        if getattr(st, "pooled", False):
+            L.check(L.lib().rgbnm_head_fwd_pooled(C.byref(a.cfg), C.byref(m._hparams), C.byref(acts), L.stream()), "head_fwd_pooled")
+        else:
+            L.check(L.lib().rgbnm_head_fwd(C.byref(a.cfg), C.byref(m._hparams), C.byref(acts), L.stream()), "head_fwd")
         ctx.st, ctx.acts, ctx.x = st, acts, x
         ctx.set_materialize_grads(False)
         if m._ncls_pad != m.n_classes:
@@ -625,10 +628,21 @@
         if not padded:
             st.begin_hold()
         ws = a.ws_head if st.holding else a.ws
+        fold = (st.holding and getattr(st, "chain_fwd", False) and st.drop is None and m._chain_backward_eligible(a)
+                and L.lib().rgbnm_get_option(b"fold_pool_bwd") and ctx.x.data_ptr() == a.xbuf(m.depth).data_ptr())
         try:
-            L.check(L.lib().rgbnm_head_bwd(C.byref(a.cfg), C.byref(m._hparams), C.byref(ctx.acts), C.byref(g),
-                                           dl.data_ptr(), a.da.data_ptr(), a.dpooled.data_ptr(), dx.data_ptr(),
-                                           ws.data_ptr(), ws.numel(), L.stream()), "head_bwd")
+            if fold:
+                L.check(L.lib().rgbnm_head_bwd_pooled(C.byref(a.cfg), C.byref(m._hparams), C.byref(ctx.acts), C.byref(g),
+                                                      dl.data_ptr(), a.da.data_ptr(), a.dpooled.data_ptr(),
+                                                      ws.data_ptr(), ws.numel(), L.stream()), "head_bwd_pooled")
+                if getattr(a, "hpart", None) is None:
+                    a.hpart = torch.empty(a.B, 2, m.emb_size, device=dx.device, dtype=torch.float32)
+                st.pool_bwd = L.ChainBwdHead(a.dpooled.data_ptr(), ctx.x.data_ptr(), m._hparams.ln_g, a.hmean.data_ptr(),
+                                             a.hrstd.data_ptr(), a.hpart.data_ptr(), g.dln_g, g.dln_b)
+            else:
+                L.check(L.lib().rgbnm_head_bwd(C.byref(a.cfg), C.byref(m._hparams), C.byref(ctx.acts), C.byref(g),
+                                               dl.data_ptr(), a.da.data_ptr(), a.dpooled.data_ptr(), dx.data_ptr(),
+                                               ws.data_ptr(), ws.numel(), L.stream()), "head_bwd")
             if padded:
                 grads[names.index("classhead.ch_linear2.weight")].copy_(dw2p[:m.n_classes])
                 grads[names.index("classhead.ch_linear2.bias")].copy_(db2p[:m.n_classes])
@@ -893,7 +907,7 @@
             warnings.warn(f"rgb-no-more_amd: the one-launch encoder {which} kernel refused this model (no GELU "
                           f"table); running the per-operation kernels (about 2x slower)", RuntimeWarning, stacklevel=3)
 
-    def _chain_forward(self, a):
+    def _chain_forward(self, a, st=None):
         if a.cdtype != torch.bfloat16 or self._chain_idx is None or not L.lib().rgbnm_get_option(b"fwd_chain"):
             return False
         if a.chain_table is None:
@@ -906,10 +920,16 @@
                                          ac.xn1, ac.mean1, ac.rstd1, ac.qkv, ac.lse, ac.attn, ac.x_mid, ac.xn2, ac.mean2, ac.rstd2,
                                          ac.u, ac.gl, ac.x_out)
             a.chain_table = blocks
+            a.chain_tail = L.ChainFwdTail(self._hparams.ln_g, self._hparams.ln_b, a.hmean.data_ptr(), a.hrstd.data_ptr(),
+                                          a.pooled.data_ptr())
+        tail = st is not None and bool(L.lib().rgbnm_get_option(b"fold_pool_fwd"))
         for s0 in range(0, self.depth, CHAIN_MAX_DEPTH):
             n = min(CHAIN_MAX_DEPTH, self.depth - s0)
             sub = C.cast(C.byref(a.chain_table, s0 * C.sizeof(L.ChainBlock)), C.POINTER(L.ChainBlock))
-            rc = L.lib().rgbnm_vit_chain_fwd(C.byref(a.cfg), sub, n, a.xbuf(s0).data_ptr(), L.stream())
+            if tail and s0 + n == self.depth:
+                rc = L.lib().rgbnm_vit_chain_fwd_ends(C.byref(a.cfg), sub, n, a.xbuf(s0).data_ptr(), C.byref(a.chain_tail), L.stream())
+            else:
+                rc = L.lib().rgbnm_vit_chain_fwd(C.byref(a.cfg), sub, n, a.xbuf(s0).data_ptr(), L.stream())
             if rc == 1 and s0 == 0:
                 self._warn_chain_refused("forward")
                 if not self._chain_refused:
@@ -917,11 +937,27 @@
                     self._prep(a.cdtype)
                 return False
             L.check(rc, "vit_chain_fwd")
+        if tail:
+            st.pooled = True
         return True
 
-    def _chain_backward(self, a, dy):
-        if (a.cdtype != torch.bfloat16 or self._chain_idx is None or not a.need_grad
-                or not L.lib().rgbnm_get_option(b"bwd_chain")):
+    def _chain_backward_eligible(self, a):
+        return bool(a.cdtype == torch.bfloat16 and self._chain_idx is not None and a.need_grad
+                    and L.lib().rgbnm_get_option(b"bwd_chain"))
+
+    def _pool_backward(self, a, head, dy):
+        L.check(L.lib().rgbnm_head_pool_bwd(L.dt_of(a.cdtype), head.dpooled, head.x, head.ln_g, head.mean, head.rstd, dy.data_ptr(),
+                                            head.dln_g, head.dln_b, a.B, self.n_tokens, self.emb_size, 0, head.part,
+                                            a.hpart.numel() * 4, L.stream()), "head_pool_bwd")
+
+    def _chain_backward(self, a, dy, st=None):
+        head = getattr(st, "pool_bwd", None)
+        if head is not None:
+            st.pool_bwd = None
+            if dy.data_ptr() != a.dx[0].data_ptr() or not self._chain_backward_eligible(a):
+                self._pool_backward(a, head, dy)
+                head = None
+        if not self._chain_backward_eligible(a):
             return False
         D, dev = self.depth, self._flat.device
         if a.chain_bwd_table is None or a.chain_bwd_dy != dy.data_ptr():
@@ -951,8 +987,13 @@
         for s0 in reversed(starts):
             n = min(CHAIN_MAX_DEPTH, D - s0)
             sub = C.cast(C.byref(a.chain_bwd_table, s0 * C.sizeof(L.ChainBwdBlock)), C.POINTER(L.ChainBwdBlock))
-            rc = L.lib().rgbnm_vit_chain_bwd(C.byref(a.cfg), sub, n, a.dattn_chain.data_ptr(), L.stream())
+            if head is not None and s0 == starts[-1]:
+                rc = L.lib().rgbnm_vit_chain_bwd_ends(C.byref(a.cfg), sub, n, a.dattn_chain.data_ptr(), C.byref(head), L.stream())
+            else:
+                rc = L.lib().rgbnm_vit_chain_bwd(C.byref(a.cfg), sub, n, a.dattn_chain.data_ptr(), L.stream())
             if rc == 1 and s0 == starts[-1]:
+                if head is not None:
+                    self._pool_backward(a, head, dy)
                 self._warn_chain_refused("backward")
                 if not self._chain_refused:
                     self._chain_refused = True
```

Result: no change. 68200 (median of 6 runs) (+0.3%).
